# meudnaes/VoronoiRT

Measured on AMD Instinct MI355X. Metric: formal-solve cell-updates/sec, higher is better.
Workload: dtype f64

## Files before the change

### include/voronoirt.h

```cpp
#ifndef VORONOIRT_H
#define VORONOIRT_H

#include <stdint.h>

#ifdef __cplusplus
extern "C" {
#endif

#define VRT_OK 0
#define VRT_EINVAL (-1)
#define VRT_EGRID (-2)
#define VRT_ENODEVICE (-3)
#define VRT_ENOMEM (-4)
#define VRT_EIO (-5)

typedef struct vrt_grid vrt_grid;
typedef struct vrt_plan vrt_plan;

#define VRT_ALPHA_SITE 0
#define VRT_ALPHA_SITE_LAM 1
#define VRT_ALPHA_ANGLE_SITE_LAM 2
#define VRT_ALPHA_ANGLE_NATIVE 3
#define VRT_ALPHA_SITE_LAM_NATIVE 4

// ... 36 lines not shown
int64_t vrt_plan_num_levels(const vrt_plan *p);
int64_t vrt_plan_num_nodes(const vrt_plan *p);
int vrt_plan_get_upwind(const vrt_plan *p, int64_t angle, int64_t *up, double *dots, double *w,
                        double *r);

int vrt_plan_execute(vrt_plan *p, int64_t nlam, int64_t ld, const double *S, const double *alpha,
                     int alpha_mode, const double *I0_up, const double *I0_down,
                     const double *weights, double *J, double *I_out);
int vrt_plan_execute_dev(vrt_plan *p, int64_t nlam, int64_t ld, const double *dS,
                         const double *dalpha, int alpha_mode, const double *dI0_up,
                         const double *dI0_down, const double *weights_host, double *dJ,
                         double *dI_out, void *stream);
int vrt_grid_get_storage_order(const vrt_grid *g, int dir, int64_t *out);
int64_t vrt_plan_native_alpha_count(const vrt_plan *p, int64_t nlam);
int vrt_plan_native_pair_block(const vrt_plan *p);
int vrt_plan_native_pair_block_f32(const vrt_plan *p);
int vrt_plan_alpha_to_native_dev(vrt_plan *p, int64_t nlam, int64_t ld, const double *dalpha,
                                 double *dalpha_native, void *stream);
int vrt_plan_alpha_to_native_dev_f32(vrt_plan *p, int64_t nlam, int64_t ld, const float *dalpha,
                                     float *dalpha_native, void *stream);

int64_t vrt_plan_native_plane_count(const vrt_plan *p, int64_t nlam);
int vrt_plan_to_native_dev(vrt_plan *p, int64_t nlam, int64_t ld, const double *d_in, double *d_up, double *d_down,
                           void *stream);
int vrt_plan_from_native_dev(vrt_plan *p, int dir, int64_t nlam, int64_t ld, const double *d_native, double *d_out,
                             void *stream);
int vrt_plan_j_from_native_dev(vrt_plan *p, int64_t nlam, int64_t ld, const double *dJ_up, const double *dJ_down,
                               double *dJ, void *stream);
int vrt_plan_execute_native_dev(vrt_plan *p, int64_t nlam, const double *dS_up, const double *dS_down,
                                const double *dalpha, int alpha_mode, const double *dI0_up, const double *dI0_down,
                                const double *weights_host, double *dJ_up, double *dJ_down, void *stream);
int vrt_plan_to_native_dev_f32(vrt_plan *p, int64_t nlam, int64_t ld, const float *d_in, float *d_up, float *d_down,
                               void *stream);
int vrt_plan_from_native_dev_f32(vrt_plan *p, int dir, int64_t nlam, int64_t ld, const float *d_native, float *d_out,
                                 void *stream);
int vrt_plan_j_from_native_dev_f32(vrt_plan *p, int64_t nlam, int64_t ld, const float *dJ_up, const float *dJ_down,
                                   float *dJ, void *stream);
int vrt_plan_execute_native_dev_f32(vrt_plan *p, int64_t nlam, const float *dS_up, const float *dS_down,
                                    const float *dalpha, int alpha_mode, const float *dI0_up, const float *dI0_down,
                                    const double *weights_host, float *dJ_up, float *dJ_down, void *stream);

int vrt_lambda_update_native_dev(vrt_grid *g, int64_t nlam, const double *dJ_up, const double *dJ_down,
                                 const double *dB_up, const double *deps, double *dS_up, double *dS_down,
                                 double *max_rel_change, void *stream);
int vrt_rates_populations_native_dev(vrt_grid *g, int64_t nlam, const double *lambda, const int64_t blocks[6],
                                     const double *dJ_up, const double *dJ_down, const double *planck2,
                                     double lambda0, double c0, const double *d_doppler_width, const double *d_gamma,
                                     double sigma_bb_const, const double *sigma_bf1, const double *sigma_bf2,
                                     const double *d_temperature, const double *d_lte_populations, double hc_over_kB,
                                     double pref_ij, double pref_ji, const double *d_C, const double *d_atom_density,
                                     double *d_R, double *d_populations, void *stream);
int vrt_lambda_update_native_dev_f32(vrt_plan *p, int64_t nlam, const float *dJ_up, const float *dJ_down,
                                     const float *dB_up, const double *deps, float *dS_up, float *dS_down,
                                     double *max_rel_change, void *stream);
int vrt_rates_populations_native_dev_f32(vrt_plan *p, int64_t nlam, const double *lambda, const int64_t blocks[6],
                                         const float *dJ_up, const float *dJ_down, const double *planck2,
                                         double lambda0, double c0, const double *d_doppler_width, const double *d_gamma,
                                         double sigma_bb_const, const double *sigma_bf1, const double *sigma_bf2,
                                         const double *d_temperature, const double *d_lte_populations, double hc_over_kB,
                                         double pref_ij, double pref_ji, const double *d_C, const double *d_atom_density,
                                         double *d_R, double *d_populations, void *stream);
int vrt_rate_shares_native_dev(vrt_grid *g, int64_t nlam, int64_t l0, int64_t l1, const double *lambda,
                               const int64_t blocks[6], const double *dJ_up, const double *dJ_down, const double *planck2,
                               double lambda0, double c0, const double *d_doppler_width, const double *d_gamma,
                               double sigma_bb_const, const double *sigma_bf1, const double *sigma_bf2,
                               const double *d_temperature, const double *d_lte_populations, double hc_over_kB,
                               double pref_ij, double pref_ji, double *d_shares, void *stream);
int vrt_rate_shares_native_dev_f32(vrt_plan *p, int64_t nlam, int64_t l0, int64_t l1, const double *lambda,
                                   const int64_t blocks[6], const float *dJ_up, const float *dJ_down, const double *planck2,
                                   double lambda0, double c0, const double *d_doppler_width, const double *d_gamma,
                                   double sigma_bb_const, const double *sigma_bf1, const double *sigma_bf2,
                                   const double *d_temperature, const double *d_lte_populations, double hc_over_kB,
                                   double pref_ij, double pref_ji, double *d_shares, void *stream);
int vrt_populations_from_shares_dev(int64_t n, const double *d_shares, const double *d_C, const double *d_atom_density,
                                    double *d_R, double *d_populations, void *stream);

int vrt_plan_execute_dev_f32(vrt_plan *p, int64_t nlam, int64_t ld, const float *dS,
                             const float *dalpha, int alpha_mode, const float *dI0_up,
                             const float *dI0_down, const double *weights_host, float *dJ,
                             float *dI_out, void *stream);
int vrt_plan_last_sweep_timing(const vrt_plan *p, double *ms, int64_t *launches);
int vrt_plan_patch_layout(const vrt_plan *p, int64_t *out);
int vrt_patch_dispatch_map(int order, int nrow, int nsplit, int lg_siblings, int64_t nred, int steps, int64_t *dims, int32_t *blocks);
int vrt_plan_patch_timeline(vrt_plan *p, int64_t cap_launches, int64_t cap_blocks, int64_t *launches, uint64_t *stamps, int64_t *counts);
int vrt_plan_check(vrt_plan *p);
int vrt_plan_last_path(const vrt_plan *p);
int vrt_plan_set_option(vrt_plan *p, const char *name, const char *value);
int vrt_grid_set_option(vrt_grid *g, const char *name, const char *value);

typedef struct vrt_schedule vrt_schedule;
int vrt_schedule_build(const vrt_grid *g, int dir, const int64_t *up, int n_sweeps, vrt_schedule **out);
int64_t vrt_schedule_num_nodes(const vrt_schedule *s);
int64_t vrt_schedule_num_levels(const vrt_schedule *s);
int vrt_schedule_get(const vrt_schedule *s, int64_t *site, int32_t *zflags, int64_t *level_off);
void vrt_schedule_destroy(vrt_schedule *s);
int vrt_layer_schedule(const vrt_grid *g, int dir, const int64_t *up, int n_sweeps, uint32_t *vis,
                       int32_t *nlev, int64_t *n_visits);
int vrt_layer_sorted_slots(const vrt_grid *g, int dir, const uint32_t *vis, int64_t *store, int64_t *self);

typedef struct vrt_patch_schedule vrt_patch_schedule;
int vrt_patch_schedule_build(const vrt_grid *g, int dir, const int64_t *up, int n_sweeps, int own_target,
                             int entry_cap, vrt_patch_schedule **out, int64_t counts[6]);
int vrt_patch_schedule_get(const vrt_patch_schedule *s, int32_t *layer_patch_off, int32_t *patch_own_lo,
                           int32_t *patch_own_cnt, int32_t *patch_nlev, int64_t *patch_ent_off,
                           int32_t *entry_pos, uint32_t *entry_vis, uint32_t *entry_loc);
int vrt_patch_schedule_get_deps(const vrt_patch_schedule *s, int64_t *dep_off, int32_t *dep_list);
int vrt_patch_schedule_get_layers(const vrt_patch_schedule *s, uint32_t *vis, int32_t *nlev, int64_t *n_visits);
void vrt_patch_schedule_destroy(vrt_patch_schedule *s);

int vrt_delaunay_up(vrt_grid *g, const double k[3], const double *S, const double *I0,
                    int64_t nI0, const double *alpha, int n_sweeps, double *I_out);
int vrt_delaunay_down(vrt_grid *g, const double k[3], const double *S, const double *I0,
                      int64_t nI0, const double *alpha, int n_sweeps, double *I_out);

#define VRT_METRIC_EUCLIDEAN   0
#define VRT_METRIC_PERIODIC_XY 1
#define VRT_RASTER_NEAREST     1
#define VRT_RASTER_INV_DIST2   2
int vrt_grid_nearest(vrt_grid *g, int64_t nq, const double *q_zxy, int metric, int k, int64_t *idx, double *dist);
int vrt_grid_to_raster_dev(vrt_grid *g, int64_t nz, int64_t nx, int64_t ny, const double *z, const double *x,
                           const double *y, int metric, int mode, int64_t nf, int64_t ld, const double *d_fields,
                           double *d_raster, void *stream);
int vrt_raster_to_grid_dev(vrt_grid *g, int64_t nz, int64_t nx, int64_t ny, const double *z, const double *x,
                           const double *y, int64_t nf, const double *d_raster, int64_t ld, double *d_fields,
                           void *stream);
int vrt_grid_to_raster(vrt_grid *g, int64_t nz, int64_t nx, int64_t ny, const double *z, const double *x,
                       const double *y, int metric, int mode, int64_t nf, int64_t ld, const double *fields,
                       double *raster);
int vrt_raster_to_grid(vrt_grid *g, int64_t nz, int64_t nx, int64_t ny, const double *z, const double *x,
                       const double *y, int64_t nf, const double *raster, int64_t ld, double *fields);
int vrt_grid_raster_stats(const vrt_grid *g, double *nearest_ms, double *gather_ms, int64_t *queries,
                          int64_t *walk_steps, int64_t *fallbacks);

int vrt_sample_sites(int device, int64_t nz, int64_t nx, int64_t ny, const double *z, const double *x, const double *y,
                     const double *quantity, int64_t n_sites, uint64_t seed, int64_t batch, int64_t max_proposals,
                     double *pos_zxy, int64_t *proposals_used);
int vrt_sample_sites_dev(int device, int64_t nz, int64_t nx, int64_t ny, const double *z, const double *x,
                         const double *y, const double *d_quantity, int64_t n_sites, uint64_t seed, int64_t batch,
                         int64_t max_proposals, double *d_pos_zxy, int64_t *proposals_used, void *stream);

int vrt_lambda_update_dev(vrt_grid *g, int64_t nlam, int64_t ld, const double *dJ, const double *dB,
                          const double *deps, const double *dS_old, double *dS_new,
                          double *max_rel_change, void *stream);

int vrt_line_opacity_dev(vrt_plan *p, int64_t nlam, const double *lambda, double lambda0, double c0,
                         const double *d_velocity, const double *d_doppler_width, const double *d_gamma,
                         const double *d_line_strength, const double *d_alpha_cont, double *d_alpha_native,
                         void *stream);
int vrt_line_opacity_dev_f32(vrt_plan *p, int64_t nlam, const double *lambda, double lambda0, double c0,
                             const double *d_velocity, const double *d_doppler_width, const double *d_gamma,
                             const double *d_line_strength, const double *d_alpha_cont, float *d_alpha_native,
                             void *stream);

int vrt_plan_execute_line(vrt_plan *p, int64_t nlam, int64_t ld, const double *lambda, double lambda0, double c0,
                          const double *velocity, const double *doppler_width, const double *gamma,
                          const double *line_strength, const double *alpha_cont, const double *S, const double *I0_up,
                          const double *I0_down, const double *weights, double *J);

int vrt_line_terms_dev(vrt_grid *g, const double *d_gamma_static, const double *d_gamma_unsold,
                       const double *d_populations, double strength_const, double Bij, double Bji, double *d_gamma,
                       double *d_line_strength, void *stream);

typedef struct vrt_lambda vrt_lambda;
typedef struct vrt_line_case {
    int64_t nlam;
    const double *lambda;
// ... 209 lines not shown
```

### voronoirt_amd/_lib.py

```python
from __future__ import annotations

import ctypes
import os

HERE = os.path.dirname(os.path.abspath(__file__))
LIB_PATH = os.path.join(HERE, "libvrt_hip.so")
if os.environ.get("VRT_LIB_PATH"):
    LIB_PATH = os.environ["VRT_LIB_PATH"]

c_i64 = ctypes.c_int64
c_dbl = ctypes.c_double
p_i64 = ctypes.POINTER(ctypes.c_int64)
p_i32 = ctypes.POINTER(ctypes.c_int32)
p_dbl = ctypes.POINTER(ctypes.c_double)
p_int = ctypes.POINTER(ctypes.c_int)
vp = ctypes.c_void_p

VRT_OK, VRT_EINVAL, VRT_EGRID, VRT_ENODEVICE, VRT_ENOMEM, VRT_EIO = 0, -1, -2, -3, -4, -5
ALPHA_SITE, ALPHA_SITE_LAM, ALPHA_ANGLE_SITE_LAM, ALPHA_ANGLE_NATIVE, ALPHA_SITE_LAM_NATIVE = 0, 1, 2, 3, 4
METRIC_EUCLIDEAN, METRIC_PERIODIC_XY = 0, 1
RASTER_NEAREST, RASTER_INV_DIST2 = 1, 2
REG_FORMS = ("solve<256>", "solve<1024>", "xy_march_lds<1>", "xy_march_lds<2>", "xy_march_lds<4>", "xy_march_lds<0>",
             "xy_march_mem")
REG_FORM_KERNEL_MASK, REG_FORM_YZ_ROW_MARCH, REG_FORM_XZ_ROW_MARCH = 0xff, 0x100, 0x200
# ... 28 lines not shown
    "vrt_tessellate_sites": (ctypes.c_int, [c_i64, p_dbl, p_dbl, c_i64, c_i64, p_i64, p_i64, p_i64]),
    "vrt_write_neighbours_file": (ctypes.c_int, [ctypes.c_char_p, c_i64, p_i64, c_i64]),
    "vrt_grid_n": (c_i64, [vp]),
    "vrt_grid_max_neighbours": (c_i64, [vp]),
    "vrt_grid_num_layer_offsets": (c_i64, [vp, ctypes.c_int]),
    "vrt_grid_get_layers": (ctypes.c_int, [vp, ctypes.c_int, p_i64]),
    "vrt_grid_get_perm": (ctypes.c_int, [vp, ctypes.c_int, p_i64]),
    "vrt_grid_get_delaunay_lines": (ctypes.c_int, [vp, p_dbl]),
    "vrt_direction": (None, [c_dbl, c_dbl, p_dbl]),
    "vrt_plan_create": (ctypes.c_int, [vp, c_i64, p_dbl, ctypes.c_int, ctypes.POINTER(vp)]),
    "vrt_plan_create_ex": (ctypes.c_int, [vp, c_i64, p_dbl, p_int, ctypes.c_int,
                                          ctypes.POINTER(vp)]),
    "vrt_plan_destroy": (None, [vp]),
    "vrt_plan_num_levels": (c_i64, [vp]),
    "vrt_plan_num_nodes": (c_i64, [vp]),
    "vrt_plan_get_upwind": (ctypes.c_int, [vp, c_i64, p_i64, p_dbl, p_dbl, p_dbl]),
    "vrt_plan_execute": (ctypes.c_int, [vp, c_i64, c_i64, p_dbl, p_dbl, ctypes.c_int, p_dbl, p_dbl,
                                        p_dbl, p_dbl, p_dbl]),
    "vrt_plan_execute_dev": (ctypes.c_int, [vp, c_i64, c_i64, vp, vp, ctypes.c_int, vp, vp, p_dbl,
                                            vp, vp, vp]),
    "vrt_plan_execute_dev_f32": (ctypes.c_int, [vp, c_i64, c_i64, vp, vp, ctypes.c_int, vp, vp, p_dbl,
                                                vp, vp, vp]),
    "vrt_plan_native_plane_count": (c_i64, [vp, c_i64]),
    "vrt_plan_to_native_dev": (ctypes.c_int, [vp, c_i64, c_i64, vp, vp, vp, vp]),
    "vrt_plan_from_native_dev": (ctypes.c_int, [vp, ctypes.c_int, c_i64, c_i64, vp, vp, vp]),
    "vrt_plan_j_from_native_dev": (ctypes.c_int, [vp, c_i64, c_i64, vp, vp, vp, vp]),
    "vrt_plan_execute_native_dev": (ctypes.c_int, [vp, c_i64, vp, vp, vp, ctypes.c_int, vp, vp, p_dbl, vp, vp, vp]),
    "vrt_plan_to_native_dev_f32": (ctypes.c_int, [vp, c_i64, c_i64, vp, vp, vp, vp]),
    "vrt_plan_from_native_dev_f32": (ctypes.c_int, [vp, ctypes.c_int, c_i64, c_i64, vp, vp, vp]),
    "vrt_plan_j_from_native_dev_f32": (ctypes.c_int, [vp, c_i64, c_i64, vp, vp, vp, vp]),
    "vrt_plan_execute_native_dev_f32": (ctypes.c_int, [vp, c_i64, vp, vp, vp, ctypes.c_int, vp, vp, p_dbl, vp, vp, vp]),
    "vrt_plan_check": (ctypes.c_int, [vp]),
    "vrt_lambda_update_native_dev": (ctypes.c_int, [vp, c_i64, vp, vp, vp, vp, vp, vp, p_dbl, vp]),
    "vrt_rates_populations_native_dev": (ctypes.c_int, [vp, c_i64, p_dbl, p_i64, vp, vp, p_dbl, c_dbl, c_dbl, vp, vp,
                                                        c_dbl, p_dbl, p_dbl, vp, vp, c_dbl, c_dbl, c_dbl, vp, vp, vp,
                                                        vp, vp]),
    "vrt_lambda_update_native_dev_f32": (ctypes.c_int, [vp, c_i64, vp, vp, vp, vp, vp, vp, p_dbl, vp]),
    "vrt_rates_populations_native_dev_f32": (ctypes.c_int, [vp, c_i64, p_dbl, p_i64, vp, vp, p_dbl, c_dbl, c_dbl, vp, vp,
                                                            c_dbl, p_dbl, p_dbl, vp, vp, c_dbl, c_dbl, c_dbl, vp, vp, vp,
                                                            vp, vp]),
    "vrt_rate_shares_native_dev": (ctypes.c_int, [vp, c_i64, c_i64, c_i64, p_dbl, p_i64, vp, vp, p_dbl, c_dbl, c_dbl, vp, vp,
                                                  c_dbl, p_dbl, p_dbl, vp, vp, c_dbl, c_dbl, c_dbl, vp, vp]),
    "vrt_rate_shares_native_dev_f32": (ctypes.c_int, [vp, c_i64, c_i64, c_i64, p_dbl, p_i64, vp, vp, p_dbl, c_dbl, c_dbl, vp, vp,
                                                      c_dbl, p_dbl, p_dbl, vp, vp, c_dbl, c_dbl, c_dbl, vp, vp]),
    "vrt_populations_from_shares_dev": (ctypes.c_int, [c_i64, vp, vp, vp, vp, vp, vp]),
    "vrt_grid_get_storage_order": (ctypes.c_int, [vp, ctypes.c_int, p_i64]),
    "vrt_plan_native_alpha_count": (c_i64, [vp, c_i64]),
    "vrt_plan_native_pair_block": (ctypes.c_int, [vp]),
    "vrt_plan_native_pair_block_f32": (ctypes.c_int, [vp]),
    "vrt_plan_alpha_to_native_dev": (ctypes.c_int, [vp, c_i64, c_i64, vp, vp, vp]),
    "vrt_line_opacity_dev": (ctypes.c_int, [vp, c_i64, p_dbl, c_dbl, c_dbl, vp, vp, vp, vp, vp, vp, vp]),
    "vrt_line_opacity_dev_f32": (ctypes.c_int, [vp, c_i64, p_dbl, c_dbl, c_dbl, vp, vp, vp, vp, vp, vp, vp]),
    "vrt_plan_alpha_to_native_dev_f32": (ctypes.c_int, [vp, c_i64, c_i64, vp, vp, vp]),
    "vrt_plan_execute_line": (ctypes.c_int, [vp, c_i64, c_i64, p_dbl, c_dbl, c_dbl, p_dbl, p_dbl, p_dbl, p_dbl, p_dbl,
                                             p_dbl, p_dbl, p_dbl, p_dbl, p_dbl]),
    "vrt_line_terms_dev": (ctypes.c_int, [vp, vp, vp, vp, c_dbl, c_dbl, c_dbl, vp, vp, vp]),
    "vrt_lambda_create": (ctypes.c_int, [vp, ctypes.POINTER(LineCaseStruct), p_dbl, ctypes.POINTER(vp)]),
    "vrt_lambda_create_f32": (ctypes.c_int, [vp, ctypes.POINTER(LineCaseStruct), p_dbl, ctypes.POINTER(vp)]),
    "vrt_lambda_storage": (ctypes.c_int, [vp]),
    "vrt_lambda_iterate": (ctypes.c_int, [vp, p_dbl]),
    "vrt_lambda_get": (ctypes.c_int, [vp, p_dbl, p_dbl, p_dbl, p_dbl, p_dbl]),
    "vrt_lambda_destroy": (None, [vp]),
    "vrt_multi_create": (ctypes.c_int, [ctypes.c_int, p_int, c_i64, p_dbl, p_i64, c_i64, p_dbl, c_i64, p_dbl, p_int,
                                        ctypes.c_int, ctypes.POINTER(vp)]),
    "vrt_multi_execute": (ctypes.c_int, [vp, c_i64, c_i64, p_dbl, p_dbl, ctypes.c_int, p_dbl, p_dbl, p_dbl, p_dbl]),
    "vrt_multi_set_shard": (ctypes.c_int, [vp, ctypes.c_char_p]),
    "vrt_multi_last_shard": (ctypes.c_int, [vp]),
    "vrt_multi_uses_rccl": (ctypes.c_int, [vp]),
    "vrt_multi_destroy": (None, [vp]),
    "vrt_multi_execute_line": (ctypes.c_int, [vp, c_i64, c_i64, p_dbl, c_dbl, c_dbl, p_dbl, p_dbl, p_dbl, p_dbl, p_dbl, p_dbl,
                                              p_dbl, p_dbl, p_dbl, p_dbl]),
    "vrt_multi_lambda_create": (ctypes.c_int, [vp, ctypes.POINTER(LineCaseStruct), p_dbl, ctypes.POINTER(vp)]),
    "vrt_multi_lambda_create_f32": (ctypes.c_int, [vp, ctypes.POINTER(LineCaseStruct), p_dbl, ctypes.POINTER(vp)]),
    "vrt_multi_lambda_storage": (ctypes.c_int, [vp]),
    "vrt_multi_lambda_iterate": (ctypes.c_int, [vp, p_dbl]),
    "vrt_multi_lambda_get": (ctypes.c_int, [vp, p_dbl, p_dbl, p_dbl, p_dbl, p_dbl]),
    "vrt_multi_lambda_destroy": (None, [vp]),
    "vrt_rates_populations_dev": (ctypes.c_int, [vp, c_i64, c_i64, p_dbl, p_i64, vp, p_dbl, c_dbl, c_dbl, vp, vp,
                                                 c_dbl, p_dbl, p_dbl, vp, vp, c_dbl, c_dbl, c_dbl, vp, vp, vp,
                                                 vp, vp]),
    "vrt_plan_last_sweep_timing": (ctypes.c_int, [vp, p_dbl, p_i64]),
    "vrt_plan_patch_layout": (ctypes.c_int, [vp, p_i64]),
    "vrt_patch_dispatch_map": (ctypes.c_int, [ctypes.c_int, ctypes.c_int, ctypes.c_int, ctypes.c_int, c_i64, ctypes.c_int, p_i64, p_i32]),
    "vrt_plan_patch_timeline": (ctypes.c_int, [vp, c_i64, c_i64, p_i64, ctypes.POINTER(ctypes.c_uint64), p_i64]),
    "vrt_plan_last_path": (ctypes.c_int, [vp]),
    "vrt_plan_set_option": (ctypes.c_int, [vp, ctypes.c_char_p, ctypes.c_char_p]),
    "vrt_grid_set_option": (ctypes.c_int, [vp, ctypes.c_char_p, ctypes.c_char_p]),
    "vrt_schedule_build": (ctypes.c_int, [vp, ctypes.c_int, p_i64, ctypes.c_int,
                                          ctypes.POINTER(vp)]),
    "vrt_schedule_num_nodes": (c_i64, [vp]),
    "vrt_schedule_num_levels": (c_i64, [vp]),
    "vrt_schedule_get": (ctypes.c_int, [vp, p_i64, p_i32, p_i64]),
    "vrt_schedule_destroy": (None, [vp]),
    "vrt_layer_schedule": (ctypes.c_int, [vp, ctypes.c_int, p_i64, ctypes.c_int,
                                          ctypes.POINTER(ctypes.c_uint32), p_i32, p_i64]),
    "vrt_layer_sorted_slots": (ctypes.c_int, [vp, ctypes.c_int, ctypes.POINTER(ctypes.c_uint32), p_i64, p_i64]),
    "vrt_patch_schedule_build": (ctypes.c_int, [vp, ctypes.c_int, p_i64, ctypes.c_int, ctypes.c_int, ctypes.c_int,
                                                ctypes.POINTER(vp), p_i64]),
    "vrt_patch_schedule_get": (ctypes.c_int, [vp, p_i32, p_i32, p_i32, p_i32, p_i64, p_i32,
                                              ctypes.POINTER(ctypes.c_uint32), ctypes.POINTER(ctypes.c_uint32)]),
    "vrt_patch_schedule_get_deps": (ctypes.c_int, [vp, p_i64, p_i32]),
    "vrt_patch_schedule_get_layers": (ctypes.c_int, [vp, ctypes.POINTER(ctypes.c_uint32), p_i32, p_i64]),
    "vrt_patch_schedule_destroy": (None, [vp]),
    "vrt_lambda_update_dev": (ctypes.c_int, [vp, c_i64, c_i64, vp, vp, vp, vp, vp, p_dbl, vp]),
    "vrt_short_characteristics": (ctypes.c_int, [c_i64, c_i64, c_i64, p_dbl, p_dbl, p_dbl, c_i64, p_dbl,
                                                 p_int, p_dbl, c_i64, p_dbl, c_i64, p_dbl, ctypes.c_int,
                                                 ctypes.c_int, p_dbl]),
    "vrt_regular_create": (ctypes.c_int, [c_i64, c_i64, c_i64, p_dbl, p_dbl, p_dbl, ctypes.c_int,
                                          ctypes.POINTER(vp)]),
    "vrt_regular_destroy": (None, [vp]),
    "vrt_regular_execute_dev": (ctypes.c_int, [vp, c_i64, p_dbl, p_int, vp, c_i64, vp, c_i64, c_i64, vp,
                                               ctypes.c_int, vp, vp]),
    "vrt_regular_last_solve_ms": (ctypes.c_int, [vp, p_dbl]),
    "vrt_regular_last_launch_form": (ctypes.c_int, [vp, p_int, p_int]),
    "vrt_regular_execute_line": (ctypes.c_int, [vp, c_i64, p_dbl, p_int, p_dbl, c_i64, p_dbl, c_dbl, c_dbl, p_dbl, p_dbl,
                                                p_dbl, p_dbl, p_dbl, p_dbl, p_dbl, ctypes.c_int, p_dbl]),
    "vrt_regular_lambda_create": (ctypes.c_int, [vp, c_i64, p_dbl, p_int, p_dbl, ctypes.POINTER(LineCaseStruct), ctypes.c_int,
                                                 ctypes.POINTER(vp)]),
    "vrt_regular_lambda_iterate": (ctypes.c_int, [vp, p_dbl]),
    "vrt_regular_lambda_get": (ctypes.c_int, [vp, p_dbl, p_dbl, p_dbl, p_dbl, p_dbl]),
    "vrt_regular_lambda_destroy": (None, [vp]),
    "vrt_synth_opacity_dev": (ctypes.c_int, [c_i64, c_i64, c_i64, p_dbl, c_i64, p_dbl, p_dbl, c_dbl, c_dbl, c_dbl, c_dbl,
                                             c_dbl, c_dbl, c_dbl, c_dbl, vp, vp, vp, vp, vp, vp, vp, vp, vp, vp]),
    "vrt_synth_opacity": (ctypes.c_int, [ctypes.c_int, c_i64, c_i64, c_i64, p_dbl, c_i64, p_dbl, p_dbl, c_dbl, c_dbl,
                                         c_dbl, c_dbl, c_dbl, c_dbl, c_dbl, c_dbl, p_dbl, p_dbl, p_dbl, p_dbl, p_dbl,
                                         p_dbl, p_dbl, p_dbl, p_dbl]),
    "vrt_regular_emergent_dev": (ctypes.c_int, [vp, p_dbl, c_i64, vp, vp, ctypes.c_int, vp, vp]),
    "vrt_top_intensity": (ctypes.c_int, [c_i64, c_i64, c_i64, p_dbl, p_dbl, p_dbl, p_dbl, c_i64, p_dbl, p_dbl,
                                         ctypes.c_int, ctypes.c_int, p_dbl]),
    "vrt_tau_unity_dev": (ctypes.c_int, [c_i64, c_i64, c_i64, p_dbl, p_dbl, p_dbl, p_dbl, c_i64, vp, vp, vp]),
    "vrt_tau_unity": (ctypes.c_int, [c_i64, c_i64, c_i64, p_dbl, p_dbl, p_dbl, p_dbl, c_i64, p_dbl, ctypes.c_int,
                                     p_dbl]),
    "vrt_grid_nearest": (ctypes.c_int, [vp, c_i64, p_dbl, ctypes.c_int, ctypes.c_int, p_i64, p_dbl]),
    "vrt_grid_to_raster_dev": (ctypes.c_int, [vp, c_i64, c_i64, c_i64, p_dbl, p_dbl, p_dbl, ctypes.c_int, ctypes.c_int,
                                              c_i64, c_i64, vp, vp, vp]),
    "vrt_raster_to_grid_dev": (ctypes.c_int, [vp, c_i64, c_i64, c_i64, p_dbl, p_dbl, p_dbl, c_i64, vp, c_i64, vp, vp]),
    "vrt_grid_to_raster": (ctypes.c_int, [vp, c_i64, c_i64, c_i64, p_dbl, p_dbl, p_dbl, ctypes.c_int, ctypes.c_int,
                                          c_i64, c_i64, p_dbl, p_dbl]),
    "vrt_raster_to_grid": (ctypes.c_int, [vp, c_i64, c_i64, c_i64, p_dbl, p_dbl, p_dbl, c_i64, p_dbl, c_i64, p_dbl]),
    "vrt_grid_raster_stats": (ctypes.c_int, [vp, p_dbl, p_dbl, p_i64, p_i64, p_i64]),
    "vrt_sample_sites": (ctypes.c_int, [ctypes.c_int, c_i64, c_i64, c_i64, p_dbl, p_dbl, p_dbl, p_dbl, c_i64,
                                        ctypes.c_uint64, c_i64, c_i64, p_dbl, p_i64]),
    "vrt_sample_sites_dev": (ctypes.c_int, [ctypes.c_int, c_i64, c_i64, c_i64, p_dbl, p_dbl, p_dbl, vp, c_i64,
                                            ctypes.c_uint64, c_i64, c_i64, vp, p_i64, vp]),
    "vrt_ng_accelerate_dev": (ctypes.c_int, [c_i64, vp, vp, vp, vp, vp, p_dbl, p_dbl, p_int, vp]),
    "vrt_ng_sums_dev": (ctypes.c_int, [c_i64, vp, vp, vp, vp, p_dbl, vp]),
    "vrt_ng_coefficients": (ctypes.c_int, [p_dbl, p_dbl]),
    "vrt_ng_apply_dev": (ctypes.c_int, [c_i64, c_dbl, c_dbl, vp, vp, vp, vp, p_int, vp]),
    "vrt_lambda_set_acceleration": (ctypes.c_int, [vp, ctypes.c_int, ctypes.c_int, ctypes.c_int]),
    "vrt_regular_lambda_set_acceleration": (ctypes.c_int, [vp, ctypes.c_int, ctypes.c_int, ctypes.c_int]),
    "vrt_lambda_last_acceleration": (ctypes.c_int, [vp, p_int, p_dbl, p_dbl]),
    "vrt_regular_lambda_last_acceleration": (ctypes.c_int, [vp, p_int, p_dbl, p_dbl]),
    "vrt_lambda_set_state": (ctypes.c_int, [vp, p_dbl, p_dbl]),
    "vrt_regular_lambda_set_state": (ctypes.c_int, [vp, p_dbl, p_dbl]),
    "vrt_multi_lambda_set_state": (ctypes.c_int, [vp, p_dbl, p_dbl]),
    "vrt_continuum_case_check": (ctypes.c_int, [ctypes.POINTER(ContinuumCaseStruct), c_i64]),
    "vrt_continuum_create": (ctypes.c_int, [vp, ctypes.POINTER(ContinuumCaseStruct), p_dbl, ctypes.POINTER(vp)]),
    "vrt_continuum_iterate": (ctypes.c_int, [vp, p_dbl]),
    "vrt_continuum_get": (ctypes.c_int, [vp, p_dbl, p_dbl]),
    "vrt_continuum_set_source": (ctypes.c_int, [vp, p_dbl]),
    "vrt_continuum_set_acceleration": (ctypes.c_int, [vp, ctypes.c_int, ctypes.c_int, ctypes.c_int]),
    "vrt_continuum_last_acceleration": (ctypes.c_int, [vp, p_int, p_dbl, p_dbl]),
    "vrt_continuum_destroy": (None, [vp]),
    "vrt_regular_continuum_create": (ctypes.c_int, [vp, c_i64, p_dbl, p_int, p_dbl, ctypes.POINTER(ContinuumCaseStruct),
                                                    ctypes.c_int, ctypes.POINTER(vp)]),
    "vrt_regular_continuum_iterate": (ctypes.c_int, [vp, p_dbl]),
# ... 87 lines not shown
```

### voronoirt_amd/api.py

```python
from __future__ import annotations

import ctypes
import os
import re
import weakref

import numpy as np

from . import _lib
from ._lib import VrtError, check

QUADRATURE_DIR = os.path.join(os.path.dirname(os.path.abspath(__file__)), "quadratures")


def _d(a):
    return a.ctypes.data_as(_lib.p_dbl) if a is not None else None


def _i(a):
    return a.ctypes.data_as(_lib.p_i64) if a is not None else None


def _f64(a):
    return np.ascontiguousarray(a, dtype=np.float64)
# ... 247 lines not shown

    def to_native_dev(self, nlam: int, ld: int, d_in: int, d_up: int = 0, d_down: int = 0, stream: int = 0, f32: bool = False) -> None:
        fn = _lib.load().vrt_plan_to_native_dev_f32 if f32 else _lib.load().vrt_plan_to_native_dev
        check(fn(self._h, nlam, ld, d_in, d_up or None, d_down or None, stream or None))

    def from_native_dev(self, d: int, nlam: int, ld: int, d_native: int, d_out: int, stream: int = 0, f32: bool = False) -> None:
        fn = _lib.load().vrt_plan_from_native_dev_f32 if f32 else _lib.load().vrt_plan_from_native_dev
        check(fn(self._h, int(d), nlam, ld, d_native, d_out, stream or None))

    def J_from_native_dev(self, nlam: int, ld: int, dJ_up: int, dJ_down: int, dJ: int, stream: int = 0, f32: bool = False) -> None:
        fn = _lib.load().vrt_plan_j_from_native_dev_f32 if f32 else _lib.load().vrt_plan_j_from_native_dev
        check(fn(self._h, nlam, ld, dJ_up or None, dJ_down or None, dJ, stream or None))

    def execute_native_dev(self, nlam: int, dS_up: int, dS_down: int, dalpha: int, alpha_mode: int, weights,
                           dJ_up: int = 0, dJ_down: int = 0, dI0_up: int = 0, dI0_down: int = 0, stream: int = 0,
                           f32: bool = False) -> None:
        w = _f64(weights)
        fn = _lib.load().vrt_plan_execute_native_dev_f32 if f32 else _lib.load().vrt_plan_execute_native_dev
        check(fn(self._h, nlam, dS_up or None, dS_down or None, dalpha, alpha_mode, dI0_up or None, dI0_down or None, _d(w),
                 dJ_up or None, dJ_down or None, stream or None))

    def check(self) -> None:
        check(_lib.load().vrt_plan_check(self._h))

    def native_alpha_count(self, nlam: int) -> int:
        return int(_lib.load().vrt_plan_native_alpha_count(self._h, nlam))

    @property
    def native_pair_block(self) -> int:
        return int(_lib.load().vrt_plan_native_pair_block(self._h))

    @property
    def native_pair_block_f32(self) -> int:
        return int(_lib.load().vrt_plan_native_pair_block_f32(self._h))

    def native_to_site_major(self, native, nlam: int, n_angles: int):
        native = np.asarray(native)
        n = self.sites.n
        B = self.native_pair_block_f32 if native.dtype == np.float32 else self.native_pair_block
        npair = (nlam + 1) // 2
        per = native.reshape(n_angles, npair * n * 2)
        out = np.empty((n_angles, n, 2 * npair), dtype=native.dtype)
        q0 = 0
        widths = [B] * (npair // B) + [1 << b for b in range(B.bit_length() - 2, -1, -1) if (npair % B) & (1 << b)]
        for w in widths:
            blk = per[:, q0 * n * 2:(q0 + w) * n * 2].reshape(n_angles, n, 2 * w)
            out[:, :, 2 * q0:2 * (q0 + w)] = blk
            q0 += w
        return out[:, :, :nlam]

    def alpha_to_native_dev(self, nlam: int, ld: int, dalpha: int, dalpha_native: int, stream: int = 0,
                            f32: bool = False) -> None:
        fn = _lib.load().vrt_plan_alpha_to_native_dev_f32 if f32 else _lib.load().vrt_plan_alpha_to_native_dev
        check(fn(self._h, nlam, ld, dalpha, dalpha_native, stream or None))

    def line_opacity_dev(self, lam, lambda0: float, c0: float, d_velocity: int, d_doppler: int, d_gamma: int,
                         d_line_strength: int, d_alpha_cont: int, d_alpha_native: int, stream: int = 0,
                         f32: bool = False) -> None:
        lam = _f64(lam)
        fn = _lib.load().vrt_line_opacity_dev_f32 if f32 else _lib.load().vrt_line_opacity_dev
        check(fn(self._h, lam.size, _d(lam), float(lambda0), float(c0), d_velocity, d_doppler, d_gamma, d_line_strength,
                 d_alpha_cont, d_alpha_native, stream or None))

    def line_lambda_diagonal_dev(self, nlam: int, d_alpha_native: int, weights, ld: int, d_diag: int, stream: int = 0) -> None:
        check(_lib.load().vrt_line_lambda_diagonal_dev(self._h, nlam, d_alpha_native, _d(_f64(weights)), ld, d_diag,
                                                       stream or None))

    def set_option(self, name: str, value) -> None:
        if getattr(self, "_h", None):
            check(_lib.load().vrt_plan_set_option(self._h, name.encode(), str(value).encode()))

    def last_sweep_timing(self):
        ms = ctypes.c_double()
        launches = ctypes.c_int64()
        check(_lib.load().vrt_plan_last_sweep_timing(self._h, ctypes.byref(ms),
                                                     ctypes.byref(launches)))
        return ms.value, launches.value

    @property
    def patch_layout(self) -> dict:
        out = (ctypes.c_int64 * 4)()
        check(_lib.load().vrt_plan_patch_layout(self._h, out))
        return {"patches": out[0], "fewest_per_angle_layer": out[1], "work_slots": out[2], "padding_slots": out[3]}

    @property
    def last_launches(self) -> int:
        return int(self.last_sweep_timing()[1])

    @property
    def last_path(self) -> str:
        return {0: "", 1: "levels", 2: "tiles", 3: "steps", 4: "patches"}[int(_lib.load().vrt_plan_last_path(self._h))]

    def close(self):
        if getattr(self, "_h", None) is not None and self._h:
            _lib.load().vrt_plan_destroy(self._h)
            self._h = None

    def __del__(self):
        try:
            self.close()
        except Exception:
            pass


class MultiDevicePlan:

    def __init__(self, positions, neighbours, bounds, k, dirs=None, n_sweeps: int = 3, devices=(0,)):
        L = _lib.load()
        pos = _f64(positions)
        nbr = np.ascontiguousarray(neighbours, dtype=np.int64)
        b = np.array([float(v) for v in bounds], dtype=np.float64)
        self.k = _f64(np.atleast_2d(k))
        self.n, self.n_angles = pos.shape[0], self.k.shape[0]
        dev = np.ascontiguousarray(devices, dtype=np.int32)
        d = np.ascontiguousarray(dirs, dtype=np.int32) if dirs is not None else None
        h = ctypes.c_void_p()
        check(L.vrt_multi_create(dev.size, dev.ctypes.data_as(_lib.p_int), self.n, _d(pos), _i(nbr), nbr.shape[0], _d(b),
                                 self.n_angles, _d(self.k), d.ctypes.data_as(_lib.p_int) if d is not None else None,
                                 int(n_sweeps), ctypes.byref(h)))
        self._h = h

    def set_shard(self, mode: str) -> None:
        check(_lib.load().vrt_multi_set_shard(self._h, mode.encode()))

    @property
    def last_shard(self) -> str:
        return {0: "", 1: "lambda", 2: "angle"}[int(_lib.load().vrt_multi_last_shard(self._h))]

    @property
    def uses_rccl(self) -> bool:
        return bool(_lib.load().vrt_multi_uses_rccl(self._h))

    def execute(self, S, alpha, weights, I0_up=None, I0_down=None, alpha_mode=None) -> np.ndarray:
        S = _f64(S)
        if S.ndim == 1:
            S = S.reshape(-1, 1)
        n, nlam = S.shape
        alpha = _f64(alpha)
        if alpha_mode is None:
            alpha_mode = {1: _lib.ALPHA_SITE, 2: _lib.ALPHA_SITE_LAM, 3: _lib.ALPHA_ANGLE_SITE_LAM}[alpha.ndim]
        if I0_up is not None:
            I0_up = _f64(I0_up).reshape(-1, nlam)
        if I0_down is not None:
            I0_down = _f64(I0_down).reshape(-1, nlam)
        w = _f64(weights)
        J = np.zeros((n, nlam))
        check(_lib.load().vrt_multi_execute(self._h, nlam, nlam, _d(S), _d(alpha), alpha_mode, _d(I0_up), _d(I0_down),
                                            _d(w), _d(J)))
        return J

    def execute_line(self, S, populations, case, weights, perm_up, n1: int) -> np.ndarray:
        S = _f64(S)
        n, nlam = S.shape
        pops = np.asarray(populations)
        gamma = _f64(case.gamma(pops))
        strength = _f64(case.strength_const * (pops[0] * case.Bij - pops[1] * case.Bji))
        lam, vel, dop, ac = _f64(case.lam), _f64(case.velocity), _f64(case.doppler), _f64(case.alpha_cont)
        I0 = _f64(np.asarray(case.B0)[np.asarray(perm_up)[:n1] - 1])
        J = np.zeros((n, nlam))
        check(_lib.load().vrt_multi_execute_line(self._h, nlam, nlam, _d(lam), float(case.lambda0), float(case.c0), _d(vel),
                                                 _d(dop), _d(gamma), _d(strength), _d(ac), _d(S), _d(I0), None,
                                                 _d(_f64(weights)), _d(J)))
        return J

    def lambda_iteration(self, eps_conv: float, maxiter: int, case, weights, S0=None, populations0=None, checkpoint=None,
                         checkpoint_every: int = 1, resume=None, ng=None, storage: str = "f64"):
# ... 1323 lines not shown
```

### voronoirt_amd/csrc/vrt_api.cpp

```cpp
#include <algorithm>
#include <atomic>
#include <chrono>
#include <cmath>
#include <cstdio>
#include <cstdlib>
#include <cstring>
#include <memory>
#include <new>
#include <thread>

#include "vrt_internal.h"
#include "vrt_line_case.h"

namespace vrt {

static thread_local std::string g_err;

void set_error(const std::string &msg) { g_err = msg; }
int fail(int code, const std::string &msg)
{
    g_err = msg;
    return code;
}

int check_source(const double *S, int64_t count)
{
    for (int64_t i = 0; i < count; i++)
        if (!std::isfinite(S[i]) || !(S[i] > 0.0)) return fail(VRT_EINVAL, "S must be finite and > 0 everywhere");
    return VRT_OK;
}

int check_state_pointers(const void *session, const double *S, const double *populations)
{
    if (!session) return fail(VRT_EINVAL, "NULL session");
    if (!S && !populations) return fail(VRT_EINVAL, "S and populations are both NULL: nothing to set");
    return VRT_OK;
}

int check_state(int64_t n, int64_t nlam, const double *S, const double *populations)
{
    if (S)
        if (int rc = check_source(S, n * nlam)) return rc;
    if (populations)
        for (int64_t i = 0; i < 3 * n; i++)
            if (!std::isfinite(populations[i]) || !(populations[i] >= 0.0))
                return fail(VRT_EINVAL, "the populations must be finite and >= 0 everywhere");
    return VRT_OK;
}

void tuning_from_env(Tuning &t)
{
    static const char *names[] = {"VRT_PATH", "VRT_STEP_K", "VRT_STEP_SINGLE", "VRT_STEP_PAIRS", "VRT_STEP_XCD",
                                  "VRT_STEP_STREAMS", "VRT_STEP_LEVEL_MAP", "VRT_STEP_GROUP_DIR", "VRT_TILE_WIDE",
                                  "VRT_TILE_PRE", "VRT_PATCH_K", "VRT_PATCH_NT", "VRT_PATCH_OWN",
                                  "VRT_PATCH_Q", "VRT_PATCH_TARGET", "VRT_PATCH_SPLIT", "VRT_PATCH_ORDER", "VRT_PATCH_TIMELINE", "VRT_PAIR_BLOCK", "VRT_PATCH_QUAD", "VRT_PATCH_LEAN", "VRT_PATCH_CHAIN", "VRT_CHAIN_PAIRS", "VRT_CHAIN_SPIN", "VRT_CHAIN_DATAFLAG", "VRT_CHAIN_STATIC", "VRT_LAMBDA_NATIVE", "VRT_DEBUG_FLAGS", "VRT_DEBUG_SKIP_LEVELS",
                                  "VRT_TILE_DEBUG"};
    for (const char *nm : names) {
        const char *e = std::getenv(nm);
        if (e && *e && tuning_set(t, nm, e, false) != VRT_OK) {
            static std::mutex mu;
            static std::vector<std::string> said;
            std::lock_guard<std::mutex> lock(mu);
            if (std::find(said.begin(), said.end(), std::string(nm)) == said.end()) {
                said.push_back(nm);
                std::fprintf(stderr, "[libvrt_hip] ignoring %s=%s: %s\n", nm, e, g_err.c_str());
            }
        }
    }
}

int tuning_set(Tuning &t, const char *name, const char *value, bool created)
{
    if (!name || !value) return fail(VRT_EINVAL, "NULL option name or value");
    const std::string nm(name), v(value);
    if (nm == "VRT_PATH") {
        static const char *paths[] = {"auto", "levels", "tiles", "steps", "patches"};
        for (int i = 0; i < 5; i++)
            if (v == paths[i]) { t.path = i; return VRT_OK; }
        if (v.empty()) { t.path = 0; return VRT_OK; }
        return fail(VRT_EINVAL, "VRT_PATH must be auto, levels, tiles, steps or patches");
    }
    char *end = nullptr;
    const long x = std::strtol(value, &end, 10);
    if (end == value || *end != 0) return fail(VRT_EINVAL, "option " + nm + " needs an integer value");
    struct { const char *name; int *field; long lo, hi; bool creation_only; } tab[] = {
        {"VRT_STEP_K", &t.step_K, 0, 18, false}, {"VRT_STEP_SINGLE", &t.step_single, 0, 1, false},
        {"VRT_STEP_PAIRS", &t.step_pairs, 0, 64, false}, {"VRT_STEP_XCD", &t.step_xcd, 0, 2, false},
        {"VRT_STEP_STREAMS", &t.step_streams, 1, 4, false}, {"VRT_STEP_LEVEL_MAP", &t.step_level_map, 0, 1, false},
        {"VRT_STEP_GROUP_DIR", &t.step_group_dir, 0, 1, false}, {"VRT_TILE_WIDE", &t.tile_wide, 0, 1, false},
        {"VRT_TILE_PRE", &t.tile_pre, 0, 1, false},
        {"VRT_PATCH_K", &t.patch_K, 1, 8, true}, {"VRT_PATCH_NT", &t.patch_NT, 64, 1024, true},
        {"VRT_PATCH_OWN", &t.patch_own, 0, 65535, true}, {"VRT_PATCH_Q", &t.patch_Q, 1, 4, false},
        {"VRT_PATCH_TARGET", &t.patch_target, 0, 1 << 20, false}, {"VRT_PATCH_SPLIT", &t.patch_split, 0, 4096, false}, {"VRT_PATCH_ORDER", &t.patch_order, 0, 1, false},
        {"VRT_PATCH_TIMELINE", &t.patch_timeline, 0, 1, false}, {"VRT_PAIR_BLOCK", &t.pair_block, 1, 16, true},
        {"VRT_PATCH_QUAD", &t.patch_quad, 0, 1, true}, {"VRT_PATCH_LEAN", &t.patch_lean, 0, 1, false},
        {"VRT_PATCH_CHAIN", &t.patch_chain, 0, 2, false}, {"VRT_CHAIN_PAIRS", &t.chain_pairs, 1, 256, false},
        {"VRT_CHAIN_SPIN", &t.chain_spin, 1, 1 << 20, false}, {"VRT_CHAIN_DATAFLAG", &t.chain_dataflag, 0, 2, false},
        {"VRT_LAMBDA_NATIVE", &t.lambda_native, 0, 1, false}, {"VRT_CHAIN_STATIC", &t.chain_static, 0, 1, false}, {"VRT_DEBUG_FLAGS", &t.debug_flags, 0, 1 << 20, false},
        {"VRT_DEBUG_SKIP_LEVELS", &t.debug_skip_levels, 0, 1, false}, {"VRT_TILE_DEBUG", &t.tile_debug, 0, 1, false},
    };
    for (auto &o : tab)
        if (nm == o.name) {
            if (o.creation_only && created)
                return fail(VRT_EINVAL, "option " + nm + " shapes what plan creation builds: preset it in the environment");
            if (x < o.lo || x > o.hi) return fail(VRT_EINVAL, "option " + nm + " out of range");
            *o.field = (int)x;
            return VRT_OK;
        }
    return fail(VRT_EINVAL, "unknown option " + nm);
}

int use_device(int device)
{
    if (device < 0)
        return fail(VRT_ENODEVICE, "host-only grid handle (device < 0): no compute without a HIP device");
    int cnt = 0;
    hipError_t e = hipGetDeviceCount(&cnt);
    if (e != hipSuccess || cnt <= 0)
        return fail(VRT_ENODEVICE, "no HIP device available (libvrt_hip has no CPU fallback)");
    if (device < 0 || device >= cnt) return fail(VRT_EINVAL, "device ordinal out of range");
    VRT_HIP_TRY(hipSetDevice(device));
    (void)hipGetLastError();
    return VRT_OK;
}

int use_current_device()
{
    int cnt = 0;
    if (hipGetDeviceCount(&cnt) != hipSuccess || cnt <= 0)
        return fail(VRT_ENODEVICE, "no HIP device available (libvrt_hip has no CPU fallback)");
    (void)hipGetLastError();
    return VRT_OK;
}

static int upload_grid(vrt_grid *g)
{
    const int64_t n = g->n;
    const size_t nnz = g->col.size();
    int rc;
    if ((rc = g->d_pos.alloc((size_t)3 * n))) return rc;
    if ((rc = g->d_rowptr.alloc((size_t)n + 1))) return rc;
    if ((rc = g->d_col.alloc(nnz))) return rc;
    if ((rc = g->d_lz.alloc(nnz))) return rc;
    if ((rc = g->d_lx.alloc(nnz))) return rc;
    if ((rc = g->d_ly.alloc(nnz))) return rc;
    if ((rc = g->stream.create())) return rc;
    VRT_HIP_TRY(hipMemcpy(g->d_pos, g->pos.data(), sizeof(double) * 3 * n, hipMemcpyHostToDevice));
    VRT_HIP_TRY(hipMemcpy(g->d_rowptr, g->rowptr.data(), sizeof(int32_t) * (n + 1), hipMemcpyHostToDevice));
    if (nnz)
        VRT_HIP_TRY(hipMemcpy(g->d_col, g->col.data(), sizeof(int32_t) * nnz, hipMemcpyHostToDevice));
    for (int d = 0; d < 2; d++) {
        Direction &dir = d == 0 ? g->up : g->down;
        std::vector<int32_t> order((size_t)n);
        for (int64_t i = 0; i < n; i++) order[(size_t)i] = (int32_t)(dir.perm[(size_t)i] - 1);
        if ((rc = dir.d_order.alloc((size_t)n))) return rc;
        VRT_HIP_TRY(hipMemcpy(dir.d_order, order.data(), sizeof(int32_t) * n, hipMemcpyHostToDevice));
        std::vector<int32_t> rank((size_t)n);
        for (int64_t i = 0; i < n; i++) rank[(size_t)order[(size_t)i]] = (int32_t)i;
        if ((rc = dir.d_rank.alloc((size_t)n))) return rc;
        VRT_HIP_TRY(hipMemcpy(dir.d_rank, rank.data(), sizeof(int32_t) * n, hipMemcpyHostToDevice));
        std::vector<int32_t> srank((size_t)n);
        for (int64_t i = 0; i < n; i++) srank[(size_t)dir.store[(size_t)i]] = (int32_t)i;
        if ((rc = dir.d_store.alloc((size_t)n))) return rc;
        if ((rc = dir.d_srank.alloc((size_t)n))) return rc;
        VRT_HIP_TRY(hipMemcpy(dir.d_store, dir.store.data(), sizeof(int32_t) * n, hipMemcpyHostToDevice));
        VRT_HIP_TRY(hipMemcpy(dir.d_srank, srank.data(), sizeof(int32_t) * n, hipMemcpyHostToDevice));
        std::vector<int32_t> lay(dir.reduced.size());
        for (size_t j = 0; j < lay.size(); j++) lay[j] = (int32_t)(dir.reduced[j] - 1);
        if ((rc = dir.d_lay.alloc(lay.size()))) return rc;
        VRT_HIP_TRY(hipMemcpy(dir.d_lay, lay.data(), sizeof(int32_t) * lay.size(), hipMemcpyHostToDevice));
    }
    if ((rc = launch_delaunay_lines(g))) return rc;
    VRT_HIP_TRY(hipStreamSynchronize(g->stream));
    return VRT_OK;
}

// ... 1069 lines not shown
    if (alpha_mode < 0 || alpha_mode > 2) return fail(VRT_EINVAL, "bad alpha_mode (host arrays: 0, 1 or 2)");
    return guarded([&] {
        std::lock_guard<std::mutex> lock(p->mu);
        vrt_grid *g = p->g;
        int rc = use_device(g->device);
        if (rc) return rc;
        const size_t n = (size_t)g->n;
        const size_t nS = n * (size_t)ld;
        const size_t nA = alpha_mode == VRT_ALPHA_SITE ? n
                          : alpha_mode == VRT_ALPHA_SITE_LAM ? nS
                                                             : nS * (size_t)p->n_angles_user;
        const size_t nU = (size_t)g->up.n1 * (size_t)nlam, nD = (size_t)g->down.n1 * (size_t)nlam;
        hipStream_t st = g->stream;
        if ((rc = p->d_stage[0].grow(nS))) return rc;
        if ((rc = p->d_stage[1].grow(nA))) return rc;
        VRT_HIP_TRY(hipMemcpyAsync(p->d_stage[0], S, sizeof(double) * nS, hipMemcpyHostToDevice, st));
        VRT_HIP_TRY(hipMemcpyAsync(p->d_stage[1], alpha, sizeof(double) * nA, hipMemcpyHostToDevice, st));
        double *dU = nullptr, *dD = nullptr, *dJ = nullptr;
        if (I0_up && nU) {
            if ((rc = p->d_stage[2].grow(nU))) return rc;
            dU = p->d_stage[2];
            VRT_HIP_TRY(hipMemcpyAsync(dU, I0_up, sizeof(double) * nU, hipMemcpyHostToDevice, st));
        }
        if (I0_down && nD) {
            if ((rc = p->d_stage[3].grow(nD))) return rc;
            dD = p->d_stage[3];
            VRT_HIP_TRY(hipMemcpyAsync(dD, I0_down, sizeof(double) * nD, hipMemcpyHostToDevice, st));
        }
        if (J) {
            if ((rc = p->d_stage[4].grow(nS))) return rc;
            dJ = p->d_stage[4];
        }
        double *dIo = nullptr;
        if (I_out) {
            if ((rc = p->d_stage[5].grow(nS * (size_t)p->n_angles_user))) return rc;
            dIo = p->d_stage[5];
        }
        rc = execute_locked(p, caller_args(nlam, ld, p->d_stage[0], p->d_stage[1], alpha_mode, dU, dD, weights, dJ, dIo, st, false));
        if (rc) return rc;
        if (J) VRT_HIP_TRY(hipMemcpyAsync(J, dJ, sizeof(double) * nS, hipMemcpyDeviceToHost, st));
        if (I_out)
            VRT_HIP_TRY(hipMemcpyAsync(I_out, dIo, sizeof(double) * nS * (size_t)p->n_angles_user,
                                       hipMemcpyDeviceToHost, st));
        VRT_HIP_TRY(hipStreamSynchronize(st));
        return patch_chain_check(p);
    });
}

int vrt_plan_check(vrt_plan *p)
{
    if (!p) return fail(VRT_EINVAL, "NULL plan");
    return guarded([&] {
        std::lock_guard<std::mutex> lock(p->mu);
        return patch_chain_check(p);
    });
}

int vrt_plan_patch_layout(const vrt_plan *p, int64_t *out)
{
    if (!p || !out) return fail(VRT_EINVAL, "NULL plan or output");
    const int maxL = p->tile_max_layers;
    int64_t fewest = 0;
    if (p->patch_ok && !p->h_patch_first.empty()) {
        fewest = INT64_MAX;
        for (int a = 0; a < p->A; a++)
            for (int layer = 2; layer <= maxL; layer++) {
                const int32_t *first = p->h_patch_first.data() + (size_t)a * (size_t)(maxL + 2);
                fewest = std::min<int64_t>(fewest, first[layer + 1] - first[layer]);
            }
        if (fewest == INT64_MAX) fewest = 0;
    }
    out[0] = p->patch_ok ? p->n_patches : 0;
    out[1] = fewest;
    out[2] = p->patch_work_off.empty() ? 0 : p->patch_work_off.back();
    out[3] = p->patch_work_padding;
    return VRT_OK;
}

int vrt_patch_dispatch_map(int order, int nrow, int nsplit, int lg_siblings, int64_t nred, int steps, int64_t *dims, int32_t *blocks)
{
    return guarded([&] { return patch_dispatch_map(order, nrow, nsplit, lg_siblings, nred, steps, dims, blocks); });
}

int vrt_plan_patch_timeline(vrt_plan *p, int64_t cap_launches, int64_t cap_blocks, int64_t *launches, uint64_t *stamps, int64_t *counts)
{
    if (!p || !launches || !stamps || !counts) return fail(VRT_EINVAL, "NULL plan or output");
    return guarded([&] {
        std::lock_guard<std::mutex> lock(p->mu);
        if (int rc = use_device(p->device)) return rc;
        return patch_timeline_read(p, cap_launches, cap_blocks, launches, stamps, counts);
    });
}

int vrt_plan_last_sweep_timing(const vrt_plan *p, double *ms, int64_t *launches)
{
    if (!p) return fail(VRT_EINVAL, "NULL plan");
    if (!p->ev_valid) return fail(VRT_EINVAL, "no execute has run on this plan yet");
    return guarded([&] {
        VRT_HIP_TRY(hipEventSynchronize(p->ev1));
        float t = 0.f;
        VRT_HIP_TRY(hipEventElapsedTime(&t, p->ev0, p->ev1));
        if (ms) *ms = (double)t;
        if (launches) *launches = p->last_launches;
        return patch_chain_check(const_cast<vrt_plan *>(p));
    });
}

int vrt_plan_last_path(const vrt_plan *p) { return p ? p->last_path : 0; }

int vrt_plan_set_option(vrt_plan *p, const char *name, const char *value)
{
    if (!p) return fail(VRT_EINVAL, "NULL plan");
    return guarded([&] {
        std::lock_guard<std::mutex> lock(p->mu);
        return tuning_set(p->tune, name, value, true);
    });
}

int vrt_grid_set_option(vrt_grid *g, const char *name, const char *value)
{
    if (!g) return fail(VRT_EINVAL, "NULL grid");
    return guarded([&] {
        if (name && std::string(name) == "VRT_NEAREST_CELLS") {
            if (!value) return fail(VRT_EINVAL, "NULL value");
            const std::string v(value);
            int64_t cells = 0;
            if (v != "auto") {
                char *end = nullptr;
                const long long c = std::strtoll(v.c_str(), &end, 10);
                if (v.empty() || *end || c < 1 || c > 256) return fail(VRT_EINVAL, "VRT_NEAREST_CELLS: auto or 1..256");
                cells = c;
            }
            std::lock_guard<std::mutex> lock(g->mu);
            g->nearest_cells = cells;
            return VRT_OK;
        }
        Tuning probe;
        int rc = tuning_set(probe, name, value, false);
        if (rc) return rc;
        std::lock_guard<std::mutex> lock(g->mu);
        bool found = false;
        for (auto &o : g->options)
            if (o.first == name) { o.second = value; found = true; }
        if (!found) g->options.emplace_back(name, value);
        for (auto &c : g->cache) {
            std::lock_guard<std::mutex> plock(c->plan->mu);
            (void)tuning_set(c->plan->tune, name, value, true);
        }
        return VRT_OK;
    });
}

int vrt_lambda_update_dev(vrt_grid *g, int64_t nlam, int64_t ld, const double *dJ, const double *dB,
                          const double *deps, const double *dS_old, double *dS_new, double *max_rel_change,
                          void *stream)
{
    return guarded([&] {
        if (!g || !dJ || !dB || !deps || !dS_old || !dS_new || !max_rel_change)
            return fail(VRT_EINVAL, "NULL argument");
        if (nlam < 1 || ld < nlam) return fail(VRT_EINVAL, "need nlam >= 1 and ld >= nlam");
        hipStream_t st = (hipStream_t)stream;
        return lambda_update_call(g, max_rel_change, st, "vrt_lambda_update_dev", [&](unsigned long long *d_res) {
            return launch_lambda_update(g->n, nlam, ld, dJ, dB, deps, dS_old, dS_new, d_res, st);
        });
    });
}
// ... 344 lines not shown
```

### voronoirt_amd/csrc/vrt_device.h

```cpp
#pragma once

#include <hip/hip_runtime.h>

#include "vrt_internal.h"
#include "vrt_weights.h"

namespace vrt {

#ifdef VRT_DIAG
constexpr bool kDiag = true;
#else
constexpr bool kDiag = false;
#endif

constexpr uint32_t kNoSlot = 0xFFFFu;

__host__ __device__ __forceinline__ void pair_block_at(int q, int npair, int lgB, int &k0, int &lw)
{
    const int full = npair >> lgB << lgB;
    if (q < full) { k0 = q >> lgB << lgB; lw = lgB; return; }
    int k = full;
    const int r = npair - full;
    for (int bit = lgB - 1; bit >= 0; bit--)
        if (r & (1 << bit)) {
// ... 79 lines not shown
    const double *t_w1, *t_w2, *t_r1, *t_r2;
    const uint32_t *t_vis;
    const uint32_t *t_loc;
    const int32_t *t_self;
    const uint32_t *t_vis_s, *t_loc_s;
    const uint32_t *t_gpos;
    const double *S[2];
    const double *alpha[2];
    const double *alpha_angle;
    double *I;
    long long *dbg;
};

struct DirWeights {
    double w[kMaxAngles];
    int32_t idx[kMaxAngles];
    int count;
};

struct DiagAngles {
    double w[kMaxAngles];
    int down[kMaxAngles];
};
inline DiagAngles diag_angles(const vrt_plan *p, const double *weights)
{
    DiagAngles ang;
    for (int a = 0; a < kMaxAngles; a++) {
        ang.w[a] = a < p->A ? weights[(size_t)p->user_of_active[(size_t)a]] : 0.0;
        ang.down[a] = a < p->A && p->dir_of_active[(size_t)a] < 0;
    }
    return ang;
}

struct StepArgs {
    TileArgs ta;
    int npair;
    int layer;
    int cg_stride;
    double2 *cg_c;
    double2 *cg_g;
    const int32_t *angle_list;
    int n_list;
    int pairs_per_thread;
    int chunks;
    int xcd_map;
    const int32_t *level_map;
    const int32_t *t_rank_s;
    const uint32_t *t_loc_ss;
    int debug_skip_levels;
    int debug_flags;
};

__device__ __forceinline__ double2 ld2(const double2 *base, unsigned idx)
{
    return *reinterpret_cast<const double2 *>(reinterpret_cast<const char *>(base) + ((size_t)idx << 4));
}
__device__ __forceinline__ double2 ld2(const float2 *base, unsigned idx)
{
    return to_d2(*reinterpret_cast<const float2 *>(reinterpret_cast<const char *>(base) + ((size_t)idx << 3)));
}

__device__ __forceinline__ void upwind_term(double r, double w, double a_c, double a_u, double S_c,
                                            double S_u, double I_u, bool early, bool inl, double &t,
                                            double &g, bool cheap = false)
{
    double ca, cb, ce;
    if (cheap) { ca = a_c; cb = a_u; ce = r; }
    else
    lin_weights(r * (a_c + a_u) / 2.0, ca, cb, ce);
    t = early ? ((ce * I_u + ca * S_u) + cb * S_c) * w : (ca * S_u + cb * S_c) * w;
    g = inl ? ce * w : 0.0;
}

struct PatchReduce {
    int nred = 0;
    int nblk[2] = {0, 0};
    int lo[2] = {0, 0}, hi[2] = {0, 0};
    int count[2] = {0, 0};
    int ppb = 4;
    void *Jd[2] = {nullptr, nullptr};
    double w[kMaxAngles];
    int32_t angles[2][kMaxAngles];
};


}
```

### voronoirt_amd/csrc/vrt_internal.h

```cpp
#pragma once

#include <hip/hip_runtime.h>

#include <algorithm>
#include <cmath>
#include <cstdint>
#include <cstring>
#include <memory>
#include <mutex>
#include <new>
#include <string>
#include <thread>
#include <vector>

#include "voronoirt.h"

namespace vrt {

void set_error(const std::string &msg);
int fail(int code, const std::string &msg);

int check_source(const double *S, int64_t count);
int check_state_pointers(const void *session, const double *S, const double *populations);
int check_state(int64_t n, int64_t nlam, const double *S, const double *populations);
// ... 171 lines not shown
    }
    operator hipEvent_t() const { return e; }
};

template <typename Body>
inline bool run_workers(int count, Body body)
{
    std::vector<char> threw((size_t)std::max(count, 1), 0);
    auto guarded = [&](int t) {
        try {
            body(t);
        } catch (...) {
            threw[(size_t)t] = 1;
        }
    };
    std::vector<std::thread> pool;
    try {
        pool.reserve((size_t)std::max(count, 1));
    } catch (...) {
    }
    for (int t = 0; t < count; t++) {
        try {
            pool.emplace_back(guarded, t);
        } catch (...) {
            guarded(t);
        }
    }
    for (auto &th : pool) th.join();
    for (int t = 0; t < count; t++)
        if (threw[(size_t)t]) return false;
    return true;
}

constexpr int kMaxAngles = 64;
constexpr int64_t kMaxGuess = 70;
constexpr int32_t kNoUpwind = -1;

struct Direction {
    std::vector<int32_t> layer_of;
    std::vector<int64_t> perm;
    std::vector<int64_t> reduced;
    int64_t n1 = 0;
    DevBuf<int32_t> d_order;
    DevBuf<int32_t> d_rank;
    DevBuf<int32_t> d_lay;
    std::vector<int32_t> store;
    DevBuf<int32_t> d_store;
    DevBuf<int32_t> d_srank;
};

struct PlanCacheEntry;

struct CopyLane {
    Stream st;
    HostBuf<char> pin[2];
    Event ev[2];
};
constexpr size_t kCopyChunk = (size_t)8 << 20;

struct Tuning {
    int path = 0;
    int step_K = 0;
    int step_single = 0;
    int step_pairs = 0;
    int step_xcd = 2;
    int step_streams = 2;
    int step_level_map = 1;
    int step_group_dir = 1;
    int tile_wide = 1;
    int tile_pre = 1;
    int patch_K = 1, patch_NT = 512;
    int patch_own = 0;
    int patch_Q = 1;
    int pair_block = 1;
    int patch_quad = 1;
    int patch_lean = 1;
    int patch_chain = 2;
    int chain_pairs = 9;
    int chain_spin = 2048;
    int chain_dataflag = 2;
    int patch_split = 0;
    int patch_target = 0;
    int patch_order = 1;
    int patch_timeline = 0;
    int chain_static = 1;
    int lambda_native = 1;
    int debug_flags = 0, debug_skip_levels = 0, tile_debug = 0;
};
void tuning_from_env(Tuning &t);
int tuning_set(Tuning &t, const char *name, const char *value, bool created);

struct ExecArgs {
    int64_t nlam = 0, ld = 0;
    const void *S = nullptr;
    const void *S_nat[2] = {nullptr, nullptr};
    const void *alpha = nullptr;
    int alpha_mode = 0;
    const void *I0[2] = {nullptr, nullptr};
    const double *weights = nullptr;
    void *J = nullptr;
    void *J_nat[2] = {nullptr, nullptr};
    void *I_out = nullptr;
    bool native = false;
    bool f32 = false;
    hipStream_t st = nullptr;
    bool wants_J() const { return native ? J_nat[0] != nullptr : J != nullptr; }
};
inline ExecArgs caller_args(int64_t nlam, int64_t ld, const void *S, const void *alpha, int alpha_mode, const void *I0_up,
                            const void *I0_down, const double *weights, void *J, void *I_out, hipStream_t st, bool f32)
{
    ExecArgs x;
    x.nlam = nlam; x.ld = ld;
    x.S = S;
    x.alpha = alpha; x.alpha_mode = alpha_mode;
    x.I0[0] = I0_up; x.I0[1] = I0_down;
    x.weights = weights;
    x.J = J; x.I_out = I_out;
    x.f32 = f32;
    x.st = st;
    return x;
}
inline ExecArgs native_args(int64_t nlam, const void *S_up, const void *S_down, const void *alpha, int alpha_mode,
                            const void *I0_up, const void *I0_down, const double *weights, void *J_up, void *J_down,
                            hipStream_t st, bool f32)
{
    ExecArgs x = caller_args(nlam, (nlam + 1) / 2 * 2, nullptr, alpha, alpha_mode, I0_up, I0_down, weights, nullptr, nullptr,
                             st, f32);
    x.S_nat[0] = S_up; x.S_nat[1] = S_down;
    x.J_nat[0] = J_up; x.J_nat[1] = J_down;
    x.native = true;
    return x;
}

struct ChainItems {
    int npair = -1, lgB = -1, nsplit = -1, reduce = -1;
    DevBuf<int4> items;
    DevBuf<int32_t> deps;
    int q_off[9] = {0, 0, 0, 0, 0, 0, 0, 0, 0};
    bool segments_even = false;
};
struct ChainLaunch {
    static constexpr size_t kSets = 4;
    std::vector<ChainItems> sets;
    DevWork<uint32_t> progress;
    bool progress_fresh = false;
    DevBuf<uint32_t> ctrl;
    HostBuf<uint32_t> h_status;
    uint32_t *d_status = nullptr;
    DevBuf<char> d_args;
    HostBuf<char> h_args_pinned;
    std::vector<char> h_args;
    Event args_ev;
    bool args_ev_valid = false;
    uint32_t epoch = 0;

    uint32_t *ctrl_words() const { return ctrl; }
    template <typename Make>
    int select(int npair, int lgB, int nsplit, bool reduce, Make make)
    {
        for (size_t c = 0; c < sets.size(); c++)
            if (sets[c].npair == npair && sets[c].lgB == lgB && sets[c].nsplit == nsplit && sets[c].reduce == (reduce ? 1 : 0)) {
                std::rotate(sets.begin(), sets.begin() + (long)c, sets.begin() + (long)c + 1);
                return VRT_OK;
            }
        sets.reserve(kSets);
        if (sets.size() == kSets) sets.pop_back();
// ... 39 lines not shown
    std::vector<std::unique_ptr<vrt::PlanCacheEntry>> cache;
    std::unique_ptr<vrt::RasterLocator, vrt::RasterLocatorDelete> locator;
    int64_t nearest_cells = 0;
};

struct vrt_plan {
    vrt_grid *g = nullptr;
    int device = 0;
    vrt::Tuning tune;
    int n_sweeps = 3;
    int64_t n_angles_user = 0;
    int A = 0;
    std::vector<int> user_of_active;
    std::vector<int> dir_of_active;
    std::vector<double> k;
    vrt::DevBuf<int32_t> d_up1, d_up2;
    vrt::DevBuf<double> d_d1, d_d2;
    vrt::DevBuf<double> d_w1, d_w2;
    vrt::DevBuf<double> d_r1, d_r2;
    vrt::DevBuf<uint32_t> d_node_site;
    vrt::DevBuf<uint32_t> d_node_meta;
    vrt::DevBuf<int32_t> d_node_u1, d_node_u2;
    std::vector<int64_t> level_off;
    bool level_ready = false;
    std::vector<int32_t> h_up1, h_up2;
    int64_t n_nodes = 0;
    vrt::DevBuf<int32_t> d_angles_up, d_angles_down;
    int n_up = 0, n_down = 0;
    std::vector<int64_t> skip_site;
    vrt::DevWork<double> d_I;
    int64_t I_ld = 0;
    vrt::DevWork<double> d_stage[6];
    bool tile_ok = false;
    bool step_tables_ready = false;
    int tile_K = 8;
    int tile_max_layers = 0;
    int64_t tile_max_layer_size = 0;
    int64_t tile_visits = 0;
    vrt::DevBuf<int32_t> t_u1, t_u2;
    vrt::DevBuf<double> t_w1, t_w2, t_r1, t_r2;
    vrt::DevBuf<uint32_t> t_vis, t_loc;
    vrt::DevBuf<int32_t> t_self;
    vrt::DevBuf<uint32_t> t_vis_s, t_loc_s;
    vrt::DevBuf<uint32_t> t_gpos;
    vrt::DevBuf<int32_t> t_rank_s;
    vrt::DevBuf<uint32_t> t_loc_ss;
    vrt::DevBuf<uint32_t> t_code_ss;
    vrt::DevBuf<int32_t> d_nlev, d_angle_dir;
    std::vector<int64_t> angle_visits;
    std::vector<int32_t> h_task_map;
    vrt::DevWork<int32_t> d_task_map;
    int task_map_nlam = -1;
    vrt::DevWork<double> ws_S[2], ws_A[2], ws_J[2];
    vrt::DevWork<double> ws_AA;
    vrt::DevWork<double> ws_cg[2];
    int step_groups = 0;
    vrt::DevBuf<int32_t> d_step_angles;
    std::vector<int> step_group_off;
    std::vector<double> angle_mean_levels;
    vrt::DevBuf<int32_t> d_level_map;
    std::vector<int> level_map_off;
    int level_map_units = 0, level_map_groups = 0;
    std::vector<int32_t> h_step_angles;
    bool patch_ok = false;
    int lg_pair_block = 0;
    int patch_cap = 0, patch_K = 0, patch_NT = 0;
    int64_t n_patches = 0, n_patch_entries = 0, n_patch_visits = 0;
    std::vector<int32_t> h_patch_first;
    std::vector<int4> h_patch_rec;
    vrt::DevBuf<int32_t> e_pos, e_u1, e_u2;
    vrt::DevBuf<uint32_t> e_vis, e_loc;
    vrt::DevBuf<double> e_w1, e_w2, e_r1, e_r2;
    std::vector<int2> h_patch_rec2;
    std::vector<int64_t> h_patch_dep_off;
    std::vector<int32_t> h_patch_deps;
    vrt::ChainLaunch chain;
    vrt::DevBuf<int4> d_patch_work;
    std::vector<int64_t> patch_work_off;
    int patch_work_groups = 0;
    int64_t patch_work_padding = 0;
    vrt::DevBuf<unsigned long long> d_patch_tl;
    std::vector<int64_t> patch_tl_launches;
    int64_t patch_tl_blocks = 0;
    vrt::Stream step_stream[4];
    vrt::Event step_fork, step_join[4];
    int last_path = 0;
    vrt::Event ev0, ev1;
    bool ev_valid = false;
    std::vector<vrt::CopyLane> copy_lanes;
    vrt::Event copy_done;
    int64_t last_launches = 0;
    std::mutex mu;
};

namespace vrt {

struct PlanDelete { void operator()(vrt_plan *p) const { vrt_plan_destroy(p); } };
using PlanPtr = std::unique_ptr<vrt_plan, PlanDelete>;
struct GridDelete { void operator()(vrt_grid *g) const { vrt_grid_destroy(g); } };
using GridPtr = std::unique_ptr<vrt_grid, GridDelete>;

struct PlanCacheEntry {
    double k[3];
    int n_sweeps;
    PlanPtr plan;
    int users;
};

int parse_neighbour_file(const char *path, int64_t n, std::vector<int64_t> &matrix, int64_t &D1);
int build_grid_host(vrt_grid *g, int64_t n, const double *pos, const int64_t *nbr, int64_t D1,
                    const double bounds[6]);

int tessellate_host(int64_t n, const double *pos, const double bounds[6], int64_t D1, int64_t *nbr_out,
                    int64_t *max_count, int nthreads);
inline int tessellate_threads(int64_t count)
{
    const unsigned hw = std::thread::hardware_concurrency();
    return (int)std::max<int64_t>(1, std::min<int64_t>({(int64_t)(hw ? hw : 4), 64, count / 256 + 1}));
}
int tessellate_host_sites(int64_t n, const double *pos, const double bounds[6], int64_t D1, int64_t m, const int64_t *sites,
                          int64_t *rows_out, int64_t *max_count, int nthreads);

struct AngleSchedule {
    std::vector<uint32_t> site;
    std::vector<uint8_t> zflags;
    std::vector<int64_t> level_off;
    int64_t bad_site = -1;
};
void build_angle_schedule(const Direction &dir, bool ascending, int64_t n, int n_sweeps,
                          const int32_t *up1, const int32_t *up2, AngleSchedule &out);
struct LayerSchedule {
    std::vector<uint32_t> vis;
    std::vector<int32_t> nlev;
    int64_t n_visits = 0;
    int64_t max_layer_size = 0;
    int64_t bad_site = -1;
    bool ok = false;
};
void build_layer_schedule(const Direction &dir, bool ascending, int64_t n, int n_sweeps,
                          const int32_t *up1, const int32_t *up2, LayerSchedule &out);
void build_sorted_slots(const Direction &dir, int64_t n, const std::vector<uint32_t> &vis_site,
                        std::vector<int32_t> &self);
struct PatchSchedule {
    std::vector<int32_t> layer_patch_off;
    std::vector<int32_t> patch_own_lo;
    std::vector<int32_t> patch_own_cnt;
    std::vector<int32_t> patch_nlev;
    std::vector<int64_t> patch_ent_off;
    std::vector<int32_t> entry_pos;
    std::vector<uint32_t> entry_vis;
    std::vector<uint32_t> entry_loc;
    std::vector<int64_t> dep_off;
    std::vector<int32_t> dep_list;
    int64_t n_visits = 0;
    int64_t n_live = 0;
    int64_t max_entries = 0;
    int64_t bad_site = -1;
    bool ok = false;
};
void build_patch_schedule(const Direction &dir, bool ascending, int64_t n, int n_sweeps, const int32_t *up1,
                          const int32_t *up2, int own_target, int entry_cap, PatchSchedule &out, int threads = 1,
                          LayerSchedule *layers = nullptr);

int launch_delaunay_lines(vrt_grid *g);
int launch_upwind_table(vrt_plan *p, int a);
struct SweepArgs {
// ... 27 lines not shown
int launch_gather_rows(int64_t rows, int64_t nlam, int64_t ld, const int32_t *d_order, const double *d_src, double *d_dst,
                       hipStream_t st);
int launch_gather_rows_f32(int64_t rows, int64_t nlam, int64_t ld, const int32_t *d_order, const double *d_src, float *d_dst,
                           hipStream_t st);
int launch_round_to_f32(size_t count, const double *d_src, float *d_dst, hipStream_t st);
int launch_widen_f32(size_t count, const float *d_src, double *d_dst, hipStream_t st);
int launch_lambda_update(int64_t n, int64_t nlam, int64_t ld, const double *dJ, const double *dB,
                         const double *deps, const double *dS_old, double *dS_new,
                         unsigned long long *d_result, hipStream_t st, const double *d_diag = nullptr);
int launch_lambda_update_native(vrt_grid *g, int64_t nlam, const double *dJ_up, const double *dJ_down, const double *dB_up,
                                const double *deps, double *dS_up, double *dS_down, unsigned long long *d_result, hipStream_t st,
                                const double *dL_up = nullptr);
int launch_line_lambda_diagonal(vrt_plan *p, int64_t nlam, const double *d_alpha_native, const double *weights, int64_t ld,
                                double *d_rows, double *d_up_planes, hipStream_t st);
int launch_lambda_update_native_f32(vrt_plan *p, int64_t nlam, const float *dJ_up, const float *dJ_down, const float *dB_up,
                                    const double *deps, float *dS_up, float *dS_down, unsigned long long *d_result, hipStream_t st);

int launch_line_opacity(vrt_plan *p, int64_t nlam, const double *d_lambda, double lambda0, double c0,
                        const double *d_velocity, const double *d_doppler, const double *d_gamma,
                        const double *d_strength, const double *d_alpha_cont, void *d_out, hipStream_t st,
                        bool f32_out = false);
int launch_line_terms(int64_t n, const double *d_gamma_static, const double *d_gamma_unsold, const double *d_pops,
                      double strength_const, double Bij, double Bji, double *d_gamma, double *d_strength, hipStream_t st);

int execute_locked(vrt_plan *p, const ExecArgs &x);

int ensure_step_tables(vrt_plan *p);
int launch_permute_table(vrt_plan *p, int a, const uint32_t *d_vis_site);
int launch_sorted_tables(vrt_plan *p, int a);
int launch_gpos(vrt_plan *p, int a);
inline int native_lg(const vrt_plan *p, bool f32)
{
    if (!p->patch_ok) return 0;
    return f32 && p->tune.patch_quad != 0 && p->patch_K == 1 ? std::max(p->lg_pair_block, 1) : p->lg_pair_block;
}
int alpha_to_native(vrt_plan *p, int64_t nlam, int64_t ld, const void *dalpha, void *out, hipStream_t st, bool f32);
int native_planes_ok(const vrt_plan *p, bool f32 = false);
int planes_to_native_f32(vrt_plan *p, int64_t nlam, int64_t ld, const float *din, float *out_up, float *out_down, hipStream_t st);
int plane_from_native_f32(vrt_plan *p, int dir_index, int64_t nlam, int64_t ld, const float *din, float *dout, hipStream_t st);
int J_from_native_f32(vrt_plan *p, int64_t nlam, int64_t ld, const float *dJ_up, const float *dJ_down, float *dJ, hipStream_t st);
int planes_to_native(vrt_plan *p, int64_t nlam, int64_t ld, const double *din, double *out_up, double *out_down, hipStream_t st);
int plane_from_native(vrt_plan *p, int dir_index, int64_t nlam, int64_t ld, const double *din, double *dout, hipStream_t st);
int J_from_native(vrt_plan *p, int64_t nlam, int64_t ld, const double *dJ_up, const double *dJ_down, double *dJ, hipStream_t st);
int execute_layers(vrt_plan *p, const ExecArgs &x, int path);
int64_t steps_max_layer(bool f32);
inline int line_path_ok(const vrt_plan *p, const char *who)
{
    if (!p->patch_ok && (!p->tile_ok || p->tile_max_layer_size > steps_max_layer(false)))
        return fail(VRT_EINVAL, std::string(who) + " needs a layer path (at most 4 visits per site and 255 levels per layer)");
    return VRT_OK;
}

struct TileArgs;
struct PatchReduce;
bool patch_shape_exists(int K, int Q, int NT);
struct PatchShape {
    int lgB = 0, quad = 0, lean = 0, lgS = 0, Q = 1;
    bool chain = false, chain_dataflag = false;
};
PatchShape patch_shape(const vrt_plan *p, int npair, bool f32, int Q_asked);
struct PatchIndex {
    const std::vector<int32_t> &first;
    const std::vector<int4> &rec;
    const std::vector<int2> &rec2;
    const std::vector<int64_t> &dep_off;
    const std::vector<int32_t> &deps;
    const std::vector<int> &dir_of_active;
    const std::vector<int64_t> *reduced[2];
    int max_layers;
    int64_t n;
};
void build_patch_work(const PatchIndex &ix, int G, const std::vector<int32_t> &group_angles, const std::vector<int> &group_off,
                      std::vector<int4> &work, std::vector<int64_t> &off, int64_t &padding);
int build_chain_items(const PatchIndex &ix, int nblock, int nsplit, bool with_reduce, std::vector<int4> &items,
                      std::vector<int32_t> &deps, ChainItems &set);
int launch_patch_entries(vrt_plan *p, int a, int64_t first, int64_t count);
int ensure_patch_work(vrt_plan *p, int G, const std::vector<int32_t> &group_angles, const std::vector<int> &group_off);
int launch_patch_layer(vrt_plan *p, const TileArgs &ta, int npair, int layer, int group, const PatchShape &shape, hipStream_t st,
                       bool f32, const PatchReduce *reduce);
constexpr int kPatchTimelineRec = 12;
void patch_timeline_begin(vrt_plan *p);
int patch_timeline_read(vrt_plan *p, int64_t cap_launches, int64_t cap_blocks, int64_t *launches, uint64_t *stamps, int64_t *counts);
int patch_dispatch_map(int order, int nrow, int nsplit, int lg_siblings, int64_t nred, int steps, int64_t *dims, int32_t *blocks);
int launch_patch_chain(vrt_plan *p, const TileArgs &ta, int npair, const PatchShape &shape, hipStream_t st, bool f32,
                       const PatchReduce *reduce, bool ctrl_zeroed = false);
int chain_ctrl_words();
int patch_chain_check(vrt_plan *p);

struct NgRange {
    int64_t dense = 0, tail = 0, tstride = 1;
};
struct NgState {
    int order = 0, start = 0, period = 0;
    DevBuf<double> hist[3];
    unsigned have = 0;
    DevBuf<double> d_ws;
    int last_applied = 0;
    double last_sums[5] = {0, 0, 0, 0, 0}, last_coeffs[2] = {0, 0};
};
inline NgRange ng_S_range(int64_t n, int64_t nlam, bool sweep_order)
{
    NgRange rg;
    if (sweep_order) { rg.dense = (nlam / 2) * 2 * n; rg.tail = nlam & 1 ? n : 0; rg.tstride = 2; }
    else { rg.dense = (n * nlam) & ~(int64_t)1; rg.tail = (n * nlam) & 1; rg.tstride = 1; }
    return rg;
}
int ng_check_settings(int order, int start, int period);
int ng_configure(NgState &ng, int order, int start, int period, size_t alloc_count);
void ng_release(NgState &ng);
int ng_sums(const NgRange &rg, const double *x0, const double *x1, const double *x2, const double *x3, double *d_ws,
            double sums[5], hipStream_t st);
bool ng_coefficients(const double sums[5], double coeffs[2]);
int ng_apply(const NgRange &rg, double a, double b, const double *x0, const double *x1, const double *x2, double *out,
             double *d_ws, bool *ok, hipStream_t st);
enum { kNgNothing = 0, kNgRecord1 = 1, kNgRecord2 = 2, kNgRecord3 = 3, kNgStep = 4 };
inline int ng_due(const NgState &ng, int64_t iterate)
{
    if (!ng.order) return kNgNothing;
    const int64_t d = iterate < ng.start ? ng.start - iterate : (ng.period - (iterate - ng.start) % ng.period) % ng.period;
    return d == 0 ? kNgStep : (d <= 3 ? (int)d : kNgNothing);
}
inline int ng_record(NgState &ng, int d, const double *S, size_t alloc_count, hipStream_t st)
{
    VRT_HIP_TRY(hipMemcpyAsync(ng.hist[d - 1], S, sizeof(double) * alloc_count, hipMemcpyDeviceToDevice, st));
    ng.have |= 1u << (d - 1);
    return VRT_OK;
}
inline bool ng_take_history(NgState &ng)
{
    const bool complete = ng.have == 7u;
    ng.have = 0;
    return complete;
}
inline void ng_add_sums(double total[5], const double part[5], bool first)
{
    for (int k = 0; k < 5; k++) total[k] = first ? part[k] : total[k] + part[k];
}
struct NgPiece {
    NgState *ng;
    DevBuf<double> *S;
    bool good;
};
inline bool ng_commit(NgPiece *pieces, int count, bool coeffs_valid)
{
    if (!coeffs_valid) return false;
    for (int i = 0; i < count; i++)
        if (!pieces[i].good) return false;
    for (int i = 0; i < count; i++) std::swap(*pieces[i].S, pieces[i].ng->hist[2]);
    return true;
}
int ng_after_iterate(NgState &ng, int64_t iterate, DevBuf<double> &S, size_t alloc_count, const NgRange &rg, hipStream_t st);
template <typename Store>
inline int ng_after_update(NgState &ng, int64_t iterate, Store &store, hipStream_t st)
{
    if (!ng.order) {
        ng.last_applied = 0;
        return VRT_OK;
    }
    int rc = ng_after_iterate(ng, iterate, store.ng_S(), store.ng_count(), store.ng_range(), st);
    if (rc || ng.last_applied != 1) return rc;
    bool queued = false;
    if ((rc = store.ng_refresh(st, &queued)) || !queued) return rc;
    VRT_HIP_TRY(hipStreamSynchronize(st));
    return VRT_OK;
}
int ng_report(const NgState &ng, int *applied, double sums[5], double coeffs[2]);
// ... 6 lines not shown
```

### voronoirt_amd/csrc/vrt_layers.hip

```cpp
#include <hip/hip_runtime.h>

#include <algorithm>
#include <cmath>
#include <cstdio>
#include <cstdlib>
#include <cstring>

#include "vrt_device.h"
#include "vrt_internal.h"

#include "vrt_layout_kernels.h"
#include "vrt_step_kernels.h"
#include "vrt_tile_kernels.h"

namespace vrt {

static int build_task_map(vrt_plan *p, int nlam, hipStream_t st)
{
    const int A = p->A;
    if (p->task_map_nlam == nlam && p->d_task_map) return VRT_OK;
    const int ntask = A * nlam;
    struct Group { int a, l0, l1; double cost; };
    std::vector<Group> groups;
    const int halves = nlam >= 2 ? 2 : 1;
// ... 580 lines not shown
                launch_levels1_K<T>(std::max(K1, 1), dim3((unsigned)lblocks),
                                    (size_t)(cnt_l + 1) * sizeof(T), sg, sa);
                r.launches += 2;
                continue;
            }
            if constexpr (!kF32) {
                const size_t lds = (size_t)(cnt_l + 1) * sizeof(double2);
                const dim3 g2((unsigned)lblocks);
                hipLaunchKernelGGL((k_step_coeffs<double, false>), g1, dim3(256), 0, sg, sa);
                switch (step_K) {
                case 1: hipLaunchKernelGGL(k_step_levels<1>, g2, dim3(1024), lds, sg, sa); break;
                case 2: hipLaunchKernelGGL(k_step_levels<2>, g2, dim3(1024), lds, sg, sa); break;
                case 3: hipLaunchKernelGGL(k_step_levels<3>, g2, dim3(1024), lds, sg, sa); break;
                case 4: hipLaunchKernelGGL(k_step_levels<4>, g2, dim3(1024), lds, sg, sa); break;
                case 5: hipLaunchKernelGGL(k_step_levels<5>, g2, dim3(1024), lds, sg, sa); break;
                case 6: hipLaunchKernelGGL(k_step_levels<6>, g2, dim3(1024), lds, sg, sa); break;
                case 7: hipLaunchKernelGGL(k_step_levels<7>, g2, dim3(1024), lds, sg, sa); break;
                default: hipLaunchKernelGGL(k_step_levels<8>, g2, dim3(1024), lds, sg, sa); break;
                }
            }
            r.launches += 2;
        }
    }
    return join_streams(p, st, G);
}

template <typename T>
static int patch_reduce_template(vrt_plan *p, const ExecArgs &x, const LayerRun &r, PatchReduce &red)
{
    int rc;
    for (int a = 0; a < p->A; a++) red.w[a] = x.weights[p->user_of_active[(size_t)a]];
    for (int d = 0; d < 2; d++)
        if (r.use_dir[d] && !x.native && (rc = p->ws_J[d].grow(dcount<T>(r.plane)))) return rc;
    return VRT_OK;
}

template <typename T>
static int run_patch_layers(vrt_plan *p, const ExecArgs &x, LayerRun &r)
{
    constexpr bool kF32 = sizeof(T) == 4;
    vrt_grid *g = p->g;
    const int64_t n = g->n;
    const int A = p->A, G = r.G, npair = r.npair;
    const hipStream_t st = x.st;
    int rc;
    if ((rc = ensure_patch_work(p, G, p->h_step_angles, p->step_group_off))) return rc;
    PatchReduce red_tmpl{};
    int owner_of_dir[2] = {-1, -1};
    int64_t reduced_upto[2] = {0, 0};
    if (x.wants_J()) {
        if ((rc = patch_reduce_template<T>(p, x, r, red_tmpl))) return rc;
        for (int d = 0; d < 2; d++)
            for (int gi = 0; gi < G && r.use_dir[d]; gi++)
                if (group_holds_dir(p, gi, d)) owner_of_dir[d] = gi;
    }
    r.fused_dir[0] = owner_of_dir[0] >= 0;
    r.fused_dir[1] = owner_of_dir[1] >= 0;
    auto make_reduce = [&](int gi, int layer_done, bool final, PatchReduce &red) -> bool {
        red = red_tmpl;
        int k = 0;
        for (int d = 0; d < 2; d++) {
            if (owner_of_dir[d] != gi) continue;
            const Direction &dir = d == 0 ? g->up : g->down;
            const int Ld = (int)dir.reduced.size() - 1;
            int64_t upto = reduced_upto[d];
            if (final) upto = n;
            else if (layer_done >= 1 && layer_done <= Ld) upto = dir.reduced[(size_t)layer_done] - 1;
            if (upto <= reduced_upto[d]) continue;
            red.lo[k] = (int)reduced_upto[d];
            red.hi[k] = (int)upto;
            red.Jd[k] = J_planes(p, x, d);
            red.count[k] = 0;
            for (int a = 0; a < A; a++)
                if ((p->dir_of_active[(size_t)a] > 0) == (d == 0)) red.angles[k][red.count[k]++] = a;
            reduced_upto[d] = upto;
            k++;
        }
        return k > 0;
    };
    const int Lmax = deepest_layer(r);
    if ((rc = fork_streams(p, st, G))) return rc;
    r.launches = 0;
    if (kDiag) patch_timeline_begin(p);
    for (int layer = 2; layer <= Lmax; layer++)
        for (int gi = 0; gi < G; gi++) {
            hipStream_t sg = gi == 0 ? st : p->step_stream[gi];
            if (p->step_group_off[gi + 1] == p->step_group_off[gi]) continue;
            PatchReduce red;
            const bool have_red = make_reduce(gi, layer - 1, false, red);
            if ((rc = launch_patch_layer(p, r.ta, npair, layer, gi, r.shape, sg, kF32, have_red ? &red : nullptr))) return rc;
            r.launches += 1;
        }
    const PatchShape tail = patch_shape(p, npair, kF32, 1);
    for (int gi = 0; gi < G; gi++) {
        PatchReduce red;
        if (!make_reduce(gi, 0, true, red)) continue;
        if ((rc = launch_patch_layer(p, r.ta, npair, p->tile_max_layers + 1, gi, tail, gi == 0 ? st : p->step_stream[gi], kF32, &red)))
            return rc;
        r.launches += 1;
    }
    return join_streams(p, st, G);
}

template <typename T>
static int run_patch_chain(vrt_plan *p, const ExecArgs &x, LayerRun &r)
{
    constexpr bool kF32 = sizeof(T) == 4;
    const int A = p->A;
    const hipStream_t st = x.st;
    int rc;
    if ((rc = ensure_patch_work(p, r.G, p->h_step_angles, p->step_group_off))) return rc;
    PatchReduce red{};
    if (x.wants_J() && (rc = patch_reduce_template<T>(p, x, r, red))) return rc;
    for (int d = 0; d < 2; d++)
        for (int gi = 1; gi < r.G; gi++)
            if (r.use_dir[d] && r.dir_st[d] == p->step_stream[gi]) {
                VRT_HIP_TRY(hipEventRecord(p->step_join[gi], p->step_stream[gi]));
                VRT_HIP_TRY(hipStreamWaitEvent(st, p->step_join[gi], 0));
            }
    VRT_HIP_TRY(hipEventRecord(p->ev0, st));
    if (x.wants_J())
        for (int d = 0; d < 2; d++) {
            red.count[d] = 0;
            red.Jd[d] = r.use_dir[d] ? J_planes(p, x, d) : nullptr;
            for (int a = 0; a < A; a++)
                if ((p->dir_of_active[(size_t)a] > 0) == (d == 0)) red.angles[d][red.count[d]++] = a;
            r.fused_dir[d] = r.use_dir[d];
        }
    if ((rc = launch_patch_chain(p, r.ta, r.npair, r.shape, st, kF32, x.wants_J() ? &red : nullptr, r.prep_ctrl))) return rc;
    r.launches = 1;
    VRT_HIP_TRY(hipEventRecord(p->ev1, st));
    return VRT_OK;
}

template <typename T>
static int finish_outputs(vrt_plan *p, const ExecArgs &x, const LayerRun &r)
{
    vrt_grid *g = p->g;
    const int64_t n = g->n, nlam = x.nlam, ld = x.ld;
    const int A = p->A;
    const hipStream_t st = x.st;
    const T *wI = reinterpret_cast<const T *>(p->d_I.get());
    int rc;
    if (x.wants_J()) {
        T *Jd[2] = {nullptr, nullptr};
        for (int d = 0; d < 2; d++) {
            if (!r.use_dir[d]) {
                if (x.native && x.J_nat[d]) VRT_HIP_TRY(hipMemsetAsync(x.J_nat[d], 0, r.plane * sizeof(T), st));
                continue;
            }
            if (!x.native && (rc = p->ws_J[d].grow(dcount<T>(r.plane)))) return rc;
            DirWeights dw;
            dw.count = 0;
            for (int a = 0; a < A; a++)
                if ((p->dir_of_active[(size_t)a] > 0) == (d == 0)) {
                    dw.w[dw.count] = x.weights[p->user_of_active[(size_t)a]];
                    dw.idx[dw.count] = a;
                    dw.count++;
                }
            Jd[d] = reinterpret_cast<T *>(J_planes(p, x, d));
            if (r.fused_dir[d]) continue;
            hipLaunchKernelGGL(k_reduce_dir<T>, dim3((unsigned)((r.plane + 255) / 256)), dim3(256), 0, st,
                               (int64_t)r.plane, (int64_t)r.plane, dw, wI, Jd[d]);
        }
        T *dJ = static_cast<T *>(x.J);
        if (x.native) {
// ... 70 lines not shown
```

### voronoirt_amd/csrc/vrt_patch.hip

```cpp
#include <hip/hip_runtime.h>

#include <algorithm>
#include <cmath>
#include <cstdio>
#include <cstdlib>
#include <cstring>
#include <type_traits>

#include "vrt_device.h"
#include "vrt_internal.h"

namespace vrt {

enum : int {
    kDiagNoLevels = 1, kDiagCentreGathers = 2, kDiagNoWeights = 4, kDiagNoStores = 8, kDiagNoGatherI = 16, kDiagNoGatherAlpha = 32,
    kDiagNoGatherS = 64, kDiagNoReduce = 128, kDiagNoWait = 256, kDiagPlainLoadI = 512, kDiagPlainStoreI = 1024, kDiagNoPairLoop = 2048,
    kDiagDirectTable = 4096,
};
__host__ __device__ __forceinline__ constexpr bool diag(int dbg, int flag) { return kDiag && (dbg & flag) != 0; }

struct PatchArgs {
    TileArgs ta;
    int npair;
    int layer;
    int ngrp;
    int nrow;
    int order;
    int prow;
    unsigned row_rcp;
    int nsplit, Q;
    int sbase, srem;
    int lgB;
    int stride;
    int cap;
    int quad;
    int lean;
    int dbg_ent0, dbg_ent_stride, dbg_ent_last;
    int dbg;
    unsigned long long *tl;
    PatchReduce red;
    const int4 *wrec;
    const int32_t *e_pos, *e_u1, *e_u2;
    const uint32_t *e_vis, *e_loc;
    const double *e_w1, *e_w2, *e_r1, *e_r2;
};

__global__ void __launch_bounds__(256)
k_patch_entries(int64_t count, const int32_t *__restrict__ e_pos, const int32_t *__restrict__ t_u1,
                const int32_t *__restrict__ t_u2, const double *__restrict__ t_w1, const double *__restrict__ t_w2,
                const double *__restrict__ t_r1, const double *__restrict__ t_r2, int32_t *__restrict__ e_u1,
                int32_t *__restrict__ e_u2, double *__restrict__ e_w1, double *__restrict__ e_w2,
                double *__restrict__ e_r1, double *__restrict__ e_r2)
{
    const int64_t e = (int64_t)blockIdx.x * blockDim.x + threadIdx.x;
    if (e >= count) return;
    const int p = e_pos[e];
    e_u1[e] = t_u1[p]; e_u2[e] = t_u2[p];
    e_w1[e] = t_w1[p]; e_w2[e] = t_w2[p];
    e_r1[e] = t_r1[p]; e_r2[e] = t_r2[p];
}

int launch_patch_entries(vrt_plan *p, int a, int64_t first, int64_t count)
{
    if (count <= 0) return VRT_OK;
    const size_t o = (size_t)a * (size_t)p->g->n;
    hipLaunchKernelGGL(k_patch_entries, dim3((unsigned)((count + 255) / 256)), dim3(256), 0, p->g->stream, count,
                       p->e_pos + first, p->t_u1 + o, p->t_u2 + o, p->t_w1 + o, p->t_w2 + o, p->t_r1 + o,
                       p->t_r2 + o, p->e_u1 + first, p->e_u2 + first, p->e_w1 + first, p->e_w2 + first,
                       p->e_r1 + first, p->e_r2 + first);
    VRT_HIP_TRY(hipGetLastError());
    return VRT_OK;
}


template <typename T2>
__device__ __forceinline__ double2 ldpair(const T2 *base, int idx, int sh)
{
    const unsigned off = (unsigned)idx << sh;
    return to_d2(*reinterpret_cast<const T2 *>(reinterpret_cast<const char *>(base) + off));
}
template <typename T2> struct Log2Size;
template <> struct Log2Size<double2> { static constexpr int value = 4; };
template <> struct Log2Size<float2> { static constexpr int value = 3; };

static void set_split(PatchArgs &pa, int nblock)
{
    const int nstep = (nblock + pa.Q - 1) / pa.Q;
    pa.sbase = nstep / pa.nsplit;
    pa.srem = nstep - pa.sbase * pa.nsplit;
}
__host__ __device__ __forceinline__ void split_blocks(const PatchArgs &pa, int split, int nblock, int &b0, int &b1)
{
    const int base = pa.sbase, rem = pa.srem;
    const int s0 = split * base + (split < rem ? split : rem), s1 = s0 + base + (split < rem ? 1 : 0);
    b0 = s0 * pa.Q;
    b1 = nblock < s1 * pa.Q ? nblock : s1 * pa.Q;
}

#ifndef VRT_REDUCE_LAST
#define VRT_REDUCE_LAST 1
#endif
struct PatchBlock { int lane, row, split, sib; };
__host__ __device__ __forceinline__ PatchBlock patch_block_of(int order, int nrow, unsigned row_rcp, int lgS, unsigned bx, unsigned y)
{
    PatchBlock b;
    const int grp = (int)(bx >> 3);
    b.lane = (int)(bx & 7u);
    if (order == 0) {
        b.row = (int)y;
        b.split = grp >> lgS;
        b.sib = grp & ((1 << lgS) - 1);
    } else {
        b.split = (int)(((unsigned long long)(2u * y) * row_rcp) >> 32);
        b.row = (int)y - b.split * nrow;
        b.sib = grp;
    }
    return b;
}
struct PatchGrid {
    int order = 0, prow = 0;
    unsigned row_rcp = 0;
    int64_t gx = 0, gy = 0;
};
static PatchGrid patch_grid(int order, int nrow, int nsplit, int lgS, int64_t nred)
{
    PatchGrid g;
    if (order == 1 && nsplit >= 2 && nrow >= 1) {
        g.gx = (int64_t)8 << lgS;
        g.prow = nsplit * nrow;
        g.gy = (int64_t)nsplit * nrow + (nred + g.gx - 1) / g.gx;
        if (g.gy <= 65535) {
            g.order = 1;
            g.row_rcp = (unsigned)((((uint64_t)1 << 31) + (uint64_t)nrow - 1) / (uint64_t)nrow);
            return g;
        }
    }
    g.order = 0;
    g.prow = nrow;
    g.row_rcp = 0;
    g.gx = (int64_t)8 * ((int64_t)nsplit << lgS);
    if (nrow == 0) g.gx = std::max<int64_t>(g.gx, ((nred + 65534) / 65535 + 7) / 8 * 8);
    g.gy = nrow + (nred + g.gx - 1) / g.gx;
    return g;
}
__device__ __forceinline__ int reduce_block_index(const PatchArgs &pa)
{
    const int rows = (int)gridDim.y - pa.prow;
    const int y = VRT_REDUCE_LAST ? (int)blockIdx.y - pa.prow : ((int)blockIdx.y < rows ? (int)blockIdx.y : -1);
    return y < 0 ? -1 : y * (int)gridDim.x + (int)blockIdx.x;
}
__device__ __forceinline__ PatchBlock patch_block(const PatchArgs &pa, int lgS)
{
    const int y = VRT_REDUCE_LAST ? (int)blockIdx.y : (int)blockIdx.y - ((int)gridDim.y - pa.prow);
    return patch_block_of(pa.order, pa.nrow, pa.row_rcp, lgS, blockIdx.x, (unsigned)y);
}
__device__ __forceinline__ int patch_row(const PatchArgs &pa) { return patch_block(pa, 0).row; }
struct BlockStamp {
    unsigned long long *slot = nullptr;
    unsigned long long t0 = 0, share = 0;
    __device__ __forceinline__ explicit BlockStamp(const PatchArgs &pa)
    {
        if (kDiag && pa.tl) {
            slot = pa.tl + 3 * ((size_t)blockIdx.y * gridDim.x + blockIdx.x);
            t0 = wall_clock64();
        }
    }
    __device__ __forceinline__ void steps(const PatchArgs &pa, int b0, int b1)
    {
        if (kDiag) share = (unsigned long long)((b1 - b0 + pa.Q - 1) / pa.Q);
    }
    __device__ __forceinline__ void reduces()
    {
        if (kDiag) share = 1ull << 32;
    }
    __device__ __forceinline__ ~BlockStamp()
    {
        if (kDiag && slot && threadIdx.x == 0) {
            slot[0] = t0;
            slot[1] = wall_clock64();
            slot[2] = share;
        }
    }
};
template <typename T, int NT>
__device__ __forceinline__ void patch_reduce_role(const PatchArgs &pa)
{
    typedef typename Pair<T>::type T2;
    const TileArgs &ta = pa.ta;
    const int tid = threadIdx.x;
    int b = reduce_block_index(pa), r = 0;
    if (b >= pa.red.nblk[0]) { b -= pa.red.nblk[0]; r = 1; }
    if (b >= pa.red.nblk[r]) return;
    if (diag(pa.dbg, kDiagNoReduce)) return;
    const int len = pa.red.hi[r] - pa.red.lo[r];
    const int per = NT * pa.red.ppb;
    const int nblock = pair_block_count(pa.npair, pa.lgB);
    int k0 = 0, lw = 0;
    for (int k = 0; k < nblock; k++) {
        pair_block_of(k, pa.npair, pa.lgB, k0, lw);
        const int cnt = (int)((((int64_t)len << lw) + per - 1) / per);
        if (b < cnt) break;
        b -= cnt;
    }
    const int64_t nn = ta.n;
    const size_t run = (size_t)len << lw;
    const size_t base = (size_t)k0 * (size_t)nn + ((size_t)pa.red.lo[r] << lw);
    T2 *Jd = reinterpret_cast<T2 *>(pa.red.Jd[r]);
    const T2 *I0 = reinterpret_cast<const T2 *>(ta.I);
    const size_t plane = (size_t)pa.npair * (size_t)nn;
    if (pa.red.ppb == 4) {
        const size_t f0 = (size_t)b * 4 * NT + tid;
        const unsigned left = f0 < run ? (unsigned)min((size_t)(run - f0 + NT - 1) / NT, (size_t)4) : 0u;
        const size_t e0 = base + (left ? f0 : 0);
        double ax[4], ay[4];
#pragma unroll
        for (int i = 0; i < 4; i++) { ax[i] = 0.0; ay[i] = 0.0; }
        for (int j = 0; j < pa.red.count[r]; j++) {
            const int a = pa.red.angles[r][j];
            const T2 *Ia = I0 + (size_t)a * plane + e0;
            double2 v[4];
#pragma unroll
            for (int i = 0; i < 4; i++) v[i] = to_d2(Ia[(unsigned)i < left ? i * NT : 0]);
#pragma unroll
            for (int i = 0; i < 4; i++) {
                ax[i] += pa.red.w[a] * v[i].x;
                ay[i] += pa.red.w[a] * v[i].y;
            }
        }
#pragma unroll
        for (int i = 0; i < 4; i++)
            if ((unsigned)i < left) Jd[e0 + (size_t)i * NT] = from_d2<T>(make_double2(ax[i], ay[i]));
        return;
    }
    for (int i = 0; i < pa.red.ppb; i++) {
        const size_t f = ((size_t)b * pa.red.ppb + i) * NT + tid;
        if (f >= run) break;
        const size_t e = base + f;
        double ax = 0.0, ay = 0.0;
        for (int j = 0; j < pa.red.count[r]; j++) {
            const int a = pa.red.angles[r][j];
            const double2 v = to_d2(I0[(size_t)a * plane + e]);
            ax += pa.red.w[a] * v.x;
            ay += pa.red.w[a] * v.y;
        }
        Jd[e] = from_d2<T>(make_double2(ax, ay));
    }
}

#ifdef VRT_PATCH_WPE
#define VRT_WPE_ATTR __attribute__((amdgpu_waves_per_eu(VRT_PATCH_WPE, VRT_PATCH_WPE)))
#else
#define VRT_WPE_ATTR
#endif
template <typename T, int AM, int K, int Q, int NT>
__global__ void __launch_bounds__(NT) VRT_WPE_ATTR
k_patch_solve(PatchArgs pa)
{
    typedef typename Pair<T>::type T2;
    extern __shared__ __attribute__((aligned(16))) double2 ptile[];
    const TileArgs &ta = pa.ta;
    const int tid = threadIdx.x;
    BlockStamp stamp(pa);
    if (reduce_block_index(pa) >= 0) {
        stamp.reduces();
        patch_reduce_role<T, NT>(pa);
        return;
    }
    const PatchBlock blk = patch_block(pa, pa.lgB);
    const int x = blk.lane, sj = blk.row;
    const int4 rec = pa.wrec[2 * (sj * 8 + x)], rec2 = pa.wrec[2 * (sj * 8 + x) + 1];
    if (rec.y <= 0) return;
    const int sib = blk.sib;
    const int nblock = pair_block_count(pa.npair, pa.lgB);
    int b0, b1;
    split_blocks(pa, blk.split, nblock, b0, b1);
    if (b0 >= b1) return;
    {
        int k0, lw;
        pair_block_of(b0, pa.npair, pa.lgB, k0, lw);
        if (sib >= (1 << lw)) return;
    }
    stamp.steps(pa, b0, b1);
    const int ent_off = rec.x, n_ent = rec.y, own_lo = rec.z, own_cnt = rec.w;
    const int dbg = kDiag ? pa.dbg : 0;
    const int nlev = diag(dbg, kDiagNoLevels) ? 0 : rec2.x, a = rec2.y & 0xFFFF;
    const int d = rec2.y >> 16;
    const int lo = rec2.z, hi = rec2.w;
    const int64_t n = ta.n;
    const int stride = pa.stride;

    double *s_w1 = reinterpret_cast<double *>(ptile + Q * stride);
    double *s_w2 = s_w1 + pa.cap, *s_r1 = s_w2 + pa.cap, *s_r2 = s_r1 + pa.cap;
    int *s_pos = reinterpret_cast<int *>(s_r2 + pa.cap);
    int *s_u1 = s_pos + pa.cap, *s_u2 = s_u1 + pa.cap;
    uint32_t *s_vis = reinterpret_cast<uint32_t *>(s_u2 + pa.cap), *s_loc = s_vis + pa.cap;
#pragma unroll
    for (int k = 0; k < K; k++) {
        const int i = tid + k * NT;
        const bool ok = i < n_ent;
        const int e = ent_off + (ok ? i : n_ent - 1);
        s_pos[i] = pa.e_pos[e];
        s_u1[i] = pa.e_u1[e];
        s_u2[i] = pa.e_u2[e];
        s_vis[i] = ok ? pa.e_vis[e] : 0u;
        const uint32_t lc = pa.e_loc[e], l1 = lc & 0xFFFFu, l2 = lc >> 16;
        s_loc[i] = (l1 == 0xFFFFu ? (uint32_t)n_ent : l1) | ((l2 == 0xFFFFu ? (uint32_t)n_ent : l2) << 16);
        s_w1[i] = pa.e_w1[e]; s_w2[i] = pa.e_w2[e]; s_r1[i] = pa.e_r1[e]; s_r2[i] = pa.e_r2[e];
    }
    if (tid == 0) {
#pragma unroll
        for (int qi = 0; qi < Q; qi++) ptile[qi * stride + n_ent] = make_double2(0.0, 0.0);
    }
    exp2_table_fill();
    __syncthreads();
    constexpr int lgT2 = Log2Size<T2>::value;
    for (int bk = b0; bk < b1; bk += Q) {
        size_t qbase[Q];
        int qsh[Q];
        bool qok[Q];
#pragma unroll
        for (int qi = 0; qi < Q; qi++) {
            int k0, lw;
            pair_block_of(min(bk + qi, b1 - 1), pa.npair, pa.lgB, k0, lw);
            qok[qi] = bk + qi < b1 && sib < (1 << lw);
            if (!qok[qi] && qi > 0) { qbase[qi] = qbase[qi - 1]; qsh[qi] = qsh[qi - 1]; continue; }
            qbase[qi] = (size_t)k0 * (size_t)n + (size_t)sib;
            qsh[qi] = lw + lgT2;
        }
        if (!qok[0]) break;
        double2 c[K][Q], g1[K][Q], g2[K][Q];
#pragma unroll
        for (int k = 0; k < K; k++) {
            const int i = tid + k * NT;
            const int p = s_pos[i];
            int v1 = s_u1[i], v2 = s_u2[i];
            if (diag(dbg, kDiagCentreGathers)) { v1 = p; v2 = p; }
            int i1 = v1 < lo ? v1 : (int)n - 1, i2 = v2 < lo ? v2 : (int)n - 1;
            if (diag(dbg, kDiagNoGatherI)) { i1 = (int)n - 1; i2 = (int)n - 1; }
            const int av1 = diag(dbg, kDiagNoGatherAlpha) ? p : v1, av2 = diag(dbg, kDiagNoGatherAlpha) ? p : v2;
            const int sv1 = diag(dbg, kDiagNoGatherS) ? p : v1, sv2 = diag(dbg, kDiagNoGatherS) ? p : v2;
            const bool in1 = (v1 >= lo) & (v1 < hi), in2 = (v2 >= lo) & (v2 < hi);
#pragma unroll
            for (int qi = 0; qi < Q; qi++) {
                const int sh = qsh[qi];
                const T2 *__restrict__ S = reinterpret_cast<const T2 *>(ta.S[d]) + qbase[qi];
                const T2 *__restrict__ I = reinterpret_cast<const T2 *>(ta.I) + (size_t)a * pa.npair * (size_t)n + qbase[qi];
                double2 a_c, a_1, a_2;
                if constexpr (AM == VRT_ALPHA_SITE) {
                    const T *__restrict__ Al = reinterpret_cast<const T *>(ta.alpha[d]);
                    const double c0 = Al[p], c1 = Al[av1], c2 = Al[av2];
                    (void)sh;
                    a_c = make_double2(c0, c0); a_1 = make_double2(c1, c1); a_2 = make_double2(c2, c2);
                } else {
                    const T2 *__restrict__ Al =
                        AM == VRT_ALPHA_SITE_LAM
                            ? reinterpret_cast<const T2 *>(ta.alpha[d]) + qbase[qi]
                            : reinterpret_cast<const T2 *>(ta.alpha_angle) + (size_t)a * pa.npair * (size_t)n + qbase[qi];
                    a_c = ldpair(Al, p, sh); a_1 = ldpair(Al, av1, sh); a_2 = ldpair(Al, av2, sh);
                }
                const double2 S_c = ldpair(S, p, sh), S_1 = ldpair(S, sv1, sh), S_2 = ldpair(S, sv2, sh);
                const double2 I_1 = ldpair(I, i1, sh), I_2 = ldpair(I, i2, sh);
                const double w1 = s_w1[i], w2 = s_w2[i], r1 = s_r1[i], r2 = s_r2[i];
                const double wg1 = in1 ? w1 : 0.0, wg2 = in2 ? w2 : 0.0;
                const double rh1 = 0.5 * r1, rh2 = 0.5 * r2;
                if (diag(dbg, kDiagNoWeights)) {
                    c[k][qi] = make_double2(a_c.x + S_c.x + I_1.x + a_1.x + S_1.x, a_c.y + S_c.y + I_2.y + a_2.y + S_2.y);
                    g1[k][qi] = make_double2(w1, w2); g2[k][qi] = make_double2(r1, r2);
                    continue;
                }
                entry_lambda(rh1, rh2, w1, w2, wg1, wg2, a_c.x, a_1.x, a_2.x, S_c.x, S_1.x, S_2.x, I_1.x, I_2.x,
                             c[k][qi].x, g1[k][qi].x, g2[k][qi].x);
                entry_lambda(rh1, rh2, w1, w2, wg1, wg2, a_c.y, a_1.y, a_2.y, S_c.y, S_1.y, S_2.y, I_1.y, I_2.y,
                             c[k][qi].y, g1[k][qi].y, g2[k][qi].y);
            }
        }
        uint32_t vis[K], loc[K];
#pragma unroll
        for (int k = 0; k < K; k++) {
            vis[k] = s_vis[tid + k * NT];
            loc[k] = s_loc[tid + k * NT];
            if (tid + k * NT < n_ent) {
#pragma unroll
                for (int qi = 0; qi < Q; qi++) ptile[qi * stride + tid + k * NT] = make_double2(0.0, 0.0);
            }
        }
        __syncthreads();
        for (int t = 1; t <= nlev; t++) {
#pragma unroll
            for (int k = 0; k < K; k++) {
                if ((vis[k] & 0xFFu) == (uint32_t)t) {
                    const uint32_t l1 = loc[k] & 0xFFFFu, l2 = loc[k] >> 16;
#pragma unroll
                    for (int qi = 0; qi < Q; qi++) {
                        const double2 xv = ptile[qi * stride + l1], yv = ptile[qi * stride + l2];
                        double2 r;
                        r.x = fma(g2[k][qi].x, yv.x, fma(g1[k][qi].x, xv.x, c[k][qi].x));
                        r.y = fma(g2[k][qi].y, yv.y, fma(g1[k][qi].y, xv.y, c[k][qi].y));
                        ptile[qi * stride + tid + k * NT] = r;
                    }
                    vis[k] >>= 8;
                }
            }
            __syncthreads();
        }
#pragma unroll
        for (int k = 0; k < K; k++) {
            const int i = tid + k * NT;
            if (i < own_cnt) {
#pragma unroll
                for (int qi = 0; qi < Q; qi++) {
                    if (qok[qi] && !(diag(dbg, kDiagNoStores) && ptile[qi * stride + i].x != 1.2345e300)) {
                        T2 *I = reinterpret_cast<T2 *>(ta.I) + (size_t)a * pa.npair * (size_t)n + qbase[qi];
                        const unsigned off = (unsigned)(own_lo + i) << qsh[qi];
                        *reinterpret_cast<T2 *>(reinterpret_cast<char *>(I) + off) = from_d2<T>(ptile[qi * stride + i]);
                    }
                }
            }
        }
    }
}


typedef int vrt_i32x8 __attribute__((ext_vector_type(8)));
typedef const __attribute__((address_space(4))) vrt_i32x8 WorkRec;
static_assert(2 * sizeof(int4) == 32 && sizeof(vrt_i32x8) == 32, "a work-list slot is two int4: 32 bytes, 32-byte aligned");
struct PatchItem {
    int sib, b0, b1;
    int ent_off, n_ent, own_lo, own_cnt, nlev, a, d, lo, hi;
};
__device__ __forceinline__ bool patch_item(const PatchArgs &pa, int lgS, PatchItem &it)
{
    const PatchBlock blk = patch_block(pa, lgS);
    const int x = blk.lane, sj = blk.row;
    const vrt_i32x8 r8 = *((const WorkRec *)(uintptr_t)pa.wrec + (sj * 8 + x));
    const int4 rec = make_int4(r8[0], r8[1], r8[2], r8[3]), rec2 = make_int4(r8[4], r8[5], r8[6], r8[7]);
    if (rec.y <= 0) return false;
    it.sib = blk.sib;
    split_blocks(pa, blk.split, pair_block_count(pa.npair, pa.lgB), it.b0, it.b1);
    if (it.b0 >= it.b1) return false;
    it.ent_off = rec.x; it.n_ent = rec.y; it.own_lo = rec.z; it.own_cnt = rec.w;
    it.nlev = rec2.x; it.a = rec2.y & 0xFFFF;
    it.d = rec2.y >> 16;
    it.lo = rec2.z;
    it.hi = rec2.w;
    return true;
}
template <int CAP>
struct EntryTable {
    double *w1, *w2, *r1, *r2;
    int *pos, *u1, *u2;
    uint32_t *vis, *loc;
    __device__ __forceinline__ EntryTable(double2 *tiles, int planes)
    {
        w1 = reinterpret_cast<double *>(tiles + planes * (CAP + 1));
        w2 = w1 + CAP; r1 = w2 + CAP; r2 = r1 + CAP;
        pos = reinterpret_cast<int *>(r2 + CAP);
        u1 = pos + CAP; u2 = u1 + CAP;
        vis = reinterpret_cast<uint32_t *>(u2 + CAP);
        loc = vis + CAP;
    }
    struct Regs {
        int p0, a1, a2;
        uint32_t vs, lc;
        double x1, x2, y1, y2;
    };
    template <typename Tables>
    static __device__ __forceinline__ Regs load(const Tables &pa, int e)
    {
        Regs r;
        r.p0 = pa.e_pos[e]; r.a1 = pa.e_u1[e]; r.a2 = pa.e_u2[e];
        r.vs = pa.e_vis[e]; r.lc = pa.e_loc[e];
        r.x1 = pa.e_w1[e]; r.x2 = pa.e_w2[e]; r.y1 = pa.e_r1[e]; r.y2 = pa.e_r2[e];
        return r;
    }
    __device__ __forceinline__ void store(const Regs &r, const PatchItem &it, int tid) const
    {
        pos[tid] = r.p0;
        u1[tid] = r.a1;
        u2[tid] = r.a2;
        vis[tid] = tid < it.n_ent ? r.vs : 0u;
        const uint32_t l1 = r.lc & 0xFFFFu, l2 = r.lc >> 16;
        loc[tid] = (l1 == 0xFFFFu ? (uint32_t)it.n_ent : l1) | ((l2 == 0xFFFFu ? (uint32_t)it.n_ent : l2) << 16);
        w1[tid] = r.x1; w2[tid] = r.x2; r1[tid] = r.y1; r2[tid] = r.y2;
    }
    template <typename Tables>
    __device__ __forceinline__ void park(const Tables &pa, const PatchItem &it, int tid) const
    {
        store(load(pa, it.ent_off + (tid < it.n_ent ? tid : it.n_ent - 1)), it, tid);
    }
};

struct PairIO {
    int n;
    int npair, lgB, dbg;
    const void *S;
    const void *alpha;
    void *I;
};
template <int AM>
__device__ __forceinline__ PairIO pair_io(const PatchArgs &pa, int d)
{
    PairIO io;
    io.n = (int)pa.ta.n; io.npair = pa.npair; io.lgB = pa.lgB; io.dbg = kDiag ? pa.dbg : 0;
    io.S = pa.ta.S[d];
    io.alpha = AM == VRT_ALPHA_ANGLE_SITE_LAM ? (const void *)pa.ta.alpha_angle : (const void *)pa.ta.alpha[d];
// ... 252 lines not shown
                }
                const __amdgpu_buffer_rsrc_t rsI = plane_rsrc(Ia + qb, n << sh);
                if (diag(dbg, kDiagPlainLoadI)) {
                    rI_1 = at(Ia + qb, (unsigned)i1 << sh);
                    rI_2 = at(Ia + qb, (unsigned)i2 << sh);
                } else {
                    rI_1 = BufSc1<T2>::load(rsI, (unsigned)i1 << sh);
                    rI_2 = BufSc1<T2>::load(rsI, (unsigned)i2 << sh);
                }
                if constexpr (CHAIN == 2) {
                    const bool in1 = (v1 >= it.lo) & (v1 < it.hi), in2 = (v2 >= it.lo) & (v2 < it.hi);
                    if (!diag(dbg, kDiagNoWeights)) {
                        LateTerms Lx, Ly;
                        late_lambda(d1x, d2x, (double)rS_1.x, (double)rS_2.x, Lx, d1y);
                        double sink = 0.0;
                        late_lambda(d1y, d2y, (double)rS_1.y, (double)rS_2.y, Ly, sink);
                        if (!diag(dbg, kDiagNoWait)) chain_data_wait<T2>(rsI, (unsigned)i1 << sh, (unsigned)i2 << sh, rI_1, rI_2, s_dep);
                        late_apply(Lx, tab.w1 + tid, tab.w2 + tid, in1, in2, (double)rS_c.x, (double)rI_1.x, (double)rI_2.x, c.x, g1.x, g2.x);
                        late_apply(Ly, tab.w1 + tid, tab.w2 + tid, in1, in2, (double)rS_c.y, (double)rI_1.y, (double)rI_2.y, c.y, g1.y, g2.y);
                    } else {
                        if (!diag(dbg, kDiagNoWait)) chain_data_wait<T2>(rsI, (unsigned)i1 << sh, (unsigned)i2 << sh, rI_1, rI_2, s_dep);
                        c = make_double2(d1x + (double)rS_c.x + (double)rS_1.x + (double)rI_1.x, d2y + (double)rS_c.y + (double)rS_2.y + (double)rI_2.y);
                        g1 = make_double2(in1 ? d2x : 0.0, in1 ? d1y : 0.0);
                        g2 = make_double2(in2 ? d1x : 0.0, in2 ? d2y : 0.0);
                    }
                }
            } else {
                rI_1 = at(Ia + qb, (unsigned)i1 << sh);
                rI_2 = at(Ia + qb, (unsigned)i2 << sh);
            }
            const bool in1 = (v1 >= it.lo) & (v1 < it.hi), in2 = (v2 >= it.lo) & (v2 < it.hi);
            if constexpr (CHAIN == 2) {
            } else if (diag(dbg, kDiagNoWeights)) {
                c = make_double2(d1x + (double)rS_c.x + (double)rS_1.x + (double)rI_1.x, d2y + (double)rS_c.y + (double)rS_2.y + (double)rI_2.y);
                g1 = make_double2(in1 ? d2x : 0.0, in1 ? d1y : 0.0);
                g2 = make_double2(in2 ? d1x : 0.0, in2 ? d2y : 0.0);
            } else {
                entry_lambda_seq(d1x, d2x, tab.w1 + tid, tab.w2 + tid, in1, in2, (double)rS_c.x, (double)rS_1.x, (double)rS_2.x,
                                 (double)rI_1.x, (double)rI_2.x, c.x, g1.x, g2.x, d1y);
                double sink = 0.0;
                entry_lambda_seq(d1y, d2y, tab.w1 + tid, tab.w2 + tid, in1, in2, (double)rS_c.y, (double)rS_1.y, (double)rS_2.y,
                                 (double)rI_1.y, (double)rI_2.y, c.y, g1.y, g2.y, sink);
            }
        }
        uint32_t vis = tab.vis[tid];
        const uint32_t loc = tab.loc[tid];
        {
            double z;
            asm volatile("v_mov_b64 %0, 0" : "=v"(z));
            if (tid < it.n_ent) ptile[tid] = make_double2(z, z);
        }
        if constexpr (CHAIN == 1) asm volatile("s_waitcnt vmcnt(0)" ::: "memory");
        __syncthreads();
        if constexpr (CHAIN == 1) {
            if (bk > it.b0 && tid == 0) chain_publish(s_dep, bk - it.b0);
        }
        const int nlev = diag(dbg, kDiagNoLevels) ? 0 : it.nlev;
        __builtin_amdgcn_s_setprio(VRT_LEVEL_PRIO);
        for (int t = 1; t <= nlev; t++) {
            if ((vis & 0xFFu) == (uint32_t)t) {
                const double2 xv = ptile[loc & 0xFFFFu], yv = ptile[loc >> 16];
                double2 r;
                r.x = fma(g2.x, yv.x, fma(g1.x, xv.x, c.x));
                r.y = fma(g2.y, yv.y, fma(g1.y, xv.y, c.y));
                ptile[tid] = r;
                vis >>= 8;
            }
            __syncthreads();
        }
        __builtin_amdgcn_s_setprio(0);
        if (tid < it.own_cnt && !(diag(dbg, kDiagNoStores) && ptile[tid].x != 1.2345e300)) {
            if (CHAIN && !diag(dbg, kDiagPlainStoreI)) {
                const __amdgpu_buffer_rsrc_t rsI = plane_rsrc(Ia + qb, n << sh);
                BufSc1<T2>::store(rsI, (unsigned)(it.own_lo + tid) << sh, from_d2<T>(ptile[tid]));
            } else {
                T2 *I = reinterpret_cast<T2 *>(pa.I) + (size_t)it.a * pa.npair * (size_t)n + qb;
                *reinterpret_cast<T2 *>(reinterpret_cast<char *>(I) + ((unsigned)(it.own_lo + tid) << sh)) = from_d2<T>(ptile[tid]);
            }
        }
        __syncthreads();
    }
}

template <typename T, int AM, int NT>
__global__ void __launch_bounds__(NT) VRT_LEAN_ATTR
k_patch_lean(PatchArgs pa)
{
    extern __shared__ __attribute__((aligned(16))) double2 ptile[];
    const int tid = threadIdx.x;
    BlockStamp stamp(pa);
    if (reduce_block_index(pa) >= 0) {
        stamp.reduces();
        patch_reduce_role<T, NT>(pa);
        return;
    }
    const double e2 = exp2_table_load();
    typename EntryTable<NT>::Regs early{};
    if (diag(pa.dbg, kDiagDirectTable))
        early = EntryTable<NT>::load(pa, min(pa.dbg_ent0 + (patch_row(pa) * 8 + ((int)blockIdx.x & 7)) * pa.dbg_ent_stride + tid, pa.dbg_ent_last));
    PatchItem it;
    if (!patch_item(pa, pa.lgB, it)) return;
    stamp.steps(pa, it.b0, it.b1);
    if (diag(pa.dbg, kDiagNoPairLoop)) it.b1 = it.b0;
    const EntryTable<NT> tab(ptile, 1);
    if (tid == 0) ptile[it.n_ent] = make_double2(0.0, 0.0);
    if (diag(pa.dbg, kDiagDirectTable)) tab.store(early, it, tid);
    else tab.park(pa, it, tid);
    exp2_table_store(e2);
    __syncthreads();
    lean_pairs<T, AM, NT, 0>(pair_io<AM>(pa, it.d), it, tab, ptile);
}


template <int AM, int NT, bool CHAIN>
__device__ __forceinline__ void quad_pairs(const PairIO &pa, const PatchItem &it, const EntryTable<NT> &tab,
                                           double2 *ptile)
{
    const int tid = threadIdx.x;
    const int sib2 = it.sib, b0 = it.b0, b1 = it.b1;
    const unsigned n = (unsigned)pa.n;
    const int n_ent = it.n_ent, own_lo = it.own_lo, own_cnt = it.own_cnt, nlev = it.nlev, a = it.a;
    const int lo = it.lo, hi = it.hi;
    constexpr int CAP = NT;
    double2 *tileA = ptile, *tileB = ptile + (CAP + 1);
    double *const s_r1 = tab.r1, *const s_r2 = tab.r2, *const s_w1 = tab.w1, *const s_w2 = tab.w2;
    int *const s_pos = tab.pos, *const s_u1 = tab.u1, *const s_u2 = tab.u2;
    uint32_t *const s_vis = tab.vis, *const s_loc = tab.loc;
    const float2 *Sd = reinterpret_cast<const float2 *>(pa.S);
    const float2 *Ia = reinterpret_cast<const float2 *>(pa.I) + (size_t)a * pa.npair * (size_t)n;
    auto at4 = [](const float2 *base, unsigned off) { return *reinterpret_cast<const float4 *>(reinterpret_cast<const char *>(base) + off); };
    const int32_t *s_dep = chain_dep_slots(tab);
    for (int bk = b0; bk < b1; bk++) {
        int k0, lw;
        if constexpr (CHAIN) { k0 = 2 * bk; lw = 1; }
        else {
            pair_block_of(bk, pa.npair, pa.lgB, k0, lw);
            if (2 * sib2 >= (1 << lw)) break;
        }
        const size_t qb = (size_t)k0 * (size_t)n + (size_t)(CHAIN ? 0 : 2 * sib2);
        const int sh = lw + 3;
        uint32_t seen = 0;
        if constexpr (CHAIN) seen = chain_peek(s_dep, bk - b0 + 1);
        const int p = s_pos[tid], v1 = s_u1[tid], v2 = s_u2[tid];
        double d1x, d2x, d1y, d2y, d1z, d2z, d1w, d2w;
        {
            float4 a_c, a_1, a_2;
            if constexpr (AM == VRT_ALPHA_SITE) {
                const float *__restrict__ A1 = reinterpret_cast<const float *>(pa.alpha);
                const float c0 = A1[p], c1 = A1[v1], c2 = A1[v2];
                a_c = make_float4(c0, c0, c0, c0); a_1 = make_float4(c1, c1, c1, c1); a_2 = make_float4(c2, c2, c2, c2);
            } else {
                const float2 *Al = AM == VRT_ALPHA_SITE_LAM ? reinterpret_cast<const float2 *>(pa.alpha) + qb
                                                            : reinterpret_cast<const float2 *>(pa.alpha) + (size_t)a * pa.npair * (size_t)n + qb;
                a_c = at4(Al, (unsigned)p << sh); a_1 = at4(Al, (unsigned)v1 << sh); a_2 = at4(Al, (unsigned)v2 << sh);
            }
            const double rh1 = 0.5 * s_r1[tid], rh2 = 0.5 * s_r2[tid];
            d1x = rh1 * ((double)a_c.x + (double)a_1.x); d2x = rh2 * ((double)a_c.x + (double)a_2.x);
            d1y = rh1 * ((double)a_c.y + (double)a_1.y); d2y = rh2 * ((double)a_c.y + (double)a_2.y);
            d1z = rh1 * ((double)a_c.z + (double)a_1.z); d2z = rh2 * ((double)a_c.z + (double)a_2.z);
            d1w = rh1 * ((double)a_c.w + (double)a_1.w); d2w = rh2 * ((double)a_c.w + (double)a_2.w);
        }
        asm volatile("" : "+v"(d1x), "+v"(d2x), "+v"(d1y), "+v"(d2y), "+v"(d1z), "+v"(d2z), "+v"(d1w), "+v"(d2w) : : "memory");
        double2 cA, g1A, g2A, cB, g1B, g2B;
        {
            const int i1 = v1 < lo ? v1 : (int)n - 1, i2 = v2 < lo ? v2 : (int)n - 1;
            const bool in1 = (v1 >= lo) & (v1 < hi), in2 = (v2 >= lo) & (v2 < hi);
            const float4 S_c = at4(Sd + qb, (unsigned)p << sh), S_1 = at4(Sd + qb, (unsigned)v1 << sh), S_2 = at4(Sd + qb, (unsigned)v2 << sh);
            float4 I_1, I_2;
            if constexpr (CHAIN) {
                chain_wait(s_dep, bk - b0 + 1, seen);
                const __amdgpu_buffer_rsrc_t rsI = plane_rsrc(Ia + qb, n << sh);
                I_1 = BufSc1<float4>::load(rsI, (unsigned)i1 << sh);
                I_2 = BufSc1<float4>::load(rsI, (unsigned)i2 << sh);
            } else {
                I_1 = at4(Ia + qb, (unsigned)i1 << sh);
                I_2 = at4(Ia + qb, (unsigned)i2 << sh);
            }
            entry_lambda_seq(d1x, d2x, s_w1 + tid, s_w2 + tid, in1, in2, (double)S_c.x, (double)S_1.x, (double)S_2.x,
                             (double)I_1.x, (double)I_2.x, cA.x, g1A.x, g2A.x, d1y);
            entry_lambda_seq(d1y, d2y, s_w1 + tid, s_w2 + tid, in1, in2, (double)S_c.y, (double)S_1.y, (double)S_2.y,
                             (double)I_1.y, (double)I_2.y, cA.y, g1A.y, g2A.y, d1z);
            entry_lambda_seq(d1z, d2z, s_w1 + tid, s_w2 + tid, in1, in2, (double)S_c.z, (double)S_1.z, (double)S_2.z,
                             (double)I_1.z, (double)I_2.z, cB.x, g1B.x, g2B.x, d1w);
            double sink = 0.0;
            entry_lambda_seq(d1w, d2w, s_w1 + tid, s_w2 + tid, in1, in2, (double)S_c.w, (double)S_1.w, (double)S_2.w,
                             (double)I_1.w, (double)I_2.w, cB.y, g1B.y, g2B.y, sink);
        }
        uint32_t vis = s_vis[tid];
        const uint32_t loc = s_loc[tid];
        {
            double z;
            asm volatile("v_mov_b64 %0, 0" : "=v"(z));
            if (tid < n_ent) {
                tileA[tid] = make_double2(z, z);
                tileB[tid] = make_double2(z, z);
            }
        }
        if constexpr (CHAIN) asm volatile("s_waitcnt vmcnt(0)" ::: "memory");
        __syncthreads();
        if constexpr (CHAIN) {
            if (bk > b0 && tid == 0) chain_publish(s_dep, bk - b0);
        }
        for (int t = 1; t <= nlev; t++) {
            if ((vis & 0xFFu) == (uint32_t)t) {
                const uint32_t l1 = loc & 0xFFFFu, l2 = loc >> 16;
                const double2 xa = tileA[l1], ya = tileA[l2], xb = tileB[l1], yb = tileB[l2];
                double2 ra, rb;
                ra.x = fma(g2A.x, ya.x, fma(g1A.x, xa.x, cA.x));
                ra.y = fma(g2A.y, ya.y, fma(g1A.y, xa.y, cA.y));
                rb.x = fma(g2B.x, yb.x, fma(g1B.x, xb.x, cB.x));
                rb.y = fma(g2B.y, yb.y, fma(g1B.y, xb.y, cB.y));
                tileA[tid] = ra;
                tileB[tid] = rb;
                vis >>= 8;
            }
            __syncthreads();
        }
        if (tid < own_cnt) {
            const double2 ra = tileA[tid], rb = tileB[tid];
            const float4 out = make_float4((float)ra.x, (float)ra.y, (float)rb.x, (float)rb.y);
            if constexpr (CHAIN) {
                const __amdgpu_buffer_rsrc_t rsI = plane_rsrc(Ia + qb, n << sh);
                BufSc1<float4>::store(rsI, (unsigned)(own_lo + tid) << sh, out);
            } else {
                float2 *I = reinterpret_cast<float2 *>(pa.I) + (size_t)a * pa.npair * (size_t)n + qb;
                *reinterpret_cast<float4 *>(reinterpret_cast<char *>(I) + ((unsigned)(own_lo + tid) << sh)) = out;
            }
        }
        __syncthreads();
    }
}

#ifndef VRT_QUAD_ATTR
#define VRT_QUAD_ATTR __attribute__((amdgpu_waves_per_eu(6, 6)))
#endif
template <int AM, int NT>
__global__ void __launch_bounds__(NT) VRT_QUAD_ATTR
k_patch_quad(PatchArgs pa)
{
    extern __shared__ __attribute__((aligned(16))) double2 ptile[];
    const int tid = threadIdx.x;
    BlockStamp stamp(pa);
    if (reduce_block_index(pa) >= 0) {
        stamp.reduces();
        patch_reduce_role<float, NT>(pa);
        return;
    }
    const double e2 = exp2_table_load();
    PatchItem it;
    if (!patch_item(pa, pa.lgB - 1, it)) return;
    stamp.steps(pa, it.b0, it.b1);
    const EntryTable<NT> tab(ptile, 2);
    if (tid == 0) {
        ptile[it.n_ent] = make_double2(0.0, 0.0);
        ptile[NT + 1 + it.n_ent] = make_double2(0.0, 0.0);
    }
    tab.park(pa, it, tid);
    exp2_table_store(e2);
    __syncthreads();
    quad_pairs<AM, NT, false>(pair_io<AM>(pa, it.d), it, tab, ptile);
}


struct ChainDev {
    TileArgs ta;
    int npair, nsplit, cap;
    const int32_t *e_pos, *e_u1, *e_u2;
    const uint32_t *e_vis, *e_loc;
    const double *e_w1, *e_w2, *e_r1, *e_r2;
    PatchReduce red;
    const int4 *items;
    int q_off[9];
    const int32_t *deps;
    uint32_t *progress;
    uint32_t *ctrl;
    uint32_t *host_status;
    int64_t n_patches;
    uint32_t spin_limit;
    int static_items;
    int dbg;
};

__device__ __forceinline__ const uint32_t *chain_abort_word(const uint32_t *cd_words)
{
    return reinterpret_cast<const ChainDev *>(cd_words)->ctrl + kChainAbortWord;
}

__device__ __forceinline__ int cd_int(const int *p) { return __builtin_amdgcn_readfirstlane(*p); }
template <typename P>
__device__ __forceinline__ P *cd_ptr(P *const *p) { return uniform_ptr(*p); }

__device__ __forceinline__ void chain_wait_slow(const int32_t *s_dep, int step)
{
    const int lane = (int)(threadIdx.x & 63u);
    const uint32_t *ctl = reinterpret_cast<const uint32_t *>(s_dep - kCtlWords);
    const ChainDev *cd = reinterpret_cast<const ChainDev *>(((uint64_t)ctl[kCtlArgsHi] << 32) | (uint64_t)ctl[kCtlArgsLo]);
    uint32_t *abort_word = cd->ctrl + kChainAbortWord;
    const uint32_t *progress = chain_progress(ctl);
    const uint32_t target = ctl[kCtlBase] + (uint32_t)step, limit = cd->spin_limit;
    const int ndep = (int)ctl[kCtlNdep];
    for (int c0 = 0; c0 < ndep; c0 += 64) {
        const int j = c0 + lane;
        const int dep = j < 64 + kChainDepLds ? s_dep[j] : (j < ndep ? (cd->deps + ctl[kCtlDepOff])[j] : (int)ctl[kCtlSelf]);
        const uint32_t *w = progress + dep;
        uint32_t spins = 0;
        for (;;) {
            const uint32_t v = ld_agent(w);
            if (__all(j >= ndep || (int)(v - target) >= 0)) break;
            __builtin_amdgcn_s_sleep(8);
            if ((++spins & 127u) == 1u) {
                if (spins > limit) {
                    st_agent(abort_word, 1u);
                    uint32_t *hs = cd->host_status;
                    __hip_atomic_store(hs + 1, ctl[kCtlItem], __ATOMIC_RELAXED, __HIP_MEMORY_SCOPE_SYSTEM);
                    __hip_atomic_store(hs, 1u, __ATOMIC_RELAXED, __HIP_MEMORY_SCOPE_SYSTEM);
                }
                if (ld_agent(abort_word) != 0u) return;
            }
        }
    }
}

__device__ __forceinline__ void chain_data_give_up_cd(const ChainDev *cd, uint32_t item)
{
    st_agent(cd->ctrl + kChainAbortWord, 1u);
    uint32_t *hs = cd->host_status;
    __hip_atomic_store(hs + 1, item, __ATOMIC_RELAXED, __HIP_MEMORY_SCOPE_SYSTEM);
    __hip_atomic_store(hs, 1u, __ATOMIC_RELAXED, __HIP_MEMORY_SCOPE_SYSTEM);
}

template <typename T, int NT, int LGB, int MODE>
__device__ __forceinline__ void chain_reduce(const ChainDev &cd, const ChainDev *cdp, uint32_t item, int r, int lo, int hi, int b0, int b1)
{
    typedef typename Pair<T>::type T2;
    const int tid = threadIdx.x;
    if (diag(cd.dbg, kDiagNoReduce)) return;
    const int64_t nn = cd.ta.n;
    const int npair = cd.npair;
    const size_t plane = (size_t)npair * (size_t)nn;
    T2 *Jd = reinterpret_cast<T2 *>(cd.red.Jd[r]);
    const T2 *I0 = reinterpret_cast<const T2 *>(cd.ta.I);
    const int count = cd.red.count[r];
    constexpr int lgT2 = Log2Size<T2>::value;
// ... 79 lines not shown
    {
        const int nblock = npair >> LGB, nsplit = ca.nsplit;
        const int per = nblock / nsplit, rem = nblock - per * nsplit;
        b0 = split * per + (split < rem ? split : rem);
        b1 = b0 + per + (split < rem ? 1 : 0);
    }
    if (tid == 0) {
        const uint64_t prog = (uint64_t)(ca.progress + (size_t)split * (size_t)ca.n_patches);
        s_ctl[kCtlSelf] = (uint32_t)Bz;
        s_ctl[kCtlNdep] = (uint32_t)By;
        s_ctl[kCtlDepOff] = (uint32_t)Bx;
        s_ctl[kCtlProgLo] = (uint32_t)prog;
        s_ctl[kCtlProgHi] = (uint32_t)(prog >> 32);
        s_ctl[kCtlBase] = base;
    }
    if (Az >> 31) {
        if constexpr (MODE == 1) {
            __syncthreads();
            chain_wait(s_dep, Bw, chain_peek(s_dep, Bw));
        }
        chain_reduce<T, NT, LGB, MODE>(ca, cd, (uint32_t)idx, d, Ax, Ay, b0, b1);
        return;
    }
    PatchItem it;
    it.sib = 0; it.b0 = b0; it.b1 = b1;
    it.ent_off = Ax; it.own_lo = Ay;
    it.n_ent = (int)(Az & 0x3FFu); it.own_cnt = (int)((Az >> 10) & 0x3FFu); it.nlev = (int)((Az >> 20) & 0xFFu);
    it.a = (int)(Aw & 63u); it.d = d;
    it.lo = __builtin_amdgcn_readfirstlane(C4.x);
    it.hi = __builtin_amdgcn_readfirstlane(C4.y);
    PairIO pa;
    pa.n = (int)ca.ta.n;
    pa.npair = npair;
    pa.lgB = LGB;
    pa.dbg = kDiag ? ca.dbg : 0;
    pa.S = ca.ta.S[d];
    pa.I = ca.ta.I;
    pa.alpha = AM == VRT_ALPHA_ANGLE_SITE_LAM ? (const void *)ca.ta.alpha_angle : (const void *)ca.ta.alpha[d];
    tab.park(ca, it, tid);
    if (tid == 0) {
        ptile[it.n_ent] = make_double2(0.0, 0.0);
        if (QUAD) ptile[NT + 1 + it.n_ent] = make_double2(0.0, 0.0);
    }
    __syncthreads();
    if (diag(ca.dbg, kDiagNoPairLoop)) it.b1 = it.b0;
    if constexpr (QUAD) quad_pairs<AM, NT, true>(pa, it, tab, ptile);
    else lean_pairs<T, AM, NT, MODE>(pa, it, tab, ptile);
    if constexpr (MODE == 2) {
        __syncthreads();
        if (tid == 0 && s_ctl[kCtlGaveUp]) chain_data_give_up_cd(cd, (uint32_t)idx);
    }
    if constexpr (MODE == 1) {
        asm volatile("s_waitcnt vmcnt(0)" ::: "memory");
        __syncthreads();
        if (tid == 0) chain_publish(s_dep, b1 - b0);
    }
}

template <typename T, int AM, int NT>
__global__ void __launch_bounds__(NT) VRT_LEAN_ATTR
k_patch_chain(ChainDev ca, const ChainDev *cd, uint32_t base)
{
    extern __shared__ __attribute__((aligned(16))) double2 ptile[];
    chain_item<T, AM, NT, false, 1>(ca, cd, base, ptile);
}
template <typename T, int AM, int NT>
__global__ void __launch_bounds__(NT) __attribute__((amdgpu_waves_per_eu(6, 6)))
k_patch_chain_df(ChainDev ca, const ChainDev *cd, uint32_t base)
{
    extern __shared__ __attribute__((aligned(16))) double2 ptile[];
    chain_item<T, AM, NT, false, 2>(ca, cd, base, ptile);
}
template <int AM, int NT>
__global__ void __launch_bounds__(NT) VRT_QUAD_ATTR
k_patch_chain_quad(ChainDev ca, const ChainDev *cd, uint32_t base)
{
    extern __shared__ __attribute__((aligned(16))) double2 ptile[];
    chain_item<float, AM, NT, true, 1>(ca, cd, base, ptile);
}

#define VRT_PATCH_SHAPES(X) \
    X(1, 1, 256) X(1, 1, 512) X(1, 1, 1024) X(2, 1, 256) X(2, 1, 512) X(1, 2, 256) X(1, 2, 512) X(1, 2, 1024) X(2, 2, 512)

template <typename T, int AM>
static int launch_shape(int K, int Q, int NT, dim3 grid, size_t lds, hipStream_t st, const PatchArgs &pa)
{
    if constexpr (sizeof(T) == 4) {
        if (pa.quad) {
            switch (NT) {
            case 256: hipLaunchKernelGGL((k_patch_quad<AM, 256>), grid, dim3(256), lds, st, pa); return VRT_OK;
            case 512: hipLaunchKernelGGL((k_patch_quad<AM, 512>), grid, dim3(512), lds, st, pa); return VRT_OK;
            case 1024: hipLaunchKernelGGL((k_patch_quad<AM, 1024>), grid, dim3(1024), lds, st, pa); return VRT_OK;
            default: break;
            }
        }
    }
    if (pa.lean && K == 1 && Q == 1) {
        switch (NT) {
        case 256: hipLaunchKernelGGL((k_patch_lean<T, AM, 256>), grid, dim3(256), lds, st, pa); return VRT_OK;
        case 512: hipLaunchKernelGGL((k_patch_lean<T, AM, 512>), grid, dim3(512), lds, st, pa); return VRT_OK;
        case 1024: hipLaunchKernelGGL((k_patch_lean<T, AM, 1024>), grid, dim3(1024), lds, st, pa); return VRT_OK;
        default: break;
        }
    }
#define VRT_PATCH_CASE(k, q, nt) \
    if (K == k && Q == q && NT == nt) { hipLaunchKernelGGL((k_patch_solve<T, AM, k, q, nt>), grid, dim3(nt), lds, st, pa); return VRT_OK; }
    VRT_PATCH_SHAPES(VRT_PATCH_CASE)
#undef VRT_PATCH_CASE
    return fail(VRT_EINVAL, "no patch kernel for this (entries per thread, pairs, threads) shape");
}

template <typename T>
static int launch_mode(int am, int K, int Q, int NT, dim3 grid, size_t lds, hipStream_t st, const PatchArgs &pa)
{
    switch (am) {
    case VRT_ALPHA_SITE: return launch_shape<T, VRT_ALPHA_SITE>(K, Q, NT, grid, lds, st, pa);
    case VRT_ALPHA_SITE_LAM: return launch_shape<T, VRT_ALPHA_SITE_LAM>(K, Q, NT, grid, lds, st, pa);
    default: return launch_shape<T, VRT_ALPHA_ANGLE_SITE_LAM>(K, Q, NT, grid, lds, st, pa);
    }
}

bool patch_shape_exists(int K, int Q, int NT)
{
#define VRT_PATCH_CASE(k, q, nt) if (K == k && Q == q && NT == nt) return true;
    VRT_PATCH_SHAPES(VRT_PATCH_CASE)
#undef VRT_PATCH_CASE
    return false;
}

static PatchIndex patch_index(const vrt_plan *p)
{
    return PatchIndex{p->h_patch_first, p->h_patch_rec, p->h_patch_rec2, p->h_patch_dep_off, p->h_patch_deps, p->dir_of_active,
                      {&p->g->up.reduced, &p->g->down.reduced}, p->tile_max_layers, p->g->n};
}

int ensure_patch_work(vrt_plan *p, int G, const std::vector<int32_t> &group_angles, const std::vector<int> &group_off)
{
    if (p->d_patch_work && p->patch_work_groups == G) return VRT_OK;
    p->d_patch_work.reset();
    std::vector<int4> work;
    build_patch_work(patch_index(p), G, group_angles, group_off, work, p->patch_work_off, p->patch_work_padding);
    if (int rc = p->d_patch_work.alloc(work.size())) return rc;
    VRT_HIP_TRY(hipMemcpy(p->d_patch_work, work.data(), sizeof(int4) * work.size(), hipMemcpyHostToDevice));
    p->patch_work_groups = G;
    return VRT_OK;
}

static void size_reduce(PatchReduce &red, int npair, int lgB, int NT)
{
    red.nred = 0;
    int64_t total = 0;
    for (int r = 0; r < 2; r++)
        if (red.count[r] > 0 && red.Jd[r]) total += (int64_t)std::max(0, red.hi[r] - red.lo[r]) * npair;
    red.ppb = total <= (int64_t)NT * 1024 ? 1 : 4;
    const int64_t per = (int64_t)NT * red.ppb;
    const int nblock = pair_block_count(npair, lgB);
    for (int r = 0; r < 2; r++) {
        const int64_t len = red.hi[r] - red.lo[r];
        red.nblk[r] = 0;
        if (len > 0 && red.count[r] > 0 && red.Jd[r])
            for (int k = 0; k < nblock; k++) {
                int k0, lw;
                pair_block_of(k, npair, lgB, k0, lw);
                red.nblk[r] += (int)(((len << lw) + per - 1) / per);
            }
        red.nred += red.nblk[r];
    }
    red.nred = (red.nred + 7) / 8 * 8;
}

int launch_patch_layer(vrt_plan *p, const TileArgs &ta, int npair, int layer, int group, const PatchShape &shape, hipStream_t st,
                       bool f32, const PatchReduce *reduce)
{
    const int Q = shape.Q, lgS = shape.lgS;
    const int target_wgs = p->tune.patch_target;
    const int maxL = p->tile_max_layers;
    const size_t wo = (size_t)group * (size_t)(maxL + 2) + (size_t)layer;
    const int64_t w0 = (layer >= 2 && layer <= maxL) ? p->patch_work_off[wo] : 0, w1 = (layer >= 2 && layer <= maxL) ? p->patch_work_off[wo + 1] : 0;
    PatchArgs pa;
    if (reduce) {
        pa.red = *reduce;
        size_reduce(pa.red, npair, shape.lgB, p->patch_NT);
    }
    if (w1 <= w0 && pa.red.nred == 0) return VRT_OK;
    pa.ta = ta;
    pa.npair = npair;
    pa.layer = layer;
    pa.lgB = shape.lgB;
    pa.quad = shape.quad;
    pa.lean = shape.lean;
    pa.Q = Q;
    pa.nsplit = 1;
    pa.ngrp = 1 << lgS;
    if (w1 > w0) {
        const int64_t items = (w1 - w0) << lgS;
        const int nblock = pair_block_count(npair, pa.lgB);
        const int steps_all = (nblock + Q - 1) / Q;
        int nsplit;
        if (p->tune.patch_split > 0) nsplit = std::min(steps_all, p->tune.patch_split);
        else if (target_wgs > 0) nsplit = (int)std::max<int64_t>(1, std::min<int64_t>(steps_all, (target_wgs + items - 1) / items));
        else {
            const double T = std::min(900.0, 460.0 + 4100.0 / (double)steps_all);
            const int s_min = (int)std::min<int64_t>(steps_all, std::max<int64_t>(1, (512 + items - 1) / items));
            double dmin = 1e300;
            for (int c = steps_all; c >= 1; c--) {
                const int sc = (steps_all + c - 1) / c;
                if (sc >= s_min) dmin = std::min(dmin, std::fabs(std::log((double)items * sc / T)));
            }
            nsplit = s_min;
            for (int c = steps_all; c >= 1; c--) {
                const int sc = (steps_all + c - 1) / c;
                if (sc >= s_min && std::fabs(std::log((double)items * sc / T)) <= dmin + 0.03) nsplit = sc;
            }
        }
        pa.nsplit = nsplit;
        pa.ngrp = nsplit << lgS;
    }
    pa.stride = p->patch_cap + 1;
    pa.cap = p->patch_cap;
    pa.dbg = kDiag ? p->tune.debug_flags : 0;
    {
        const int64_t slots = std::max<int64_t>(1, p->patch_work_off.back());
        pa.dbg_ent_stride = (int)std::max<int64_t>(1, p->n_patch_entries / slots);
        pa.dbg_ent0 = (int)(w0 * pa.dbg_ent_stride);
        pa.dbg_ent_last = (int)std::max<int64_t>(0, p->n_patch_entries - 1);
    }
    pa.wrec = p->d_patch_work + 2 * w0;
    pa.e_pos = p->e_pos; pa.e_u1 = p->e_u1; pa.e_u2 = p->e_u2;
    pa.e_vis = p->e_vis; pa.e_loc = p->e_loc;
    pa.e_w1 = p->e_w1; pa.e_w2 = p->e_w2; pa.e_r1 = p->e_r1; pa.e_r2 = p->e_r2;
    pa.nrow = (int)((w1 - w0) / 8);
    const PatchGrid pg = patch_grid(p->tune.patch_order, pa.nrow, pa.nsplit, lgS, pa.red.nred);
    pa.order = pg.order;
    pa.prow = pg.prow;
    pa.row_rcp = pg.row_rcp;
    set_split(pa, pair_block_count(npair, pa.lgB));
    const int64_t gx = pg.gx, gy = pg.gy;
    if (gy > 65535 || gx > INT32_MAX)
        return fail(VRT_EINVAL, "a layer of this size needs more than 65535 rows of patch and reduction blocks in one launch");
    pa.tl = nullptr;
    if (kDiag && p->tune.patch_timeline) {
        const int64_t cap = (int64_t)1 << 20, blocks = gx * gy;
        if (!p->d_patch_tl && p->d_patch_tl.alloc((size_t)(3 * cap)) != VRT_OK) return VRT_ENOMEM;
        if (p->patch_tl_blocks + blocks <= cap) {
            pa.tl = p->d_patch_tl + 3 * p->patch_tl_blocks;
            const int64_t rec[kPatchTimelineRec] = {layer, group, gx, gy, pa.nrow, pa.nsplit, lgS, pa.order, pa.prow, pa.red.nred,
                                                    p->patch_tl_blocks, (pair_block_count(npair, pa.lgB) + Q - 1) / Q};
            p->patch_tl_launches.insert(p->patch_tl_launches.end(), rec, rec + kPatchTimelineRec);
            p->patch_tl_blocks += blocks;
        }
    }
    const dim3 grid((unsigned)gx, (unsigned)gy);
    const size_t lds = (size_t)(pa.quad ? 2 : Q) * (size_t)pa.stride * sizeof(double2) + (size_t)pa.cap * (4 * sizeof(double) + 5 * sizeof(int32_t));
    const int rc = f32 ? launch_mode<float>(ta.alpha_mode, p->patch_K, Q, p->patch_NT, grid, lds, st, pa)
                       : launch_mode<double>(ta.alpha_mode, p->patch_K, Q, p->patch_NT, grid, lds, st, pa);
    return rc;
}

void patch_timeline_begin(vrt_plan *p)
{
    p->patch_tl_launches.clear();
    p->patch_tl_blocks = 0;
}

int patch_timeline_read(vrt_plan *p, int64_t cap_launches, int64_t cap_blocks, int64_t *launches, uint64_t *stamps, int64_t *counts)
{
    if (!kDiag) return fail(VRT_EINVAL, "the timeline of the patch launches exists in the -DVRT_DIAG build only");
    const int64_t nl = (int64_t)p->patch_tl_launches.size() / kPatchTimelineRec, nb = p->patch_tl_blocks;
    if (nl > cap_launches || nb > cap_blocks) return fail(VRT_EINVAL, "timeline buffers too small");
    VRT_HIP_TRY(hipDeviceSynchronize());
    int khz = 0;
    VRT_HIP_TRY(hipDeviceGetAttribute(&khz, hipDeviceAttributeWallClockRate, p->device));
    counts[0] = nl; counts[1] = nb; counts[2] = khz;
    std::copy(p->patch_tl_launches.begin(), p->patch_tl_launches.end(), launches);
    if (nb > 0) VRT_HIP_TRY(hipMemcpy(stamps, p->d_patch_tl, sizeof(uint64_t) * 3 * (size_t)nb, hipMemcpyDeviceToHost));
    return VRT_OK;
}

int patch_dispatch_map(int order, int nrow, int nsplit, int lg_siblings, int64_t nred, int steps, int64_t *dims, int32_t *blocks)
{
    if (!dims) return fail(VRT_EINVAL, "NULL output");
    if (order < 0 || order > 1 || nrow < 0 || nrow > 65535 || nsplit < 1 || nsplit > 4096 || lg_siblings < 0 || lg_siblings > 4 ||
        nred < 0 || nred > INT32_MAX || steps < nsplit)
        return fail(VRT_EINVAL, "dispatch map: argument out of range");
    const PatchGrid pg = patch_grid(order, nrow, nsplit, lg_siblings, nred);
    if (pg.gy > 65535) return fail(VRT_EINVAL, "more than 65535 rows of patch and reduction blocks");
    dims[0] = pg.gx; dims[1] = pg.gy; dims[2] = pg.order; dims[3] = pg.prow;
    if (!blocks) return VRT_OK;
    PatchArgs sp;
    sp.nsplit = nsplit;
    sp.Q = 1;
    set_split(sp, steps);
    for (int64_t by = 0; by < pg.gy; by++)
        for (int64_t bx = 0; bx < pg.gx; bx++) {
            int32_t *o = blocks + 6 * (by * pg.gx + bx);
            std::fill(o, o + 6, 0);
            if (by >= pg.prow) {
                o[0] = 1;
                o[1] = (int32_t)((by - pg.prow) * pg.gx + bx);
                continue;
            }
            const PatchBlock b = patch_block_of(pg.order, nrow, pg.row_rcp, lg_siblings, (unsigned)bx, (unsigned)by);
            int b0, b1;
            split_blocks(sp, b.split, steps, b0, b1);
            o[1] = b.lane; o[2] = b.row; o[3] = b.split; o[4] = b.sib; o[5] = b1 - b0;
        }
    return VRT_OK;
}

static int chain_nsplit(const vrt_plan *p, int nblock)
{
    const int per = std::max(1, p->tune.chain_pairs);
    const double per_layer = (double)p->n_patches / (double)std::max(1, p->tile_max_layers);
    const int fill = (int)std::ceil(1024.0 / std::max(1.0, per_layer));
    return std::max(1, std::min({std::max((nblock + per - 1) / per, fill), nblock, 511}));
}

template <typename T, int AM>
static int launch_chain_mode(bool quad, bool dataflag, int64_t items, size_t lds, hipStream_t st, const ChainDev &h, const ChainDev *cd, uint32_t base)
{
    constexpr int NT = 512;
    if constexpr (sizeof(T) == 8) {
        if (dataflag) {
            hipLaunchKernelGGL((k_patch_chain_df<T, AM, NT>), dim3((unsigned)items), dim3(NT), lds, st, h, cd, base);
            return VRT_OK;
        }
    }
    if constexpr (sizeof(T) == 4) {
        if (quad) {
            hipLaunchKernelGGL((k_patch_chain_quad<AM, NT>), dim3((unsigned)items), dim3(NT), lds, st, h, cd, base);
            return VRT_OK;
        }
    }
    hipLaunchKernelGGL((k_patch_chain<T, AM, NT>), dim3((unsigned)items), dim3(NT), lds, st, h, cd, base);
    return VRT_OK;
}

int chain_ctrl_words() { return kChainAbortWord + 4; }

int launch_patch_chain(vrt_plan *p, const TileArgs &ta, int npair, const PatchShape &shape, hipStream_t st, bool f32,
                       const PatchReduce *reduce, bool ctrl_zeroed)
{
    if (int rc0 = patch_chain_check(p)) return rc0;
    const bool quad = shape.quad != 0, dataflag = shape.chain_dataflag;
    const int nsplit = chain_nsplit(p, pair_block_count(npair, shape.lgB));
    ChainLaunch &cl = p->chain;
    int rc = cl.select(npair, shape.lgB, nsplit, reduce != nullptr, [&](ChainItems &cs) -> int {
        if ((int64_t)nsplit * p->n_patches >= ((int64_t)1 << 31)) return fail(VRT_EINVAL, "too many (split, patch) progress words");
        std::vector<int4> items;
        std::vector<int32_t> deps;
        int rcb;
        if ((rcb = build_chain_items(patch_index(p), pair_block_count(npair, shape.lgB), nsplit, reduce != nullptr, items, deps, cs))) return rcb;
        if ((rcb = cs.items.alloc(items.size())) || (rcb = cs.deps.alloc(deps.size()))) return rcb;
        VRT_HIP_TRY(hipMemcpy(cs.items, items.data(), sizeof(int4) * items.size(), hipMemcpyHostToDevice));
        VRT_HIP_TRY(hipMemcpy(cs.deps, deps.data(), sizeof(int32_t) * deps.size(), hipMemcpyHostToDevice));
        return VRT_OK;
    });
    if (rc) return rc;
    const size_t words = (size_t)nsplit * (size_t)std::max<int64_t>(p->n_patches, 1);
    if (words > cl.progress.cap) {
        if ((rc = cl.progress.grow(words))) return rc;
        cl.progress_fresh = true;
    }
    if (!cl.ctrl && (rc = cl.ctrl.alloc(kChainAbortWord + 4))) return rc;
    if (!cl.h_status) {
        if ((rc = cl.h_status.alloc(16, hipHostMallocMapped))) return rc;
        *cl.h_status = 0;
        VRT_HIP_TRY(hipHostGetDevicePointer((void **)&cl.d_status, cl.h_status.p, 0));
    }
    const ChainItems &set = cl.sets.front();
    if (set.q_off[8] == 0) return VRT_OK;
    static_assert(std::is_trivially_copyable<ChainDev>::value, "ChainDev is uploaded byte for byte");
    ChainDev h;
    std::memset(&h, 0, sizeof(h));
    h.ta = ta;
    h.npair = npair;
    h.nsplit = nsplit;
    h.cap = p->patch_cap;
    h.e_pos = p->e_pos; h.e_u1 = p->e_u1; h.e_u2 = p->e_u2;
    h.e_vis = p->e_vis; h.e_loc = p->e_loc;
    h.e_w1 = p->e_w1; h.e_w2 = p->e_w2; h.e_r1 = p->e_r1; h.e_r2 = p->e_r2;
    if (reduce) h.red = *reduce;
    h.items = set.items;
    for (int x = 0; x <= 8; x++) h.q_off[x] = set.q_off[x];
    h.deps = set.deps;
    h.progress = cl.progress;
    h.ctrl = cl.ctrl;
    h.host_status = cl.d_status;
    h.n_patches = p->n_patches;
// ... 61 lines not shown
```

Measured before the change: 91.41 billion.

## Fold layer reduction work into patch-solve blocks and speed up reduce-block indexing

Adds an optional mode where the angle-weighted J reduction, previously run by extra reduction rows in the patch launch, is instead carried by the patch-solve blocks themselves. Each block issues its first chunk of intensity loads before solving and finishes the sums afterwards, so the reduction overlaps with the solve and the grid loses its reduction rows. It also replaces the linear pair-block scan in the reduce role with a reciprocal-multiply division. The ride mode is gated by a tuning option that defaults to off, so by default only the faster reduce-block indexing changes. Enabling ride mode raises register pressure in the solve kernels.

```diff
diff --git a/include/voronoirt.h b/include/voronoirt.h
--- a/include/voronoirt.h
+++ b/include/voronoirt.h
@@ -142,6 +142,9 @@
 int vrt_plan_last_sweep_timing(const vrt_plan *p, double *ms, int64_t *launches);
 int vrt_plan_patch_layout(const vrt_plan *p, int64_t *out);
 int vrt_patch_dispatch_map(int order, int nrow, int nsplit, int lg_siblings, int64_t nred, int steps, int64_t *dims, int32_t *blocks);
+int vrt_patch_ride_map(int order, int nrow, int nsplit, int lg_siblings, int npair, int lg_block, int NT, int64_t n, const int32_t *lo,
+                       const int32_t *hi, int64_t first_block, int64_t nblocks, int64_t *dims, int64_t *elems);
+int vrt_plan_patch_ride_stats(const vrt_plan *p, int64_t *out);
 int vrt_plan_patch_timeline(vrt_plan *p, int64_t cap_launches, int64_t cap_blocks, int64_t *launches, uint64_t *stamps, int64_t *counts);
 int vrt_plan_check(vrt_plan *p);
 int vrt_plan_last_path(const vrt_plan *p);
diff --git a/voronoirt_amd/_lib.py b/voronoirt_amd/_lib.py
--- a/voronoirt_amd/_lib.py
+++ b/voronoirt_amd/_lib.py
@@ -134,6 +134,8 @@
     "vrt_plan_last_sweep_timing": (ctypes.c_int, [vp, p_dbl, p_i64]),
     "vrt_plan_patch_layout": (ctypes.c_int, [vp, p_i64]),
     "vrt_patch_dispatch_map": (ctypes.c_int, [ctypes.c_int, ctypes.c_int, ctypes.c_int, ctypes.c_int, c_i64, ctypes.c_int, p_i64, p_i32]),
+    "vrt_plan_patch_ride_stats": (ctypes.c_int, [ctypes.c_void_p, p_i64]),
+    "vrt_patch_ride_map": (ctypes.c_int, [ctypes.c_int] * 7 + [c_i64, p_i32, p_i32, c_i64, c_i64, p_i64, p_i64]),
     "vrt_plan_patch_timeline": (ctypes.c_int, [vp, c_i64, c_i64, p_i64, ctypes.POINTER(ctypes.c_uint64), p_i64]),
     "vrt_plan_last_path": (ctypes.c_int, [vp]),
     "vrt_plan_set_option": (ctypes.c_int, [vp, ctypes.c_char_p, ctypes.c_char_p]),
diff --git a/voronoirt_amd/api.py b/voronoirt_amd/api.py
--- a/voronoirt_amd/api.py
+++ b/voronoirt_amd/api.py
@@ -353,6 +353,12 @@
         out = (ctypes.c_int64 * 4)()
         check(_lib.load().vrt_plan_patch_layout(self._h, out))
         return {"patches": out[0], "fewest_per_angle_layer": out[1], "work_slots": out[2], "padding_slots": out[3]}
+
+    @property
+    def patch_ride_stats(self) -> dict:
+        out = (ctypes.c_int64 * 2)()
+        check(_lib.load().vrt_plan_patch_ride_stats(self._h, out))
+        return {"launches": int(out[0]), "max_chunks": int(out[1])}
 
     @property
     def last_launches(self) -> int:
diff --git a/voronoirt_amd/csrc/vrt_api.cpp b/voronoirt_amd/csrc/vrt_api.cpp
--- a/voronoirt_amd/csrc/vrt_api.cpp
+++ b/voronoirt_amd/csrc/vrt_api.cpp
@@ -53,7 +53,7 @@
     static const char *names[] = {"VRT_PATH", "VRT_STEP_K", "VRT_STEP_SINGLE", "VRT_STEP_PAIRS", "VRT_STEP_XCD",
                                   "VRT_STEP_STREAMS", "VRT_STEP_LEVEL_MAP", "VRT_STEP_GROUP_DIR", "VRT_TILE_WIDE",
                                   "VRT_TILE_PRE", "VRT_PATCH_K", "VRT_PATCH_NT", "VRT_PATCH_OWN",
-                                  "VRT_PATCH_Q", "VRT_PATCH_TARGET", "VRT_PATCH_SPLIT", "VRT_PATCH_ORDER", "VRT_PATCH_TIMELINE", "VRT_PAIR_BLOCK", "VRT_PATCH_QUAD", "VRT_PATCH_LEAN", "VRT_PATCH_CHAIN", "VRT_CHAIN_PAIRS", "VRT_CHAIN_SPIN", "VRT_CHAIN_DATAFLAG", "VRT_CHAIN_STATIC", "VRT_LAMBDA_NATIVE", "VRT_DEBUG_FLAGS", "VRT_DEBUG_SKIP_LEVELS",
+                                  "VRT_PATCH_Q", "VRT_PATCH_TARGET", "VRT_PATCH_SPLIT", "VRT_PATCH_ORDER", "VRT_PATCH_REDUCE_RIDE", "VRT_PATCH_TIMELINE", "VRT_PAIR_BLOCK", "VRT_PATCH_QUAD", "VRT_PATCH_LEAN", "VRT_PATCH_CHAIN", "VRT_CHAIN_PAIRS", "VRT_CHAIN_SPIN", "VRT_CHAIN_DATAFLAG", "VRT_CHAIN_STATIC", "VRT_LAMBDA_NATIVE", "VRT_DEBUG_FLAGS", "VRT_DEBUG_SKIP_LEVELS",
                                   "VRT_TILE_DEBUG"};
     for (const char *nm : names) {
         const char *e = std::getenv(nm);
@@ -92,6 +92,7 @@
         {"VRT_PATCH_K", &t.patch_K, 1, 8, true}, {"VRT_PATCH_NT", &t.patch_NT, 64, 1024, true},
         {"VRT_PATCH_OWN", &t.patch_own, 0, 65535, true}, {"VRT_PATCH_Q", &t.patch_Q, 1, 4, false},
         {"VRT_PATCH_TARGET", &t.patch_target, 0, 1 << 20, false}, {"VRT_PATCH_SPLIT", &t.patch_split, 0, 4096, false}, {"VRT_PATCH_ORDER", &t.patch_order, 0, 1, false},
+        {"VRT_PATCH_REDUCE_RIDE", &t.patch_reduce_ride, 0, 1, false},
         {"VRT_PATCH_TIMELINE", &t.patch_timeline, 0, 1, false}, {"VRT_PAIR_BLOCK", &t.pair_block, 1, 16, true},
         {"VRT_PATCH_QUAD", &t.patch_quad, 0, 1, true}, {"VRT_PATCH_LEAN", &t.patch_lean, 0, 1, false},
         {"VRT_PATCH_CHAIN", &t.patch_chain, 0, 2, false}, {"VRT_CHAIN_PAIRS", &t.chain_pairs, 1, 256, false},
@@ -1327,6 +1328,20 @@
     return guarded([&] { return patch_dispatch_map(order, nrow, nsplit, lg_siblings, nred, steps, dims, blocks); });
 }
 
+int vrt_patch_ride_map(int order, int nrow, int nsplit, int lg_siblings, int npair, int lg_block, int NT, int64_t n, const int32_t *lo,
+                       const int32_t *hi, int64_t first_block, int64_t nblocks, int64_t *dims, int64_t *elems)
+{
+    return guarded([&] { return patch_ride_map(order, nrow, nsplit, lg_siblings, npair, lg_block, NT, n, lo, hi, first_block, nblocks, dims, elems); });
+}
+
+int vrt_plan_patch_ride_stats(const vrt_plan *p, int64_t *out)
+{
+    if (!p || !out) return fail(VRT_EINVAL, "NULL plan or output");
+    out[0] = p->patch_rode_launches;
+    out[1] = p->patch_rode_chunks;
+    return VRT_OK;
+}
+
 int vrt_plan_patch_timeline(vrt_plan *p, int64_t cap_launches, int64_t cap_blocks, int64_t *launches, uint64_t *stamps, int64_t *counts)
 {
     if (!p || !launches || !stamps || !counts) return fail(VRT_EINVAL, "NULL plan or output");
diff --git a/voronoirt_amd/csrc/vrt_device.h b/voronoirt_amd/csrc/vrt_device.h
--- a/voronoirt_amd/csrc/vrt_device.h
+++ b/voronoirt_amd/csrc/vrt_device.h
@@ -185,6 +185,12 @@
     double w[kMaxAngles];
     int32_t angles[2][kMaxAngles];
 };
+struct PatchRide {
+    int on = 0;
+    unsigned blocks = 0;
+    unsigned chunks[2] = {0, 0};
+    unsigned rcp[2] = {0, 0};
+};
 
 
 }
diff --git a/voronoirt_amd/csrc/vrt_internal.h b/voronoirt_amd/csrc/vrt_internal.h
--- a/voronoirt_amd/csrc/vrt_internal.h
+++ b/voronoirt_amd/csrc/vrt_internal.h
@@ -277,6 +277,7 @@
     int patch_split = 0;
     int patch_target = 0;
     int patch_order = 1;
+    int patch_reduce_ride = 0;
     int patch_timeline = 0;
     int chain_static = 1;
     int lambda_native = 1;
@@ -482,6 +483,7 @@
     vrt::DevBuf<unsigned long long> d_patch_tl;
     std::vector<int64_t> patch_tl_launches;
     int64_t patch_tl_blocks = 0;
+    int64_t patch_rode_launches = 0, patch_rode_chunks = 0;
     vrt::Stream step_stream[4];
     vrt::Event step_fork, step_join[4];
     int last_path = 0;
@@ -675,6 +677,8 @@
 void patch_timeline_begin(vrt_plan *p);
 int patch_timeline_read(vrt_plan *p, int64_t cap_launches, int64_t cap_blocks, int64_t *launches, uint64_t *stamps, int64_t *counts);
 int patch_dispatch_map(int order, int nrow, int nsplit, int lg_siblings, int64_t nred, int steps, int64_t *dims, int32_t *blocks);
+int patch_ride_map(int order, int nrow, int nsplit, int lg_siblings, int npair, int lg_block, int NT, int64_t n, const int32_t *lo,
+                   const int32_t *hi, int64_t first_block, int64_t nblocks, int64_t *dims, int64_t *elems);
 int launch_patch_chain(vrt_plan *p, const TileArgs &ta, int npair, const PatchShape &shape, hipStream_t st, bool f32,
                        const PatchReduce *reduce, bool ctrl_zeroed = false);
 int chain_ctrl_words();
diff --git a/voronoirt_amd/csrc/vrt_layers.hip b/voronoirt_amd/csrc/vrt_layers.hip
--- a/voronoirt_amd/csrc/vrt_layers.hip
+++ b/voronoirt_amd/csrc/vrt_layers.hip
@@ -686,6 +686,7 @@
     if ((rc = fork_streams(p, st, G))) return rc;
     r.launches = 0;
     if (kDiag) patch_timeline_begin(p);
+    p->patch_rode_launches = p->patch_rode_chunks = 0;
     for (int layer = 2; layer <= Lmax; layer++)
         for (int gi = 0; gi < G; gi++) {
             hipStream_t sg = gi == 0 ? st : p->step_stream[gi];
diff --git a/voronoirt_amd/csrc/vrt_patch.hip b/voronoirt_amd/csrc/vrt_patch.hip
--- a/voronoirt_amd/csrc/vrt_patch.hip
+++ b/voronoirt_amd/csrc/vrt_patch.hip
@@ -43,6 +43,8 @@
     const int32_t *e_pos, *e_u1, *e_u2;
     const uint32_t *e_vis, *e_loc;
     const double *e_w1, *e_w2, *e_r1, *e_r2;
+    unsigned rows_rcp[2] = {0, 0};
+    PatchRide ride;
 };
 
 __global__ void __launch_bounds__(256)
@@ -143,6 +145,66 @@
     g.gy = nrow + (nred + g.gx - 1) / g.gx;
     return g;
 }
+__host__ __device__ __forceinline__ unsigned rcp32_of(unsigned len)
+{
+    return len <= 1u ? 0xFFFFFFFFu : (unsigned)(((unsigned long long)1 << 32) / len);
+}
+__host__ __device__ __forceinline__ unsigned div_by_rcp(unsigned f, unsigned len, unsigned rcp)
+{
+    unsigned t = (unsigned)(((unsigned long long)f * rcp) >> 32);
+    if (f - t * len >= len) t++;
+    return t;
+}
+struct RideSlice {
+    int r;
+    bool ok;
+    size_t e;
+};
+__host__ __device__ __forceinline__ unsigned ride_chunks_of(const PatchRide &rd, unsigned lin)
+{
+    const unsigned total = rd.chunks[0] + rd.chunks[1];
+    if (lin >= rd.blocks) return 0u;
+    unsigned rounds = 0;
+    for (unsigned i = 0; i < 4u; i++) rounds += lin + i * rd.blocks < total ? 1u : 0u;
+    return rounds;
+}
+__host__ __device__ __forceinline__ RideSlice ride_slice(const PatchReduce &red, const PatchRide &rd, int npair, int lgB, int64_t n, unsigned NT,
+                                                         unsigned lin, unsigned round, unsigned tid)
+{
+    RideSlice s;
+    s.r = -1; s.ok = false; s.e = 0;
+    if (lin >= rd.blocks) return s;
+    unsigned c = lin + round * rd.blocks;
+    if (c >= rd.chunks[0] + rd.chunks[1]) return s;
+    s.r = c >= rd.chunks[0] ? 1 : 0;
+    if (s.r) c -= rd.chunks[0];
+    const unsigned len = (unsigned)(red.hi[s.r] - red.lo[s.r]);
+    const unsigned count = len * (unsigned)npair;
+    unsigned f = c * NT + tid;
+    s.ok = f < count;
+    if (!s.ok) f = count - 1;
+    int k0, lw;
+    pair_block_at((int)div_by_rcp(f, len, rd.rcp[s.r]), npair, lgB, k0, lw);
+    s.e = (size_t)k0 * (size_t)n + ((size_t)red.lo[s.r] << lw) + (size_t)(f - len * (unsigned)k0);
+    return s;
+}
+static bool ride_fits(const PatchReduce &red, PatchRide &rd, int npair, int NT, int64_t blocks)
+{
+    rd = PatchRide{};
+    int64_t chunks = 0;
+    for (int r = 0; r < 2; r++) {
+        const int64_t len = (red.count[r] > 0 && red.Jd[r]) ? std::max(0, red.hi[r] - red.lo[r]) : 0;
+        const int64_t count = len * npair;
+        if (count > (int64_t)INT32_MAX - 4096) return false;
+        rd.chunks[r] = (unsigned)((count + NT - 1) / NT);
+        rd.rcp[r] = rcp32_of((unsigned)len);
+        chunks += rd.chunks[r];
+    }
+    if (chunks == 0 || blocks < 1 || blocks >= ((int64_t)1 << 29) || chunks > 4 * blocks) return false;
+    rd.on = 1;
+    rd.blocks = (unsigned)blocks;
+    return true;
+}
 __device__ __forceinline__ int reduce_block_index(const PatchArgs &pa)
 {
     const int rows = (int)gridDim.y - pa.prow;
@@ -167,11 +229,18 @@
     }
     __device__ __forceinline__ void steps(const PatchArgs &pa, int b0, int b1)
     {
-        if (kDiag) share = (unsigned long long)((b1 - b0 + pa.Q - 1) / pa.Q);
+        if (kDiag) share |= (unsigned long long)((b1 - b0 + pa.Q - 1) / pa.Q);
     }
     __device__ __forceinline__ void reduces()
     {
         if (kDiag) share = 1ull << 32;
+    }
+    __device__ __forceinline__ void rode(unsigned elements)
+    {
+        if (kDiag && slot) {
+            const unsigned long long dt = wall_clock64() - t0;
+            share |= ((unsigned long long)(elements & 0x3FFFu) << 33) | ((dt < 0xFFFFull ? dt : 0xFFFFull) << 48);
+        }
     }
     __device__ __forceinline__ ~BlockStamp()
     {
@@ -193,14 +262,28 @@
     if (b >= pa.red.nblk[r]) return;
     if (diag(pa.dbg, kDiagNoReduce)) return;
     const int len = pa.red.hi[r] - pa.red.lo[r];
-    const int per = NT * pa.red.ppb;
-    const int nblock = pair_block_count(pa.npair, pa.lgB);
-    int k0 = 0, lw = 0;
-    for (int k = 0; k < nblock; k++) {
-        pair_block_of(k, pa.npair, pa.lgB, k0, lw);
-        const int cnt = (int)((((int64_t)len << lw) + per - 1) / per);
-        if (b < cnt) break;
-        b -= cnt;
+    static_assert((NT & (NT - 1)) == 0, "blocks per pair block are counted with a shift");
+    const int lgper = (31 - __builtin_clz((unsigned)NT)) + (pa.red.ppb == 4 ? 2 : 0);
+    const int nfull = pa.npair >> pa.lgB;
+    int k0 = 0, lw = pa.lgB;
+    {
+        const unsigned cnt = (unsigned)((((unsigned long long)len << lw) + ((1u << lgper) - 1)) >> lgper);
+        const unsigned k = div_by_rcp((unsigned)b, cnt, pa.rows_rcp[r]);
+        if ((int)k < nfull) {
+            k0 = (int)k << pa.lgB;
+            b -= (int)(k * cnt);
+        } else {
+            b -= (int)((unsigned)nfull * cnt);
+            k0 = nfull << pa.lgB;
+            const int rest = pa.npair - k0;
+            for (lw = pa.lgB - 1; lw > 0; lw--)
+                if (rest & (1 << lw)) {
+                    const int c = (int)((((unsigned long long)len << lw) + ((1u << lgper) - 1)) >> lgper);
+                    if (b < c) break;
+                    b -= c;
+                    k0 += 1 << lw;
+                }
+        }
     }
     const int64_t nn = ta.n;
     const size_t run = (size_t)len << lw;
@@ -247,14 +330,82 @@
     }
 }
 
+template <typename T>
+struct RideLoads {
+    static constexpr int kEarly = sizeof(T) == 8 ? 5 : 6;
+    T x0, y0, x1, y1, x2, y2, x3, y3, x4, y4, x5, y5;
+    unsigned chunks = 0;
+};
+template <typename T>
+__device__ __forceinline__ void ride_load(const PatchArgs &pa, RideLoads<T> &rl, const RideSlice &s)
+{
+    typedef typename Pair<T>::type T2;
+    const T2 *I0 = reinterpret_cast<const T2 *>(pa.ta.I);
+    const size_t plane = (size_t)pa.npair * (size_t)pa.ta.n;
+    const int cnt = pa.red.count[s.r];
+    constexpr int kRideEarly = RideLoads<T>::kEarly;
+#define VRT_RIDE_LOAD(K) \
+    if (K < kRideEarly && K < cnt) { \
+        const T2 t = I0[(size_t)pa.red.angles[s.r][K] * plane + s.e]; \
+        rl.x##K = t.x; rl.y##K = t.y; \
+    }
+    VRT_RIDE_LOAD(0) VRT_RIDE_LOAD(1) VRT_RIDE_LOAD(2) VRT_RIDE_LOAD(3) VRT_RIDE_LOAD(4) VRT_RIDE_LOAD(5)
+#undef VRT_RIDE_LOAD
+}
+template <typename T>
+__device__ __forceinline__ void ride_sum(const PatchArgs &pa, const RideLoads<T> &rl, const RideSlice &s)
+{
+    typedef typename Pair<T>::type T2;
+    const T2 *I0 = reinterpret_cast<const T2 *>(pa.ta.I);
+    const size_t plane = (size_t)pa.npair * (size_t)pa.ta.n;
+    const int cnt = pa.red.count[s.r];
+    double ax = 0.0, ay = 0.0;
+    constexpr int kRideEarly = RideLoads<T>::kEarly;
+#define VRT_RIDE_SUM(J) \
+    if (J < kRideEarly && J < cnt) { \
+        const int a = pa.red.angles[s.r][J]; \
+        ax += pa.red.w[a] * (double)rl.x##J; \
+        ay += pa.red.w[a] * (double)rl.y##J; \
+    }
+    VRT_RIDE_SUM(0) VRT_RIDE_SUM(1) VRT_RIDE_SUM(2) VRT_RIDE_SUM(3) VRT_RIDE_SUM(4) VRT_RIDE_SUM(5)
+#undef VRT_RIDE_SUM
+    for (int j = kRideEarly; j < cnt; j++) {
+        const int a = pa.red.angles[s.r][j];
+        const double2 v = to_d2(I0[(size_t)a * plane + s.e]);
+        ax += pa.red.w[a] * v.x;
+        ay += pa.red.w[a] * v.y;
+    }
+    if (s.ok) reinterpret_cast<T2 *>(pa.red.Jd[s.r])[s.e] = from_d2<T>(make_double2(ax, ay));
+}
+template <typename T, int NT>
+__device__ __forceinline__ void ride_issue(const PatchArgs &pa, RideLoads<T> &rl)
+{
+    if (diag(pa.dbg, kDiagNoReduce)) return;
+    const unsigned lin = blockIdx.y * gridDim.x + blockIdx.x;
+    rl.chunks = ride_chunks_of(pa.ride, lin);
+    if (rl.chunks == 0) return;
+    ride_load<T>(pa, rl, ride_slice(pa.red, pa.ride, pa.npair, pa.lgB, pa.ta.n, NT, lin, 0, threadIdx.x));
+}
+template <typename T, int NT>
+__device__ __forceinline__ void ride_finish(const PatchArgs &pa, RideLoads<T> &rl, BlockStamp &stamp)
+{
+    if (rl.chunks == 0) return;
+    const unsigned lin = blockIdx.y * gridDim.x + blockIdx.x;
+    for (unsigned round = 0; round < rl.chunks; round++) {
+        const RideSlice s = ride_slice(pa.red, pa.ride, pa.npair, pa.lgB, pa.ta.n, NT, lin, round, threadIdx.x);
+        if (round > 0) ride_load<T>(pa, rl, s);
+        ride_sum<T>(pa, rl, s);
+    }
+    stamp.rode(rl.chunks * NT);
+}
+
 #ifdef VRT_PATCH_WPE
 #define VRT_WPE_ATTR __attribute__((amdgpu_waves_per_eu(VRT_PATCH_WPE, VRT_PATCH_WPE)))
 #else
 #define VRT_WPE_ATTR
 #endif
-template <typename T, int AM, int K, int Q, int NT>
-__global__ void __launch_bounds__(NT) VRT_WPE_ATTR
-k_patch_solve(PatchArgs pa)
+template <typename T, int AM, int K, int Q, int NT, bool RIDE>
+__device__ __forceinline__ void patch_solve_body(const PatchArgs &pa)
 {
     typedef typename Pair<T>::type T2;
     extern __shared__ __attribute__((aligned(16))) double2 ptile[];
@@ -266,19 +417,30 @@
         patch_reduce_role<T, NT>(pa);
         return;
     }
+    RideLoads<T> ride;
+    if constexpr (RIDE) ride_issue<T, NT>(pa, ride);
     const PatchBlock blk = patch_block(pa, pa.lgB);
     const int x = blk.lane, sj = blk.row;
     const int4 rec = pa.wrec[2 * (sj * 8 + x)], rec2 = pa.wrec[2 * (sj * 8 + x) + 1];
-    if (rec.y <= 0) return;
+    if (rec.y <= 0) {
+        if constexpr (RIDE) ride_finish<T, NT>(pa, ride, stamp);
+        return;
+    }
     const int sib = blk.sib;
     const int nblock = pair_block_count(pa.npair, pa.lgB);
     int b0, b1;
     split_blocks(pa, blk.split, nblock, b0, b1);
-    if (b0 >= b1) return;
+    if (b0 >= b1) {
+        if constexpr (RIDE) ride_finish<T, NT>(pa, ride, stamp);
+        return;
+    }
     {
         int k0, lw;
         pair_block_of(b0, pa.npair, pa.lgB, k0, lw);
-        if (sib >= (1 << lw)) return;
+        if (sib >= (1 << lw)) {
+            if constexpr (RIDE) ride_finish<T, NT>(pa, ride, stamp);
+            return;
+        }
     }
     stamp.steps(pa, b0, b1);
     const int ent_off = rec.x, n_ent = rec.y, own_lo = rec.z, own_cnt = rec.w;
@@ -307,6 +469,7 @@
         s_loc[i] = (l1 == 0xFFFFu ? (uint32_t)n_ent : l1) | ((l2 == 0xFFFFu ? (uint32_t)n_ent : l2) << 16);
         s_w1[i] = pa.e_w1[e]; s_w2[i] = pa.e_w2[e]; s_r1[i] = pa.e_r1[e]; s_r2[i] = pa.e_r2[e];
     }
+    if constexpr (RIDE) ride_finish<T, NT>(pa, ride, stamp);
     if (tid == 0) {
 #pragma unroll
         for (int qi = 0; qi < Q; qi++) ptile[qi * stride + n_ent] = make_double2(0.0, 0.0);
@@ -421,6 +584,19 @@
 }
 
 
+template <typename T, int AM, int K, int Q, int NT>
+__global__ void __launch_bounds__(NT) VRT_WPE_ATTR
+k_patch_solve(PatchArgs pa)
+{
+    patch_solve_body<T, AM, K, Q, NT, false>(pa);
+}
+template <typename T, int AM, int K, int Q, int NT>
+__global__ void __launch_bounds__(NT) VRT_WPE_ATTR
+k_ride_solve(PatchArgs pa)
+{
+    patch_solve_body<T, AM, K, Q, NT, true>(pa);
+}
+
 typedef int vrt_i32x8 __attribute__((ext_vector_type(8)));
 typedef const __attribute__((address_space(4))) vrt_i32x8 WorkRec;
 static_assert(2 * sizeof(int4) == 32 && sizeof(vrt_i32x8) == 32, "a work-list slot is two int4: 32 bytes, 32-byte aligned");
@@ -839,9 +1015,8 @@
     }
 }
 
-template <typename T, int AM, int NT>
-__global__ void __launch_bounds__(NT) VRT_LEAN_ATTR
-k_patch_lean(PatchArgs pa)
+template <typename T, int AM, int NT, bool RIDE>
+__device__ __forceinline__ void patch_lean_body(const PatchArgs &pa)
 {
     extern __shared__ __attribute__((aligned(16))) double2 ptile[];
     const int tid = threadIdx.x;
@@ -855,17 +1030,35 @@
     typename EntryTable<NT>::Regs early{};
     if (diag(pa.dbg, kDiagDirectTable))
         early = EntryTable<NT>::load(pa, min(pa.dbg_ent0 + (patch_row(pa) * 8 + ((int)blockIdx.x & 7)) * pa.dbg_ent_stride + tid, pa.dbg_ent_last));
+    RideLoads<T> ride;
+    if constexpr (RIDE) ride_issue<T, NT>(pa, ride);
     PatchItem it;
-    if (!patch_item(pa, pa.lgB, it)) return;
+    if (!patch_item(pa, pa.lgB, it)) {
+        if constexpr (RIDE) ride_finish<T, NT>(pa, ride, stamp);
+        return;
+    }
     stamp.steps(pa, it.b0, it.b1);
     if (diag(pa.dbg, kDiagNoPairLoop)) it.b1 = it.b0;
     const EntryTable<NT> tab(ptile, 1);
     if (tid == 0) ptile[it.n_ent] = make_double2(0.0, 0.0);
     if (diag(pa.dbg, kDiagDirectTable)) tab.store(early, it, tid);
     else tab.park(pa, it, tid);
+    if constexpr (RIDE) ride_finish<T, NT>(pa, ride, stamp);
     exp2_table_store(e2);
     __syncthreads();
     lean_pairs<T, AM, NT, 0>(pair_io<AM>(pa, it.d), it, tab, ptile);
+}
+template <typename T, int AM, int NT>
+__global__ void __launch_bounds__(NT) VRT_LEAN_ATTR
+k_patch_lean(PatchArgs pa)
+{
+    patch_lean_body<T, AM, NT, false>(pa);
+}
+template <typename T, int AM, int NT>
+__global__ void __launch_bounds__(NT) VRT_LEAN_ATTR
+k_ride_lean(PatchArgs pa)
+{
+    patch_lean_body<T, AM, NT, true>(pa);
 }
 
 
@@ -991,9 +1184,8 @@
 #ifndef VRT_QUAD_ATTR
 #define VRT_QUAD_ATTR __attribute__((amdgpu_waves_per_eu(6, 6)))
 #endif
-template <int AM, int NT>
-__global__ void __launch_bounds__(NT) VRT_QUAD_ATTR
-k_patch_quad(PatchArgs pa)
+template <int AM, int NT, bool RIDE>
+__device__ __forceinline__ void patch_quad_body(const PatchArgs &pa)
 {
     extern __shared__ __attribute__((aligned(16))) double2 ptile[];
     const int tid = threadIdx.x;
@@ -1004,8 +1196,13 @@
         return;
     }
     const double e2 = exp2_table_load();
+    RideLoads<float> ride;
+    if constexpr (RIDE) ride_issue<float, NT>(pa, ride);
     PatchItem it;
-    if (!patch_item(pa, pa.lgB - 1, it)) return;
+    if (!patch_item(pa, pa.lgB - 1, it)) {
+        if constexpr (RIDE) ride_finish<float, NT>(pa, ride, stamp);
+        return;
+    }
     stamp.steps(pa, it.b0, it.b1);
     const EntryTable<NT> tab(ptile, 2);
     if (tid == 0) {
@@ -1013,9 +1210,22 @@
         ptile[NT + 1 + it.n_ent] = make_double2(0.0, 0.0);
     }
     tab.park(pa, it, tid);
+    if constexpr (RIDE) ride_finish<float, NT>(pa, ride, stamp);
     exp2_table_store(e2);
     __syncthreads();
     quad_pairs<AM, NT, false>(pair_io<AM>(pa, it.d), it, tab, ptile);
+}
+template <int AM, int NT>
+__global__ void __launch_bounds__(NT) VRT_QUAD_ATTR
+k_patch_quad(PatchArgs pa)
+{
+    patch_quad_body<AM, NT, false>(pa);
+}
+template <int AM, int NT>
+__global__ void __launch_bounds__(NT) VRT_QUAD_ATTR
+k_ride_quad(PatchArgs pa)
+{
+    patch_quad_body<AM, NT, true>(pa);
 }
 
 
@@ -1261,29 +1471,45 @@
 #define VRT_PATCH_SHAPES(X) \
     X(1, 1, 256) X(1, 1, 512) X(1, 1, 1024) X(2, 1, 256) X(2, 1, 512) X(1, 2, 256) X(1, 2, 512) X(1, 2, 1024) X(2, 2, 512)
 
-template <typename T, int AM>
+template <typename T, int AM, bool RIDE>
 static int launch_shape(int K, int Q, int NT, dim3 grid, size_t lds, hipStream_t st, const PatchArgs &pa)
 {
     if constexpr (sizeof(T) == 4) {
         if (pa.quad) {
             switch (NT) {
-            case 256: hipLaunchKernelGGL((k_patch_quad<AM, 256>), grid, dim3(256), lds, st, pa); return VRT_OK;
-            case 512: hipLaunchKernelGGL((k_patch_quad<AM, 512>), grid, dim3(512), lds, st, pa); return VRT_OK;
-            case 1024: hipLaunchKernelGGL((k_patch_quad<AM, 1024>), grid, dim3(1024), lds, st, pa); return VRT_OK;
+            case 256: if constexpr (RIDE) hipLaunchKernelGGL((k_ride_quad<AM, 256>), grid, dim3(256), lds, st, pa);
+                      else hipLaunchKernelGGL((k_patch_quad<AM, 256>), grid, dim3(256), lds, st, pa);
+                      return VRT_OK;
+            case 512: if constexpr (RIDE) hipLaunchKernelGGL((k_ride_quad<AM, 512>), grid, dim3(512), lds, st, pa);
+                      else hipLaunchKernelGGL((k_patch_quad<AM, 512>), grid, dim3(512), lds, st, pa);
+                      return VRT_OK;
+            case 1024: if constexpr (RIDE) hipLaunchKernelGGL((k_ride_quad<AM, 1024>), grid, dim3(1024), lds, st, pa);
+                      else hipLaunchKernelGGL((k_patch_quad<AM, 1024>), grid, dim3(1024), lds, st, pa);
+                      return VRT_OK;
             default: break;
             }
         }
     }
     if (pa.lean && K == 1 && Q == 1) {
         switch (NT) {
-        case 256: hipLaunchKernelGGL((k_patch_lean<T, AM, 256>), grid, dim3(256), lds, st, pa); return VRT_OK;
-        case 512: hipLaunchKernelGGL((k_patch_lean<T, AM, 512>), grid, dim3(512), lds, st, pa); return VRT_OK;
-        case 1024: hipLaunchKernelGGL((k_patch_lean<T, AM, 1024>), grid, dim3(1024), lds, st, pa); return VRT_OK;
+        case 256: if constexpr (RIDE) hipLaunchKernelGGL((k_ride_lean<T, AM, 256>), grid, dim3(256), lds, st, pa);
+                  else hipLaunchKernelGGL((k_patch_lean<T, AM, 256>), grid, dim3(256), lds, st, pa);
+                  return VRT_OK;
+        case 512: if constexpr (RIDE) hipLaunchKernelGGL((k_ride_lean<T, AM, 512>), grid, dim3(512), lds, st, pa);
+                  else hipLaunchKernelGGL((k_patch_lean<T, AM, 512>), grid, dim3(512), lds, st, pa);
+                  return VRT_OK;
+        case 1024: if constexpr (RIDE) hipLaunchKernelGGL((k_ride_lean<T, AM, 1024>), grid, dim3(1024), lds, st, pa);
+                  else hipLaunchKernelGGL((k_patch_lean<T, AM, 1024>), grid, dim3(1024), lds, st, pa);
+                  return VRT_OK;
         default: break;
         }
     }
 #define VRT_PATCH_CASE(k, q, nt) \
-    if (K == k && Q == q && NT == nt) { hipLaunchKernelGGL((k_patch_solve<T, AM, k, q, nt>), grid, dim3(nt), lds, st, pa); return VRT_OK; }
+    if (K == k && Q == q && NT == nt) { \
+        if constexpr (RIDE) hipLaunchKernelGGL((k_ride_solve<T, AM, k, q, nt>), grid, dim3(nt), lds, st, pa); \
+        else hipLaunchKernelGGL((k_patch_solve<T, AM, k, q, nt>), grid, dim3(nt), lds, st, pa); \
+        return VRT_OK; \
+    }
     VRT_PATCH_SHAPES(VRT_PATCH_CASE)
 #undef VRT_PATCH_CASE
     return fail(VRT_EINVAL, "no patch kernel for this (entries per thread, pairs, threads) shape");
@@ -1292,10 +1518,17 @@
 template <typename T>
 static int launch_mode(int am, int K, int Q, int NT, dim3 grid, size_t lds, hipStream_t st, const PatchArgs &pa)
 {
+    if (pa.ride.on) {
+        switch (am) {
+        case VRT_ALPHA_SITE: return launch_shape<T, VRT_ALPHA_SITE, true>(K, Q, NT, grid, lds, st, pa);
+        case VRT_ALPHA_SITE_LAM: return launch_shape<T, VRT_ALPHA_SITE_LAM, true>(K, Q, NT, grid, lds, st, pa);
+        default: return launch_shape<T, VRT_ALPHA_ANGLE_SITE_LAM, true>(K, Q, NT, grid, lds, st, pa);
+        }
+    }
     switch (am) {
-    case VRT_ALPHA_SITE: return launch_shape<T, VRT_ALPHA_SITE>(K, Q, NT, grid, lds, st, pa);
-    case VRT_ALPHA_SITE_LAM: return launch_shape<T, VRT_ALPHA_SITE_LAM>(K, Q, NT, grid, lds, st, pa);
-    default: return launch_shape<T, VRT_ALPHA_ANGLE_SITE_LAM>(K, Q, NT, grid, lds, st, pa);
+    case VRT_ALPHA_SITE: return launch_shape<T, VRT_ALPHA_SITE, false>(K, Q, NT, grid, lds, st, pa);
+    case VRT_ALPHA_SITE_LAM: return launch_shape<T, VRT_ALPHA_SITE_LAM, false>(K, Q, NT, grid, lds, st, pa);
+    default: return launch_shape<T, VRT_ALPHA_ANGLE_SITE_LAM, false>(K, Q, NT, grid, lds, st, pa);
     }
 }
 
@@ -1325,7 +1558,7 @@
     return VRT_OK;
 }
 
-static void size_reduce(PatchReduce &red, int npair, int lgB, int NT)
+static void size_reduce(PatchReduce &red, unsigned rows_rcp[2], int npair, int lgB, int NT)
 {
     red.nred = 0;
     int64_t total = 0;
@@ -1337,6 +1570,7 @@
     for (int r = 0; r < 2; r++) {
         const int64_t len = red.hi[r] - red.lo[r];
         red.nblk[r] = 0;
+        rows_rcp[r] = rcp32_of((unsigned)((((uint64_t)std::max<int64_t>(len, 0) << lgB) + (uint64_t)per - 1) / (uint64_t)per));
         if (len > 0 && red.count[r] > 0 && red.Jd[r])
             for (int k = 0; k < nblock; k++) {
                 int k0, lw;
@@ -1359,7 +1593,7 @@
     PatchArgs pa;
     if (reduce) {
         pa.red = *reduce;
-        size_reduce(pa.red, npair, shape.lgB, p->patch_NT);
+        size_reduce(pa.red, pa.rows_rcp, npair, shape.lgB, p->patch_NT);
     }
     if (w1 <= w0 && pa.red.nred == 0) return VRT_OK;
     pa.ta = ta;
@@ -1409,6 +1643,14 @@
     pa.e_vis = p->e_vis; pa.e_loc = p->e_loc;
     pa.e_w1 = p->e_w1; pa.e_w2 = p->e_w2; pa.e_r1 = p->e_r1; pa.e_r2 = p->e_r2;
     pa.nrow = (int)((w1 - w0) / 8);
+    if (pa.red.nred > 0 && p->tune.patch_reduce_ride > 0 && pa.nrow > 0) {
+        const PatchGrid pg0 = patch_grid(p->tune.patch_order, pa.nrow, pa.nsplit, lgS, 0);
+        if (pg0.gy <= 65535 && ride_fits(pa.red, pa.ride, npair, p->patch_NT, pg0.gx * (int64_t)pg0.prow)) {
+            pa.red.nred = pa.red.nblk[0] = pa.red.nblk[1] = 0;
+            p->patch_rode_launches += 1;
+            p->patch_rode_chunks = std::max<int64_t>(p->patch_rode_chunks, ((int64_t)pa.ride.chunks[0] + pa.ride.chunks[1] + pa.ride.blocks - 1) / pa.ride.blocks);
+        }
+    }
     const PatchGrid pg = patch_grid(p->tune.patch_order, pa.nrow, pa.nsplit, lgS, pa.red.nred);
     pa.order = pg.order;
     pa.prow = pg.prow;
@@ -1484,6 +1726,44 @@
             split_blocks(sp, b.split, steps, b0, b1);
             o[1] = b.lane; o[2] = b.row; o[3] = b.split; o[4] = b.sib; o[5] = b1 - b0;
         }
+    return VRT_OK;
+}
+
+int patch_ride_map(int order, int nrow, int nsplit, int lg_siblings, int npair, int lg_block, int NT, int64_t n, const int32_t *lo,
+                   const int32_t *hi, int64_t first_block, int64_t nblocks, int64_t *dims, int64_t *elems)
+{
+    if (!dims || !lo || !hi) return fail(VRT_EINVAL, "NULL argument");
+    if (order < 0 || order > 1 || nrow < 1 || nrow > 65535 || nsplit < 1 || nsplit > 4096 || lg_siblings < 0 || lg_siblings > 4 ||
+        npair < 1 || lg_block < 0 || lg_block > 4 || NT < 64 || NT > 1024 || (NT & (NT - 1)) || n < 1 || n >= ((int64_t)1 << 28))
+        return fail(VRT_EINVAL, "ride map: argument out of range");
+    for (int r = 0; r < 2; r++)
+        if (lo[r] < 0 || hi[r] < lo[r] || hi[r] > n) return fail(VRT_EINVAL, "ride map: range outside the grid");
+    const PatchGrid pg = patch_grid(order, nrow, nsplit, lg_siblings, 0);
+    if (pg.gy > 65535) return fail(VRT_EINVAL, "more than 65535 rows of patch blocks");
+    const int64_t blocks = pg.gx * (int64_t)pg.prow;
+    PatchReduce red;
+    static double plane_tag;
+    for (int r = 0; r < 2; r++) {
+        red.lo[r] = lo[r]; red.hi[r] = hi[r];
+        red.count[r] = hi[r] > lo[r] ? 1 : 0;
+        red.Jd[r] = hi[r] > lo[r] ? &plane_tag : nullptr;
+    }
+    PatchRide rd;
+    const bool rides = ride_fits(red, rd, npair, NT, blocks);
+    dims[0] = blocks; dims[1] = rd.chunks[0]; dims[2] = rd.chunks[1]; dims[3] = rides ? 1 : 0;
+    if (!rides || !elems) return VRT_OK;
+    if (first_block < 0 || nblocks < 0 || first_block + nblocks > blocks) return fail(VRT_EINVAL, "ride map: no such blocks");
+    for (int64_t b = 0; b < nblocks; b++) {
+        const unsigned lin = (unsigned)(first_block + b), chunks = ride_chunks_of(rd, lin);
+        for (unsigned i = 0; i < 4; i++)
+            for (unsigned t = 0; t < (unsigned)NT; t++) {
+                int64_t &o = elems[(b * 4 + i) * NT + t];
+                o = -1;
+                if (i >= chunks) continue;
+                const RideSlice s = ride_slice(red, rd, npair, lg_block, n, (unsigned)NT, lin, i, t);
+                if (s.r >= 0 && s.ok) o = (int64_t)s.e | ((int64_t)s.r << 62);
+            }
+    }
     return VRT_OK;
 }
 
```

After: 92.68 billion, median of 6. 1.01x the previous value.
